# OrangeSodahub/InfGen

Measured on AMD Instinct MI355X. Metric: agent-steps/sec (closed-loop rollout), higher is better.
Workload: dtype f32

## Files before the change

### include/infgen_hip.h

```cpp
#ifndef INFGEN_HIP_H_
#define INFGEN_HIP_H_

#include <stdint.h>

#ifdef __cplusplus
extern "C" {
#endif

#define INFGEN_MAX_LAYERS 8

enum {
  INFGEN_Q_ATTN_PACK_SIZE = 0,
  INFGEN_Q_FOURIER_PACK_SIZE_N2 = 1,
  INFGEN_Q_FOURIER_PACK_SIZE_N3 = 2,
  INFGEN_Q_FOURIER_PACK_SIZE_N4 = 3,
  INFGEN_Q_TILE_ROWS = 4,
  INFGEN_Q_EDGE_ATTN_CAP = 5,
  INFGEN_Q_MAX_AGENTS = 6,
  INFGEN_Q_ABI_VERSION = 7,
  INFGEN_Q_SIZEOF_ROLLOUT = 8,
  INFGEN_Q_ATTN_SPLIT_ROWS = 9,
  INFGEN_Q_HEADS_SAMPLE_K = 10,
};
int infgen_layout_query(int what);
int infgen_attn_pack_offset(const char* field);
int infgen_fourier_pack_offset(const char* field, int n_dims, int dim);
const char* infgen_last_error(void);

typedef struct InfgenEdgeBuf {
  int* off;
  int* cnt;
  int* src;
  float* raw;
  float* rhat;
  int* total;
  int cap;
  int _pad;
} InfgenEdgeBuf;

typedef struct InfgenOptions {
  int use;
  int attn_mode;
  int gemm_terms;
  int fourier_mode;
  int edge_fuse;
  int edge_loop;
  int overlap;
  int row_group_margin;
  int layers_p;
  int rhat_format;
  int edge_kernel;
  int _pad0;
  const int* row_groups; const int* n_row_groups;
} InfgenOptions;

typedef struct InfgenRollout {
  int S, A_cap, T, M_cap, W, ring, R, token_size, grid_size, num_layers;
  int force_valid;
  int store_logits;
  float r_map, r_agent;
  const int* n_agents; const int* n_map; const int* av_index;
  float* pos; float* head; int* state; int* token; int* grid;
  uint8_t* tmask; uint8_t* imask; uint8_t* catflag;
  const int* type; int* bos;
  const float* map_pos; const float* map_orient;
  const float* attn_t[INFGEN_MAX_LAYERS]; const float* attn_m[INFGEN_MAX_LAYERS]; const float* attn_a[INFGEN_MAX_LAYERS];
  const float* four_t; const float* four_m; const float* four_a; const float* four_xa;
  const float* fusion_pack;
  const float* tok_head_pack; const float* st_head_pack;
  const float* tok_tab; const float* grid_tab; const float* state_emb;
  const float* cat_agent; const float* cat_seed; const float* vocab; const float* grid_xy;
  float* ringK[INFGEN_MAX_LAYERS]; float* ringV[INFGEN_MAX_LAYERS];
  const float* mapK[INFGEN_MAX_LAYERS]; const float* mapV[INFGEN_MAX_LAYERS];
  float* X; float* Q; float* U; float* Ka; float* Va; float* AGG; float* Z; float* SIG;
  InfgenEdgeBuf et, em, ea;
  float* raw2; float* cat; float* fus_in; float* tmp1; float* tmp2;
  int* next_token; int* next_state;
  float* logits;
  const int* teacher_token; const int* teacher_state;
  float* pred_traj; float* pred_head; float* pred_state;
  const int* first_new; const float* hv_ovr;
  int sample_k; int _pad1;
  const float* sample_u; float* logits_scratch;
  InfgenOptions opts;
  const int* teacher_grid;
  const float* four_t_dt;
  const float* teacher_pos; const float* teacher_head;
  const unsigned char* replay_row;
  const int* map_scene;
  float* tap_x;
  float* sample_logprob;
  float* token_logprob;
  int no_grid_token; int no_state_token;
} InfgenRollout;

int infgen_linear(const float* X, int ldx, const int* gather, int rows, int K,
                  const float* Wp, int Np, const float* bias, int N,
                  const float* pre_g, const float* pre_b, const float* post_g, const float* post_b, int relu,
                  float* Y, int ldy, void* stream);

typedef struct InfgenLinearDesc {
  const float* X; int ldx; const int* gather; int rows; int K;
  const float* Wp; int Np; const float* bias; int N;
  const float* pre_g; const float* pre_b; const float* post_g; const float* post_b; int relu;
  float* Y; int ldy;
} InfgenLinearDesc;
int infgen_linear_multi(const InfgenLinearDesc* desc, int n, void* stream);
int infgen_mlp_embedding(const float* X, int ldx, int rows, int K0, const float* pack, float* tmp1, float* tmp2,
                         float* Y, int ldy, void* stream);
int infgen_layernorm(const float* X, int rows, const float* gamma, const float* beta, float* Y, void* stream);
int infgen_fourier_embed(const float* raw, int n_dims, const int* count_dev, int e_cap, const float* pack,
                         const float* cat, int ldcat, float* out, int ldo, int normalize, void* stream);
int infgen_fourier_last_dim_table(const float* pack, int n_dims, float* table, void* stream);
int infgen_fourier_embed_tab(const float* raw, int n_dims, const int* count_dev, int e_cap, const float* pack,
                             const float* table, float* out, int ldo, int normalize, void* stream);
int infgen_set_fourier_mode(int mode);
int infgen_set_attn_mode(int mode);
int infgen_attn_pre(const float* X, int rows, const float* pack, int use_src_ln,
                    float* Q, float* U, float* K, float* V, void* stream);
int infgen_edge_attn(int rows, const float* Q, const float* U, const float* Ksrc, const float* Vsrc,
                     const int* off, const int* cnt, const int* src, const float* rhat,
                     float* AGG, float* Z, float* SIG, void* stream);
int infgen_edge_attn_fused(int rows, const float* Q, const float* pack, const float* Ksrc, const float* Vsrc,
                           const int* off, const int* cnt, const int* src, const float* rhat,
                           float* AGG, void* stream);
int infgen_fourier_embed_r24(const float* raw, int n_dims, const int* count_dev, int e_cap, const float* pack, void* out, void* stream);
int infgen_edge_attn_fused_r24(int rows, const float* Q, const float* pack, const float* Ksrc, const float* Vsrc,
                               const int* off, const int* cnt, const int* src, const void* rhat24, float* AGG, void* stream);
int infgen_set_rhat_format(int format);
int infgen_set_edge_kernel(int kernel);
int infgen_set_edge_fuse(int mode);
int infgen_get_options(InfgenOptions* out);
int infgen_thread_options(const InfgenOptions* o);
int infgen_get_effective_options(InfgenOptions* out);
int infgen_edge_fused_occupancy(void);
int infgen_debug_stream_read(const float* p, unsigned long long n_bytes, int width, float* out, void* stream);
int infgen_set_edge_loop(int variant);
int infgen_set_overlap(int mode);
int infgen_set_layers_p(int mode);
int infgen_layers_p_capacity(void);
int infgen_edge_attn_mode(int rows, const float* Q, const float* U, const float* Ksrc, const float* Vsrc,
                          const int* off, const int* cnt, const int* src, const float* rhat,
                          float* AGG, float* Z, float* SIG, int wide, void* stream);
int infgen_attn_post(float* X, int rows, const float* pack, const float* AGG, const float* Z, const float* SIG,
                     int has_pos, void* stream);
int infgen_attn_post_pre(float* X, int rows, const float* pack, const float* AGG, const float* Z, const float* SIG,
                         int has_pos, const float* next_pack, float* nQ, float* nU, float* nK, float* nV, void* stream);
int infgen_heads(const float* X, int rows, const float* tok_pack, const float* st_pack, int token_size,
                 float* logits, int* next_token, int* next_state, void* stream);
int infgen_heads_logprob(const float* X, int rows, const float* tok_pack, const float* st_pack, int token_size,
                         float* logits, int* next_token, int* next_state, float* token_logprob, void* stream);
int infgen_token_logprob(const float* logits, int rows, int n, const int* token, float* out, void* stream);
int infgen_heads_sample(const float* X, int rows, const float* tok_pack, const float* st_pack, int token_size, int k,
                        const float* uniform, float* logits, int* next_token, int* next_state, float* token_logprob,
                        float* sample_logprob, void* stream);
int infgen_heads_sample_fused(int attn_mode, int rows, int k);
int infgen_heads_logprob_fused(int attn_mode, int rows);
int infgen_map_token_head(const float* X, int ldx, const int* gather, int n, const float* pack, int token_size,
                          float* hidden, float* logits, long long* top_idx, void* stream);
int infgen_embedding_sum4(const float* tab0, const long long* idx0, int n0, const float* tab1, const long long* idx1, int n1,
                          const float* tab2, const long long* idx2, int n2, const float* tab3, const long long* idx3, int n3,
                          int rows, float* out, void* stream);
int infgen_map_graph(int S, int M_cap, const int* n_map, const float* pos, const float* orient, float radius,
                     int max_nbr, int* off, int* cnt, int* src, float* raw, int* total, int cap, void* stream);

int infgen_rollout_validate(const InfgenRollout* r);
int infgen_build_edges(const InfgenRollout* r, int c, int edgeless, void* stream);
int infgen_integrate(const InfgenRollout* r, int t, void* stream);
int infgen_raw_feature(const InfgenRollout* r, int col, void* stream);
int infgen_raw_feature_rows(const InfgenRollout* r, int col, const int* row_list, const int* row_mask, int n, void* stream);
int infgen_decode_layers(const InfgenRollout* r, int c, int edgeless, void* stream);
int infgen_decode_step(const InfgenRollout* r, int t, void* stream);
int infgen_rollout_run(const InfgenRollout* r, int t0, int t1, void* stream);

int infgen_sample_topk(const float* logits, int rows, int n, int k, const float* uniform, int* token, void* stream);
int infgen_sample_topk_logprob(const float* logits, int rows, int n, int k, const float* uniform, int* token,
// ... 178 lines not shown
```

### infgen_amd/_lib.py

```python
from __future__ import annotations

import ctypes as C
import threading
import os
from typing import Optional

_HERE = os.path.dirname(os.path.abspath(__file__))
LIB_PATH = os.path.join(_HERE, 'libinfgen_hip.so')
MAX_LAYERS = 8

_p = C.c_void_p
_i = C.c_int
_f = C.c_float


class LinearDesc(C.Structure):
    _fields_ = [('X', C.c_void_p), ('ldx', C.c_int), ('gather', C.c_void_p), ('rows', C.c_int), ('K', C.c_int),
                ('Wp', C.c_void_p), ('Np', C.c_int), ('bias', C.c_void_p), ('N', C.c_int),
                ('pre_g', C.c_void_p), ('pre_b', C.c_void_p), ('post_g', C.c_void_p), ('post_b', C.c_void_p), ('relu', C.c_int),
                ('Y', C.c_void_p), ('ldy', C.c_int)]


class EdgeBuf(C.Structure):
    _fields_ = [('off', _p), ('cnt', _p), ('src', _p), ('raw', _p), ('rhat', _p), ('total', _p),
# ... 1 lines not shown


class RadiusEdges(C.Structure):
    _fields_ = [('n_q', _i), ('_pad0', _i),
                ('q_node', _p), ('q_pt', _p), ('q_c0', _p), ('q_c1', _p), ('q_self', _p), ('q_pair_off', _p),
                ('p_pos', _p), ('p_head', _p), ('p_inv', _p),
                ('c_pos', _p), ('c_head', _p), ('c_inv', _p), ('c_ok', _p), ('c_src', _p), ('pair_ok', _p),
                ('radius', C.c_float), ('K', _i), ('gap_rule', _i), ('index_diff', _i), ('e_base', _i), ('_pad1', _i)]


class Insertion(C.Structure):
    _fields_ = [('attn_occ2sa', _p * 3), ('attn_pt2sa', _p * 3), ('attn_a2sa', _p * 3),
                ('four_a2sa', _p), ('four_pt2sa', _p),
                ('head_state', _p), ('head_type', _p), ('head_shape', _p), ('head_pos', _p), ('head_heading', _p),
                ('head_offset', _p), ('occ_embed', _p), ('shape_emb', _p), ('type_a_emb', _p), ('f_seed', _p),
                ('occ', _p), ('occ_emb', _p), ('Kocc', _p * 3), ('Vocc', _p * 3), ('mapK', _p * 3), ('mapV', _p * 3),
                ('Ksa', _p * 3), ('Vsa', _p * 3), ('Kh', _p * 3), ('Vh', _p * 3), ('Xc', _p),
                ('zero_agg', _p), ('zero_z', _p), ('zero_sig', _p),
                ('XS', _p), ('QS', _p), ('US', _p), ('AGGS', _p), ('ZS', _p), ('SIGS', _p), ('KN', _p), ('VN', _p),
                ('ea_s', EdgeBuf), ('em_s', EdgeBuf), ('ea_h', EdgeBuf), ('em_h', EdgeBuf),
                ('occ_off', _p), ('occ_cnt', _p), ('occ_src', _p),
                ('active', _p), ('n_new', _p), ('inserted', _p), ('new_row', _p), ('new_cell', _p), ('new_local', _p), ('new_shape', _p),
                ('prev_row', _p), ('prev_mask', _p), ('pend_row', _p), ('pend_mask', _p),
                ('hv_ovr', _p), ('shape_all', _p),
                ('hid', _p), ('lg_state', _p), ('lg_type', _p), ('shape', _p), ('lg_pos', _p), ('lg_heading', _p), ('offset', _p),
                ('t1', _p), ('t2', _p), ('shp', _p), ('host_dec', _p),
                ('r_seed', C.c_float), ('r_a2sa', C.c_float), ('r_pl2sa', C.c_float), ('angle_interval', C.c_float),
                ('n_heading', _i), ('force_enter', _i), ('insert_k', _i), ('max_new', _i),
                ('head_pos_xy', _p), ('head_heading_theta', _p), ('no_grid_token', _i), ('no_head_token', _i)]


class Options(C.Structure):
    _fields_ = [('use', _i), ('attn_mode', _i), ('gemm_terms', _i), ('fourier_mode', _i), ('edge_fuse', _i), ('edge_loop', _i),
                ('overlap', _i), ('row_group_margin', _i), ('layers_p', _i), ('rhat_format', _i), ('edge_kernel', _i), ('_pad0', _i), ('row_groups', _p), ('n_row_groups', _p)]


OPTIONS_VALUE_BYTES = C.sizeof(_i) * 12


class Rollout(C.Structure):
    _fields_ = [
        ('S', _i), ('A_cap', _i), ('T', _i), ('M_cap', _i), ('W', _i), ('ring', _i), ('R', _i),
        ('token_size', _i), ('grid_size', _i), ('num_layers', _i), ('force_valid', _i), ('store_logits', _i),
        ('r_map', _f), ('r_agent', _f),
        ('n_agents', _p), ('n_map', _p), ('av_index', _p),
        ('pos', _p), ('head', _p), ('state', _p), ('token', _p), ('grid', _p),
        ('tmask', _p), ('imask', _p), ('catflag', _p), ('type', _p), ('bos', _p),
        ('map_pos', _p), ('map_orient', _p),
        ('attn_t', _p * MAX_LAYERS), ('attn_m', _p * MAX_LAYERS), ('attn_a', _p * MAX_LAYERS),
        ('four_t', _p), ('four_m', _p), ('four_a', _p), ('four_xa', _p),
        ('fusion_pack', _p), ('tok_head_pack', _p), ('st_head_pack', _p),
        ('tok_tab', _p), ('grid_tab', _p), ('state_emb', _p), ('cat_agent', _p), ('cat_seed', _p),
        ('vocab', _p), ('grid_xy', _p),
        ('ringK', _p * MAX_LAYERS), ('ringV', _p * MAX_LAYERS), ('mapK', _p * MAX_LAYERS), ('mapV', _p * MAX_LAYERS),
        ('X', _p), ('Q', _p), ('U', _p), ('Ka', _p), ('Va', _p), ('AGG', _p), ('Z', _p), ('SIG', _p),
        ('et', EdgeBuf), ('em', EdgeBuf), ('ea', EdgeBuf),
        ('raw2', _p), ('cat', _p), ('fus_in', _p), ('tmp1', _p), ('tmp2', _p),
        ('next_token', _p), ('next_state', _p), ('logits', _p),
        ('teacher_token', _p), ('teacher_state', _p),
        ('pred_traj', _p), ('pred_head', _p), ('pred_state', _p),
        ('first_new', _p), ('hv_ovr', _p),
        ('sample_k', _i), ('_pad1', _i), ('sample_u', _p), ('logits_scratch', _p),
        ('opts', Options),
        ('teacher_grid', _p),
        ('four_t_dt', _p),
        ('teacher_pos', _p), ('teacher_head', _p),
        ('replay_row', _p),
        ('map_scene', _p),
        ('tap_x', _p),
        ('sample_logprob', _p),
        ('token_logprob', _p),
        ('no_grid_token', _i), ('no_state_token', _i),
    ]


class BatchIngest(C.Structure):
    _fields_ = ([(k, _i) for k in ('S', 'copies', 'A_cap', 'M_cap', 'T', 'T0', 'P', 'hc', 'H', 'motion_cols', 'pos_dim',
                                   'pt_pos_dim', 'n_polygons', '_pad0')] +
                [(k, _p) for k in ('agent_ptr', 'pt_ptr', 'av_index', 'src_graph', 'state_idx', 'token_idx', 'grid_token_idx',
                                   'token_pos', 'token_heading', 'raw_valid', 'valid_mask', 'shape', 'position', 'heading', 'type',
                                   'id', 'pt_position', 'pt_orientation', 'pt_token_idx', 'pt_type', 'pt_pl_type', 'pt_polygon',
                                   'light_type',
                                   'pos', 'head', 'state', 'token', 'gridtok', 'tmask', 'imask', 'catflag', 'atype', 'bos',
                                   'shape10', 'n_agents', 'av', 'n_map', 'map_pos', 'map_orient', 'map_tok', 'map_type', 'map_pl',
                                   'map_light', 'htok', 'hst', 'p0', 'h0', 'shp', 'gt', 'val', 'ids', 'counts',
                                   'replay_in', 'plan_token', 'plan_state', 'plan_pos', 'plan_head',
                                   'teacher_token', 'teacher_state', 'teacher_pos', 'teacher_head', 'replay_row')])


SYMBOLS = {
    'infgen_layout_query': (_i, [_i]),
    'infgen_attn_pack_offset': (_i, [C.c_char_p]),
    'infgen_fourier_pack_offset': (_i, [C.c_char_p, _i, _i]),
    'infgen_last_error': (C.c_char_p, []),
    'infgen_linear': (_i, [_p, _i, _p, _i, _i, _p, _i, _p, _i, _p, _p, _p, _p, _i, _p, _i, _p]),
    'infgen_linear_multi': (_i, [_p, _i, _p]),
    'infgen_radius_edges': (_i, [_p, _p, _p]),
    'infgen_motion_features': (_i, [_p, _p, _p, _p, _i, _i, _p, _p]),
    'infgen_layernorm': (_i, [_p, _i, _p, _p, _p, _p]),
    'infgen_fourier_embed': (_i, [_p, _i, _p, _i, _p, _p, _i, _p, _i, _i, _p]),
    'infgen_set_fourier_mode': (_i, [_i]),
    'infgen_set_attn_mode': (_i, [_i]),
# ... 3 lines not shown
    'infgen_rollout_validate': (_i, [_p]),
    'infgen_set_edge_loop': (_i, [_i]),
    'infgen_set_rhat_format': (_i, [_i]),
    'infgen_set_edge_kernel': (_i, [_i]),
    'infgen_mlp_embedding': (_i, [_p, _i, _i, _i, _p, _p, _p, _p, _i, _p]),
    'infgen_get_options': (_i, [C.POINTER(Options)]),
    'infgen_thread_options': (_i, [C.POINTER(Options)]),
    'infgen_get_effective_options': (_i, [C.POINTER(Options)]),
    'infgen_edge_fused_occupancy': (_i, []),
    'infgen_debug_stream_read': (_i, [_p, C.c_ulonglong, _i, _p, _p]),
    'infgen_set_overlap': (_i, [_i]),
    'infgen_edge_attn_fused': (_i, [_i, _p, _p, _p, _p, _p, _p, _p, _p, _p, _p]),
    'infgen_edge_attn_fused_r24': (_i, [_i, _p, _p, _p, _p, _p, _p, _p, _p, _p, _p]),
    'infgen_fourier_embed_r24': (_i, [_p, _i, _p, _i, _p, _p, _p]),
    'infgen_embedding_sum4': (_i, [_p, _p, _i, _p, _p, _i, _p, _p, _i, _p, _p, _i, _i, _p, _p]),
    'infgen_fourier_last_dim_table': (_i, [_p, _i, _p, _p]),
    'infgen_fourier_embed_tab': (_i, [_p, _i, _p, _i, _p, _p, _p, _i, _i, _p]),
    'infgen_distance_to_nearest_object': (_i, [_p, _p, _p, _p, _p, _p, _i, _i, _i, _i, C.c_float, _p, _p, _p]),
    'infgen_kinematic_features': (_i, [_p, _p, _p, _p, _i, _i, C.c_float, _p, _p, _p, _p, _p]),
    'infgen_time_to_collision': (_i, [_p, _p, _p, _p, _p, _p, _p, _p, _i, _i, _i, _i, _p, _p]),
    'infgen_set_gemm_terms': (_i, [_i]),
    'infgen_active_row_groups': (_i, [_p, _i, _i, _i, _p, _p, _p]),
    'infgen_set_row_groups': (_i, [_p, _p, _i]),
    'infgen_set_row_limits': (_i, [_p, _i, _i]),
    'infgen_fetch_enterings': (_i, [_p] * 5 + [_i] * 3 + [_p, _i, _f, _f, _i, _i] + [_p] * 9 + [_i, _p, _i, _p, _p]),
    'infgen_tokenize_agent': (_i, [_p] * 9 + [_i] * 10 + [_p] * 8),
    'infgen_distance_to_road_edge': (_i, [_p] * 9 + [_i] * 4 + [_p, _p, _p, _i, _f, _p, _p]),
    'infgen_window_log_likelihood': (_i, [_p, _p, _i, _i, _i, _i, _p, _p, _i, _p, _p, _p]),
    'infgen_placement_features': (_i, [_p, _p, _p, _p, _p, _i, _i, _i, _i, _i, _p, _p, _p, _p, _p]),
    'infgen_bundle_scores': (_i, [_p] * 14 + [_i] * 11 + [_p] * 5),
    'infgen_match_map_tokens': (_i, [_p, _p, _p, _i, _i, _p, _p]),
    'infgen_match_agent_tokens': (_i, [_p, _p, _p, _p, _p, _p, C.c_longlong, _i, _i, _i, _i, _p, _p, _p]),
    'infgen_attn_pre': (_i, [_p, _i, _p, _i, _p, _p, _p, _p, _p]),
    'infgen_edge_attn': (_i, [_i, _p, _p, _p, _p, _p, _p, _p, _p, _p, _p, _p, _p]),
    'infgen_edge_attn_mode': (_i, [_i, _p, _p, _p, _p, _p, _p, _p, _p, _p, _p, _p, _i, _p]),
    'infgen_attn_post': (_i, [_p, _i, _p, _p, _p, _p, _i, _p]),
    'infgen_attn_post_pre': (_i, [_p, _i, _p, _p, _p, _p, _i, _p, _p, _p, _p, _p, _p]),
    'infgen_heads': (_i, [_p, _i, _p, _p, _i, _p, _p, _p, _p]),
    'infgen_heads_logprob': (_i, [_p, _i, _p, _p, _i, _p, _p, _p, _p, _p]),
    'infgen_token_logprob': (_i, [_p, _i, _i, _p, _p, _p]),
    'infgen_heads_sample': (_i, [_p, _i, _p, _p, _i, _i, _p, _p, _p, _p, _p, _p, _p]),
    'infgen_heads_sample_fused': (_i, [_i, _i, _i]),
    'infgen_heads_logprob_fused': (_i, [_i, _i]),
    'infgen_map_token_head': (_i, [_p, _i, _p, _i, _p, _i, _p, _p, _p, _p]),
    'infgen_map_graph': (_i, [_i, _i, _p, _p, _p, _f, _i, _p, _p, _p, _p, _p, _i, _p]),
    'infgen_build_edges': (_i, [C.POINTER(Rollout), _i, _i, _p]),
    'infgen_integrate': (_i, [C.POINTER(Rollout), _i, _p]),
    'infgen_raw_feature': (_i, [C.POINTER(Rollout), _i, _p]),
    'infgen_raw_feature_rows': (_i, [_p, _i, _p, _p, _i, _p]),
    'infgen_decode_layers': (_i, [C.POINTER(Rollout), _i, _i, _p]),
    'infgen_decode_step': (_i, [C.POINTER(Rollout), _i, _p]),
    'infgen_rollout_run': (_i, [C.POINTER(Rollout), _i, _i, _p]),
    'infgen_sample_topk': (_i, [_p, _i, _i, _i, _p, _p, _p]),
    'infgen_sample_topk_logprob': (_i, [_p, _i, _i, _i, _p, _p, _p, _p]),
    'infgen_occupancy': (_i, [C.POINTER(Rollout), _i, _p, _p]),
    'infgen_occupancy_embed': (_i, [C.POINTER(Rollout), _i, _p, _p, _p, _p]),
    'infgen_point_edges': (_i, [C.POINTER(Rollout), _i, _p, _p, _i, _i, _f, _i, _f, _i, C.POINTER(EdgeBuf), C.POINTER(EdgeBuf), _p]),
    'infgen_insert_decide': (_i, [C.POINTER(Rollout), _i, _i, _i, _p, _p, _p, _p, _p, _p, _p, _p, _p, _p, _p, _p]),
    'infgen_insert_seed': (_i, [C.POINTER(Rollout), C.POINTER(Insertion), _i, _i, _i, _p, _p]),
    'infgen_insert_heading': (_i, [C.POINTER(Rollout), C.POINTER(Insertion), _i, _i, _i, _p]),
    'infgen_insert_decide_topk': (_i, [C.POINTER(Rollout), _i, _i, _i, _p, _p, _p, _p, _p, _p, _p, _p, _p, _p, _p, _i, _p, _p]),
    'infgen_insert_finalize': (_i, [C.POINTER(Rollout), _i, _f, _p, _p, _p, _i, _p, _p, _p]),
    'infgen_prof_enable': (_i, [C.c_uint, _i]),
    'infgen_prof_collect': (_i, [C.POINTER(C.c_double), C.POINTER(_i), C.POINTER(C.c_double), C.POINTER(C.c_ulonglong)]),
    'infgen_prof_collect_steps': (_i, [C.POINTER(C.c_double), C.POINTER(_i), C.POINTER(C.c_double), C.POINTER(C.c_ulonglong),
                                       C.POINTER(C.c_double), C.POINTER(_i)]),
# ... 22 lines not shown


class InfgenHipError(RuntimeError):
    pass


def load() -> C.CDLL:
    global _lib
    if _lib is not None:
        return _lib
    if not os.path.exists(LIB_PATH):
        raise InfgenHipError(
            f'{LIB_PATH} not found: build it with `python -c "import __graft_entry__ as g; g.build()"` '
            f'or `make -C infgen_amd/csrc` (there is no CPU fallback for the product path)')
    import torch
    lib = C.CDLL(LIB_PATH)
    for name, (res, args) in SYMBOLS.items():
        fn = getattr(lib, name)
        fn.restype = res
        fn.argtypes = args
    if lib.infgen_layout_query(Q_SIZEOF_ROLLOUT) != C.sizeof(Rollout):
        raise InfgenHipError('InfgenRollout layout mismatch between include/infgen_hip.h and infgen_amd/_lib.py: '
                             f'{lib.infgen_layout_query(Q_SIZEOF_ROLLOUT)} != {C.sizeof(Rollout)}')
    _lib = lib
    return lib


def check(rc: int, what: str = '') -> None:
    if rc != 0:
        msg = load().infgen_last_error()
        raise InfgenHipError(f'{what} failed ({rc}): {msg.decode() if msg else "?"}')


def ptr(t) -> Optional[int]:
    if t is None:
        return None
    assert t.is_contiguous(), 'tensor must be contiguous'
    return t.data_ptr()


_tl = threading.local()


class thread_options:

    def __init__(self, opts: 'Options'):
        self.opts, self.prev = opts, None

    def __enter__(self):
        lib = load()
        depth = getattr(_tl, 'depth', 0)
        if depth > 0:
            self.prev = Options()
            check(lib.infgen_get_effective_options(C.byref(self.prev)), 'infgen_get_effective_options')
        check(lib.infgen_thread_options(C.byref(self.opts)), 'infgen_thread_options')
        _tl.depth = depth + 1
        return self

    def __exit__(self, *exc):
        _tl.depth -= 1
        check(load().infgen_thread_options(C.byref(self.prev) if self.prev is not None else None), 'infgen_thread_options')
        return False


_prof_mask = 0


def prof_enable(mask: int, max_launches: int = 20000) -> None:
    global _prof_mask
    check(load().infgen_prof_enable(mask, max_launches), 'infgen_prof_enable')
# ... 33 lines not shown
```

### infgen_amd/csrc/api.hip

```cpp
#include <cstdio>
#include <cstring>
#include <cstdlib>
#include <string>
#include <vector>
#include <atomic>
#include <mutex>
#include <unordered_map>
#include "kernels.h"
#include "../../include/infgen_hip.h"

using namespace ig;

static thread_local std::string g_err;

static int fail(const char* where, const char* what) {
  g_err = std::string(where) + ": " + what;
  return -1;
}
static int check_launch(const char* where) {
  hipError_t e = hipGetLastError();
  if (e != hipSuccess) return fail(where, hipGetErrorString(e));
  return 0;
}
#define RET_IF(x) do { int _r = (x); if (_r) return _r; } while (0)

extern "C" const char* infgen_last_error(void) { return g_err.c_str(); }

static int env_int(const char* name, int dflt, bool* is_set = nullptr) {
  const char* e = getenv(name);
  if (is_set) *is_set = e != nullptr;
  return e ? atoi(e) : dflt;
}
static int env_layers_p() { const int v = env_int("INFGEN_LAYERS_P", 1); return v < 0 ? 0 : v > 2 ? 2 : v; }
static int env_lp_rows_min() {
  bool set8 = false;
  const int rows8 = env_int("INFGEN_LP_ROWS8", 0, &set8);
  return set8 ? (rows8 ? 8 : 16) : env_int("INFGEN_LP_ROWS_MIN", 4);
}
namespace knob {
const int layers_p = env_layers_p();
const int qs_dbg = env_int("INFGEN_QS_DBG", 0);
const int fh12_min = env_int("INFGEN_FH12_MIN", 150000);
const int fh12_multi_rows = env_int("INFGEN_FH12_MULTI_ROWS", 0);
const int fourier_nomulti = env_int("INFGEN_FOURIER_NOMULTI", 0);
const int attn_hs_max = env_int("INFGEN_ATTN_HS_MAX", 6144);
const int attn_waves = env_int("INFGEN_ATTN_WAVES", IG_QSU ? 8 : 4);
const int warm = env_int("INFGEN_WARM", 1);
const int warm_max_groups = env_int("INFGEN_WARM_MAX_GROUPS", 128);
const int edge_dbg = env_int("INFGEN_EDGE_DBG", 0);
const int edge_noxcd = env_int("INFGEN_EDGE_NOXCD", 0);
const int edge_small = env_int("INFGEN_EDGE_SMALL", 4096);
const int edge_wg2 = env_int("INFGEN_EDGE_WG2", 1);
const int edge_lds_pad = env_int("INFGEN_EDGE_LDS_PAD", 0);
const int heads_nosplit = env_int("INFGEN_HEADS_NOSPLIT", 0);
const int be_wide_scenes = env_int("INFGEN_BE_WIDE_SCENES", 128);
const int int_group_scenes = env_int("INFGEN_INT_GROUP_SCENES", 128);
const int no_tail_fold = env_int("INFGEN_NO_TAIL_FOLD", 0);
const int lp_max_chunks = env_int("INFGEN_LP_MAX_CHUNKS", 2);
const int lp_max_groups = env_int("INFGEN_LP_MAX_GROUPS", 256);
const int lp_rows_min = env_lp_rows_min();
const int lp_trace = env_int("INFGEN_LP_TRACE", 0);
const char* const lp_spin_str = getenv("INFGEN_LP_SPIN_LIMIT");
const unsigned lp_spin_limit = lp_spin_str ? (unsigned)strtoul(lp_spin_str, nullptr, 0) : 0u;
}

namespace {
InfgenOptions g_def = {0,  2,  3,  1,  1,  6,  0,
                        0,  knob::layers_p,  0,  1, 0, nullptr, nullptr};
int g_def_group_rows = 0;
const int* g_def_limit_n_agents = nullptr;
int g_def_limit_A_cap = 0;
struct Active { const InfgenOptions* o; int group_rows; const int* n_agents; int A_cap; };
thread_local Active tl_active = {nullptr, 0, nullptr, 0};
thread_local InfgenOptions tl_thread_opts;
thread_local bool tl_thread_set = false;
inline const InfgenOptions& O() { return tl_active.o ? *tl_active.o : tl_thread_set ? tl_thread_opts : g_def; }
inline int group_rows() { return tl_active.o ? tl_active.group_rows : g_def_group_rows; }
inline const int* limit_n_agents() { return tl_active.o ? tl_active.n_agents : g_def_limit_n_agents; }
inline int limit_A_cap() { return tl_active.o ? tl_active.A_cap : g_def_limit_A_cap; }
struct OptScope {
  Active prev;
  explicit OptScope(const InfgenRollout* r) : prev(tl_active) {
    if (r && r->opts.use) tl_active = Active{&r->opts, r->S * r->A_cap, r->opts.row_groups ? r->n_agents : nullptr, r->A_cap};
  }
  ~OptScope() { tl_active = prev; }
};
}

extern "C" int infgen_get_options(InfgenOptions* out) {
  if (!out) return fail("infgen_get_options", "null pointer");
  *out = g_def;
  return 0;
}

extern "C" int infgen_thread_options(const InfgenOptions* o) {
  if (o) { tl_thread_opts = *o; tl_thread_opts.row_groups = nullptr; tl_thread_opts.n_row_groups = nullptr; }
  tl_thread_set = o != nullptr;
  return 0;
}

extern "C" int infgen_get_effective_options(InfgenOptions* out) {
// ... 352 lines not shown
  if (per <= 0) return grid;
  w = req; w.wg0 = wg0; w.per_xcd = per;
  return wg0 + 8 * per;
}

static void launch_attn_h(const AttnHArgs& a_in, void* stream) {
  AttnHArgs a = a_in;
  a.dbg = knob::qs_dbg;
  if (O().row_groups && a.rows == group_rows()) { a.groups = O().row_groups; a.n_groups = O().n_row_groups; }
  if (attn_kind(a.rows) == 2) {
    const int grid = warm_take(a.warm, ceil_div(a.rows, 16));
    hipLaunchKernelGGL(by_terms(k_attn_hs<3>, k_attn_hs_b16<1>, k_attn_hs<1>), dim3(grid), dim3(512), 0, (hipStream_t)stream, a);
    return;
  }
  t_warm = WarmArgs{};
  if (knob::attn_waves != 8) {
    auto kern = by_terms(k_attn_h<4, 3>, k_attn_h_b16<4, 1>, k_attn_h<4, 1>);
    hipLaunchKernelGGL(kern, dim3(grid64(a.rows)), dim3(256), 0, (hipStream_t)stream, a);
  } else {
    int grid = ceil_div(a.rows, 128);
    if (grid > 256) grid = 256;
    hipLaunchKernelGGL((k_attn_h<8, 3>), dim3(grid), dim3(512), 0, (hipStream_t)stream, a);
  }
}

static double attn_pre_macs(int rows, const void* Q, const void* U, const void* K, const void* V) {
  return (double)rows * 16384.0 * ((Q || U ? 1 : 0) + (K ? 1 : 0) + (V ? 1 : 0) + (U ? 1 : 0));
}
static double attn_post_macs(int rows, int has_pos, const void* next_pack, const void* nQ, const void* nU, const void* nK, const void* nV) {
  return (double)rows * (196608.0 + (has_pos ? 16384.0 : 0.0)) + (next_pack ? attn_pre_macs(rows, nQ, nU, nK, nV) : 0.0);
}
static double heads_macs(int rows, int token_size) { return (double)rows * (2 * 16384.0 + 128.0 * token_size + 384.0); }

extern "C" int infgen_attn_pre(const float* X, int rows, const float* pack, int use_src_ln,
                               float* Q, float* U, float* K, float* V, void* stream) {
  if (rows <= 0) return 0;
  { ProfScope _ps(INFGEN_KID_ATTN_PRE, stream, attn_pre_macs(rows, Q, U, K, V));
    if (attn_kind(rows)) {
      launch_attn_h(AttnHArgs{const_cast<float*>(X), rows, nullptr, nullptr, nullptr, nullptr, 0, pack, use_src_ln, Q, U, K, V}, stream);
    } else {
      AttnPreArgs a{X, rows, pack, use_src_ln, Q, U, K, V};
      hipLaunchKernelGGL(k_attn_pre, dim3(ceil_div(rows, TR)), dim3(NT), 0, (hipStream_t)stream, a);
    } }
  return check_launch("infgen_attn_pre");
}

static int edge_attn_impl(int rows, const float* Q, const float* U, const float* Ksrc, const float* Vsrc,
                          const int* off, const int* cnt, const int* src, const float* rhat,
                          float* AGG, float* Z, float* SIG, int wide, void* stream, const int* row_mask = nullptr) {
  if (rows <= 0) return 0;
  EdgeAttnArgs a{rows, Q, U, Ksrc, Vsrc, EdgeSet{off, cnt, src, rhat}, AGG, Z, SIG, nullptr, nullptr, 0, 0, wide ? row_mask : nullptr};
  if (limit_n_agents() && O().row_groups && rows == group_rows() && !wide) {
    a.n_agents = limit_n_agents(); a.A_cap = limit_A_cap(); a.margin = O().row_group_margin;
  }
  { ProfScope _ps(INFGEN_KID_EDGE_ATTN, stream);
    if (wide) hipLaunchKernelGGL(k_edge_attn_wide, dim3(rows), dim3(512), 0, (hipStream_t)stream, a);
    else hipLaunchKernelGGL(k_edge_attn, dim3(ceil_div(rows, 4)), dim3(NT), 0, (hipStream_t)stream, a); }
  return check_launch("infgen_edge_attn");
}

extern "C" int infgen_set_edge_fuse(int mode) {
  if (mode < 0 || mode > 2) return fail("infgen_set_edge_fuse", "mode must be 0 (off), 1 (from 257 rows) or 2 (always)");
  g_def.edge_fuse = mode;
  return 0;
}

extern "C" int infgen_set_rhat_format(int format) {
  if (format != 0 && format != 1) return fail("infgen_set_rhat_format", "format must be 0 (fp32 rows) or 1 (packed 24-bit rows)");
  g_def.rhat_format = format;
  return 0;
}

extern "C" int infgen_set_edge_kernel(int kernel) {
  if (kernel < 0 || kernel > 2) return fail("infgen_set_edge_kernel", "kernel must be 0, 1 or 2");
  g_def.edge_kernel = kernel;
  return 0;
}

extern "C" int infgen_set_edge_loop(int v) {
  if (v != 4 && v != 6 && v != 8) return fail("infgen_set_edge_loop", "edges per trip must be 4, 6 or 8");
  g_def.edge_loop = v;
  return 0;
}

extern "C" int infgen_edge_fused_occupancy(void) {
  int n = -1;
  if (hipOccupancyMaxActiveBlocksPerMultiprocessor(&n, k_edge_fused<6, true, 1, 8>, 512, 0) != hipSuccess) return -1;
  return n;
}

static int edge_fused_launch(int rows, const float* Q, const float* pack, const float* Ksrc, const float* Vsrc, const EdgeSet& es,
                             float* AGG, int rows_per_scene, int kv_once, void* stream, int r24 = 0) {
  if (rows <= 0) return 0;
  if (!pack || !es.rhat) return fail("infgen_edge_attn_fused", "needs the layer pack and rhat");
  const int dbg = knob::edge_dbg, no_xcd = knob::edge_noxcd, small_max = knob::edge_small, wg2 = knob::edge_wg2;
  const int G = O().edge_loop;
  const bool small = rows <= small_max && G == 6;
  const bool two = !small && wg2 && G == 6;
  const int tr = (small || two) ? 16 : 32;
  EdgeFusedArgs a{rows, Q, pack, Ksrc, Vsrc, es, AGG, nullptr, nullptr, dbg, 0, kv_once};
  int grid = ceil_div(rows, tr);
  if (O().row_groups && rows == group_rows()) { a.groups = O().row_groups; a.n_groups = O().n_row_groups; }
  else if (rows_per_scene > tr && rows_per_scene % tr == 0 && !(no_xcd & 1)) {
    a.tiles_per_scene = rows_per_scene / tr;
    const int grp = 8 * a.tiles_per_scene;
    grid = ceil_div(grid, grp) * grp;
  }
  if (no_xcd & 2) a.kv_once = 0;
  if (!r24 && (O().edge_kernel == 2 || (O().edge_kernel == 1 && !small))) {
    EdgeFusedArgs m = a;
    int mg = ceil_div(rows, 16);
    m.tiles_per_scene = 0;
    if (!m.groups && rows_per_scene > 16 && rows_per_scene % 16 == 0 && !(no_xcd & 1)) {
      m.tiles_per_scene = rows_per_scene / 16;
      const int grp = 8 * m.tiles_per_scene;
      mg = ceil_div(mg, grp) * grp;
    }
    m.n_virtual = mg;
    t_warm = WarmArgs{};
    { ProfScope _ps(INFGEN_KID_EDGE_ATTN, stream);
      auto k3 = G == 4 ? k_edge_fused3<4> : G == 8 ? k_edge_fused3<8> : k_edge_fused3<6>;
      hipLaunchKernelGGL(k3, dim3(mg), dim3(512), knob::edge_lds_pad, (hipStream_t)stream, m); }
    return check_launch("infgen_edge_attn_fused(k_edge_fused3)");
  }
  a.n_virtual = grid;
  if (small) grid = warm_take(a.warm, grid); else t_warm = WarmArgs{};
  static unsigned long long* ef_trace = nullptr;
  if (dbg & 128) {
    if (!ef_trace && hipMalloc(&ef_trace, 64 * sizeof(unsigned long long)) != hipSuccess) return fail("infgen_edge_attn_fused", "trace buffer");
    (void)hipMemsetAsync(ef_trace, 0, 64 * sizeof(unsigned long long), (hipStream_t)stream);
    a.dbgbuf = reinterpret_cast<unsigned*>(ef_trace);
  }
  { ProfScope _ps(INFGEN_KID_EDGE_ATTN, stream);
    auto kern = small ? (r24 ? k_edge_fused<6, true, 1, 16> : k_edge_fused<6, false, 1, 16>)
              : two ? (r24 ? k_edge_fused<6, true, 1, 8> : k_edge_fused<6, false, 1, 8>)
              : r24 ? (G == 4 ? k_edge_fused<4, true, 2, 16> : G == 8 ? k_edge_fused<8, true, 2, 16> : k_edge_fused<6, true, 2, 16>)
                    : (G == 4 ? k_edge_fused<4, false, 2, 16> : G == 8 ? k_edge_fused<8, false, 2, 16> : k_edge_fused<6, false, 2, 16>);
    hipLaunchKernelGGL(kern, dim3(grid), dim3(two ? 512 : 1024), 0, (hipStream_t)stream, a); }
  if (dbg & 128) {
    static int dumps = 0;
    if (dumps++ < 3) {
      unsigned long long hst[64];
      (void)hipStreamSynchronize((hipStream_t)stream);
      (void)hipMemcpy(hst, ef_trace, sizeof(hst), hipMemcpyDeviceToHost);
      for (int i = 1; i < 8; ++i) fprintf(stderr, "[ef trace] %d +%lld\n", i, hst[i] && hst[0] ? (long long)(hst[i] - hst[0]) : -1ll);
    }
  }
  return check_launch("infgen_edge_attn_fused");
}

extern "C" int infgen_edge_attn_fused(int rows, const float* Q, const float* pack, const float* Ksrc, const float* Vsrc,
                                      const int* off, const int* cnt, const int* src, const float* rhat,
                                      float* AGG, void* stream) {
  return edge_fused_launch(rows, Q, pack, Ksrc, Vsrc, EdgeSet{off, cnt, src, rhat}, AGG, 0, 0, stream);
}

extern "C" int infgen_fourier_embed_r24(const float* raw, int n, const int* count_dev, int e_cap, const float* pack, void* out,
                                        void* stream) {
  return fourier_embed_impl(raw, n, count_dev, e_cap, pack, nullptr, 0, static_cast<float*>(out), 128, 1, 1, stream);
}

extern "C" int infgen_edge_attn_fused_r24(int rows, const float* Q, const float* pack, const float* Ksrc, const float* Vsrc,
                                          const int* off, const int* cnt, const int* src, const void* rhat24,
                                          float* AGG, void* stream) {
  return edge_fused_launch(rows, Q, pack, Ksrc, Vsrc, EdgeSet{off, cnt, src, static_cast<const float*>(rhat24)}, AGG, 0, 0, stream, 1);
}

extern "C" int infgen_edge_attn(int rows, const float* Q, const float* U, const float* Ksrc, const float* Vsrc,
                                const int* off, const int* cnt, const int* src, const float* rhat,
                                float* AGG, float* Z, float* SIG, void* stream) {
  return edge_attn_impl(rows, Q, U, Ksrc, Vsrc, off, cnt, src, rhat, AGG, Z, SIG, rows <= 256 ? 1 : 0, stream);
}

extern "C" int infgen_edge_attn_mode(int rows, const float* Q, const float* U, const float* Ksrc, const float* Vsrc,
                                     const int* off, const int* cnt, const int* src, const float* rhat,
                                     float* AGG, float* Z, float* SIG, int wide, void* stream) {
  return edge_attn_impl(rows, Q, U, Ksrc, Vsrc, off, cnt, src, rhat, AGG, Z, SIG, wide, stream);
}

static int attn_post_fused(float* X, int rows, const float* pack, const float* AGG, const float* Z, const float* SIG,
                           int has_pos, const float* next_pack, float* nQ, float* nU, float* nK, float* nV, void* stream) {
  if (rows <= 0) return 0;
  { ProfScope _ps(INFGEN_KID_ATTN_POST, stream, attn_post_macs(rows, has_pos, next_pack, nQ, nU, nK, nV));
    if (attn_kind(rows)) {
      launch_attn_h(AttnHArgs{X, rows, pack, AGG, Z, SIG, has_pos, next_pack, 0, nQ, nU, nK, nV}, stream);
    } else {
      AttnPostArgs a{X, rows, pack, AGG, Z, SIG, has_pos, next_pack, nQ, nU, nK, nV};
      hipLaunchKernelGGL(k_attn_post, dim3(ceil_div(rows, TR)), dim3(NT), 0, (hipStream_t)stream, a);
    } }
  return check_launch("infgen_attn_post");
}

extern "C" int infgen_attn_post(float* X, int rows, const float* pack, const float* AGG, const float* Z,
                                const float* SIG, int has_pos, void* stream) {
  return attn_post_fused(X, rows, pack, AGG, Z, SIG, has_pos, nullptr, nullptr, nullptr, nullptr, nullptr, stream);
}

extern "C" int infgen_attn_post_pre(float* X, int rows, const float* pack, const float* AGG, const float* Z,
                                    const float* SIG, int has_pos, const float* next_pack, float* nQ, float* nU,
                                    float* nK, float* nV, void* stream) {
  return attn_post_fused(X, rows, pack, AGG, Z, SIG, has_pos, next_pack, nQ, nU, nK, nV, stream);
}

extern "C" int infgen_match_agent_tokens(const unsigned char* valid, const float* pos, const float* heading, const float* shape,
                                        const int* type, const float* tok, long long tok_agent_stride, int A, int T, int shift,
                                        int n_token, int* token_index, float* token_contour, void* stream) {
  if (A <= 0) return 0;
  if (shift <= 0 || T <= shift) return fail("infgen_match_agent_tokens", "need 0 < shift < T");
  if (n_token <= 0 || n_token > 2048) return fail("infgen_match_agent_tokens", "n_token must be in 1..2048");
  MatchTokensArgs a{valid, pos, heading, shape, type, tok, tok_agent_stride, A, T, shift, n_token, token_index, token_contour};
  hipLaunchKernelGGL(k_match_tokens, dim3(A), dim3(256), 0, (hipStream_t)stream, a);
  return check_launch("infgen_match_agent_tokens");
}

extern "C" int infgen_tokenize_agent(unsigned char* valid, float* pos, float* heading, float* velocity, const int* type,
                                    const float* tok, const float* shape_in, float* shape_out, float* wl_work, int A, int T,
                                    int shift, int current_step, int n_token, int invalid_state, int valid_state,
                                    int enter_state, int exit_state, int predict_state, int* token_index,
                                    float* token_contour, int* state_idx, float* token_pos, float* token_heading,
                                    unsigned char* token_valid, unsigned char* raw_token_valid, void* stream) {
  if (A <= 0) return 0;
  if (shift <= 0 || T <= shift || current_step < shift || current_step >= T)
    return fail("infgen_tokenize_agent", "need 0 < shift <= current_step < T");
  if (n_token <= 0 || n_token > 2048) return fail("infgen_tokenize_agent", "n_token must be in 1..2048");
  TokenizeArgs t{valid, pos, heading, velocity, type, wl_work, shape_in, shape_out, A, T, shift, current_step,
                 invalid_state, valid_state, enter_state, exit_state, predict_state, token_index, token_contour,
                 state_idx, token_pos, token_heading, token_valid, raw_token_valid};
  hipLaunchKernelGGL(k_tokenize_prep, dim3((A + 63) / 64), dim3(64), 0, (hipStream_t)stream, t);
  MatchTokensArgs m{valid, pos, heading, wl_work, type, tok, 0, A, T, shift, n_token, token_index, token_contour};
  hipLaunchKernelGGL(k_match_tokens, dim3(A), dim3(256), 0, (hipStream_t)stream, m);
  hipLaunchKernelGGL(k_tokenize_state, dim3((A + 63) / 64), dim3(64), 0, (hipStream_t)stream, t);
  return check_launch("infgen_tokenize_agent");
}

// ... 379 lines not shown
                nullptr, nullptr, nullptr, nullptr, 0, logits, token_size};
  const int gy = tiles < 512 ? min(passes, ceil_div(512, tiles)) : 1;
  hipLaunchKernelGGL(k_linear, dim3(tiles, gy), dim3(NT), 0, s, l1);
  hipLaunchKernelGGL(k_map_topk, dim3(ceil_div(n, 4)), dim3(256), 0, s, a);
  return check_launch("infgen_map_token_head");
}

extern "C" int infgen_embedding_sum4(const float* tab0, const long long* idx0, int n0, const float* tab1, const long long* idx1, int n1,
                                     const float* tab2, const long long* idx2, int n2, const float* tab3, const long long* idx3, int n3,
                                     int rows, float* out, void* stream) {
  if (rows <= 0) return 0;
  if (!tab0 || !tab1 || !tab2 || !tab3 || !idx0 || !idx1 || !idx2 || !idx3 || !out || n0 < 1 || n1 < 1 || n2 < 1 || n3 < 1)
    return fail("infgen_embedding_sum4", "null table / index array or empty table");
  EmbedSum4Args a{{tab0, tab1, tab2, tab3}, {idx0, idx1, idx2, idx3}, {n0, n1, n2, n3}, rows, out};
  hipLaunchKernelGGL(k_embedding_sum4, dim3((unsigned)(((long long)rows * 32 + NT - 1) / NT)), dim3(NT), 0, (hipStream_t)stream, a);
  return check_launch("infgen_embedding_sum4");
}

extern "C" int infgen_map_graph(int S, int M_cap, const int* n_map, const float* pos, const float* orient,
                                float radius, int max_nbr, int* off, int* cnt, int* src, float* raw, int* total,
                                int cap, void* stream) {
  if (S <= 0 || M_cap <= 0) return 0;
  if (hipMemsetAsync(total, 0, sizeof(int), (hipStream_t)stream) != hipSuccess)
    return fail("infgen_map_graph", "memset failed");
  MapGraphArgs a{S, M_cap, n_map, pos, orient, radius, max_nbr, EdgeBuf{off, cnt, src, raw, total, cap}, 0};
  a.lds_tokens = (M_cap <= 4096 && M_cap % (4 * MAP_GRAPH_C) == 0) ? M_cap : 0;
  { ProfScope _ps(INFGEN_KID_MAP_GRAPH, stream);
    hipLaunchKernelGGL(k_map_graph, dim3(ceil_div(S * M_cap, 4 * MAP_GRAPH_C)), dim3(NT), (size_t)a.lds_tokens * 12, (hipStream_t)stream, a); }
  return check_launch("infgen_map_graph");
}

static SceneState scene_of(const InfgenRollout* r) {
  SceneState st;
  st.S = r->S; st.A_cap = r->A_cap; st.T = r->T; st.M_cap = r->M_cap; st.W = r->W; st.ring = r->ring;
  st.n_agents = r->n_agents; st.n_map = r->n_map; st.av_index = r->av_index;
  st.pos = r->pos; st.head = r->head; st.state = r->state; st.token = r->token; st.grid = r->grid;
  st.tmask = r->tmask; st.imask = r->imask; st.catflag = r->catflag; st.type = r->type; st.bos = r->bos;
  st.map_pos = r->map_pos; st.map_orient = r->map_orient; st.map_scene = r->map_scene;
  st.first_new = r->first_new; st.hv_ovr = r->hv_ovr;
  return st;
}
static EdgeBuf ebuf(const InfgenEdgeBuf& e) { return EdgeBuf{e.off, e.cnt, e.src, e.raw, e.total, e.cap}; }
static EdgeSet eset(const InfgenEdgeBuf& e) { return EdgeSet{e.off, e.cnt, e.src, e.rhat}; }

static int validate(const InfgenRollout* r, const char* where) {
  if (!r) return fail(where, "null context");
  if (r->A_cap > 1024 || r->A_cap <= 0) return fail(where, "A_cap must be in 1..1024");
  if (r->A_cap % 32) return fail(where, "A_cap must be a multiple of 32");
  if (r->num_layers <= 0 || r->num_layers > INFGEN_MAX_LAYERS) return fail(where, "bad num_layers");
  if (r->ring <= r->W) return fail(where, "ring must exceed the temporal window");
  if (r->W > 16) return fail(where, "temporal window larger than 16 columns is not supported");
  if ((r->no_grid_token | r->no_state_token) & ~1) return fail(where, "no_grid_token / no_state_token must be 0 or 1");
  if (r->token_logprob && !(r->store_logits && r->logits) && !r->logits_scratch) {
    const int mode = (r->opts.use ? r->opts : O()).attn_mode;
    const bool sampled = r->sample_k > 1 && r->sample_u;
    const bool fused = sampled ? heads_sample_fused_for(mode, r->S * r->A_cap, r->sample_k) : attn_split_for(mode, r->S * r->A_cap);
    if (!fused) return fail(where, "token_logprob needs store_logits or logits_scratch [rows][token_size] (few rows, or sampling)");
  }
  return 0;
}

static int build_edges_impl(const InfgenRollout* r, int c, int edgeless, void* stream, bool zero_totals, unsigned long long* clear_keys = nullptr,
                            bool clear_sync = false) {
  RET_IF(validate(r, "infgen_build_edges"));
  OptScope _opts(r);
  hipStream_t s = (hipStream_t)stream;
  if (!edgeless && zero_totals) {
    if (r->em.total == r->et.total + 1 && r->ea.total == r->et.total + 2) {
      if (hipMemsetAsync(r->et.total, 0, 3 * sizeof(int), s) != hipSuccess) return fail("infgen_build_edges", "memset failed");
    } else if (hipMemsetAsync(r->et.total, 0, sizeof(int), s) != hipSuccess ||
               hipMemsetAsync(r->em.total, 0, sizeof(int), s) != hipSuccess ||
               hipMemsetAsync(r->ea.total, 0, sizeof(int), s) != hipSuccess)
      return fail("infgen_build_edges", "memset failed");
  }
  BuildEdgesArgs a;
  a.st = scene_of(r); a.c = c; a.edgeless = edgeless; a.r_map = r->r_map; a.r_agent = r->r_agent;
  a.rows = r->S * r->A_cap; a.t = ebuf(r->et); a.m = ebuf(r->em); a.a = ebuf(r->ea);
  a.clear_keys = clear_keys;
  a.clear_sync = clear_sync ? reinterpret_cast<int*>(r->SIG) : nullptr;
  a.prof = (g_prof.mask & ((1u << INFGEN_KID_EDGE_ATTN) | (1u << INFGEN_KID_BUILD_EDGES))) ? g_prof.rows_dev : nullptr;
  { ProfScope _ps(INFGEN_KID_BUILD_EDGES, stream);
    a.map_lds = r->M_cap < 4096 ? r->M_cap : 4096;
    const size_t lds = (size_t)a.map_lds * 8;
// ... 251 lines not shown
    if (hipEventRecord(g_ev_m, g_side) != hipSuccess) return fail("infgen_decode_layers", "event failed");
    RET_IF(launch_fourier(step_fourier_set(r, FS_AGENT, sm), g_side));
    if (hipEventRecord(g_ev_a, g_side) != hipSuccess) return fail("infgen_decode_layers", "event failed");
    RET_IF(launch_fourier(step_fourier_set(r, FS_TEMPORAL, sm), stream));
  } else if (fourier_multi_ok(rows, edgeless)) {
    const int n_sets = with_xa ? 4 : 3;
    FourierMultiArgs m;
    for (int k = 0; k < n_sets; ++k) m.set[k] = step_fourier_set(r, (FourierSet)k, sm);
    int cap = r->et.cap > r->em.cap ? r->et.cap : r->em.cap;
    if (r->ea.cap > cap) cap = r->ea.cap;
    const bool wide = knob::fh12_multi_rows > 0 && rows >= knob::fh12_multi_rows && three_terms() && FH_WAVES == 8;
    const int grid = fourier_h_grid(cap, wide);
    { ProfScope _ps(INFGEN_KID_FOURIER, stream);
      if (wide) hipLaunchKernelGGL(k_fourier_h12_multi<3>, dim3(grid, n_sets), dim3(FH12_NT), 0, (hipStream_t)stream, m);
      else hipLaunchKernelGGL(by_terms(k_fourier_h_multi<3>, k_fourier_h_multi_b16<1>, k_fourier_h_multi<1>), dim3(grid, n_sets),
                              dim3(FH_NT), 0, (hipStream_t)stream, m); }
    RET_IF(check_launch("infgen_decode_layers(fourier)"));
  } else if (!edgeless) {
    for (FourierSet k : {FS_TEMPORAL, FS_MAP, FS_AGENT}) RET_IF(launch_fourier(step_fourier_set(r, k, sm), stream));
  }
  return 0;
}

constexpr int LP_REFUSED = -12345;
static int layers_p_launch(const InfgenRollout* r, int c, const StepMode& sm, void* stream, bool sync_clear = true) {
  const int rows = r->S * r->A_cap;
  LayersPArgs a;
  a.rows = rows; a.A_cap = r->A_cap; a.num_layers = r->num_layers;
  a.X = r->X;
  for (int i = 0; i < r->num_layers; ++i) {
    a.attn_t[i] = r->attn_t[i]; a.attn_m[i] = r->attn_m[i]; a.attn_a[i] = r->attn_a[i];
    a.ringK[i] = r->ringK[i]; a.ringV[i] = r->ringV[i]; a.mapK[i] = r->mapK[i]; a.mapV[i] = r->mapV[i];
  }
  a.slot_off = (size_t)(c % r->ring) * rows * D;
  a.Ka[0] = r->Ka; a.Va[0] = r->Va; a.Ka[1] = r->U; a.Va[1] = r->U + (size_t)rows * D;
  a.et = eset(r->et); a.em = eset(r->em); a.ea = eset(r->ea);
  a.sync = reinterpret_cast<int*>(r->SIG);
  a.trace = nullptr;
  const int lp_trace = knob::lp_trace;
  static unsigned long long* trace_dev = nullptr;
  if (lp_trace) {
    if (!trace_dev && hipMalloc(&trace_dev, 2048 * sizeof(unsigned long long)) != hipSuccess) return fail("infgen_decode_layers", "trace buffer");
    (void)hipMemsetAsync(trace_dev, 0, 2048 * sizeof(unsigned long long), (hipStream_t)stream);
    a.trace = trace_dev;
  }
  if (sync_clear && hipMemsetAsync(a.sync, 0, (size_t)r->S * sizeof(int), (hipStream_t)stream) != hipSuccess)
    return fail("infgen_decode_layers", "memset failed");
  const int limit = lp_limit();
  a.rows_per_wg = 16;
  for (int rr = 8; rr >= 4 && rr >= knob::lp_rows_min; rr >>= 1)
    if (r->A_cap % rr == 0 && rows / rr <= (rr == 4 ? limit / 2 : limit)) a.rows_per_wg = rr;
  const int gps = r->A_cap / a.rows_per_wg;
  const int per = rows / a.rows_per_wg <= limit ? r->S : (a.rows_per_wg == 16 ? lp_chunk_scenes(r, limit) : 0);
  if (per <= 0 || per * gps > infgen_layers_p_capacity()) return fail("infgen_decode_layers", "k_layers_p: batch does not fit the device's resident capacity");
  auto kern = a.rows_per_wg == 4 ? (sm.r24 ? k_layers_p<true, 4> : k_layers_p<false, 4>)
            : a.rows_per_wg == 8 ? (sm.r24 ? k_layers_p<true, 8> : k_layers_p<false, 8>)
                                 : (sm.r24 ? k_layers_p<true, 16> : k_layers_p<false, 16>);
  const bool capturing = is_capturing(stream);
  a.spin_limit = capturing ? (1u << 22) : knob::lp_spin_str ? knob::lp_spin_limit : (O().layers_p == 2 ? 0u : (1u << 24));
  std::unique_lock<std::mutex> lk(g_lp_mu, std::defer_lock);
  LpOrder& ord = g_lp_order[lp_current_device()];
  if (!capturing) {
    lk.lock();
    if (!ord.ev && hipEventCreateWithFlags(&ord.ev, hipEventDisableTiming) != hipSuccess)
      return fail("infgen_decode_layers", "event creation failed");
    if (ord.any && hipStreamWaitEvent((hipStream_t)stream, ord.ev, 0) != hipSuccess) {
      (void)hipGetLastError();
      ord.any = false;
// ... 15 lines not shown
        (void)hipGetLastError();
        if (s0 > 0) return fail("infgen_decode_layers", "k_layers_p: cooperative launch of a later chunk refused");
        g_lp_refused.store(true);
        return LP_REFUSED;
      }
    }
  }
  if (!capturing) {
    ord.any = hipEventRecord(ord.ev, (hipStream_t)stream) == hipSuccess;
    if (!ord.any) (void)hipGetLastError();
    lk.unlock();
  }
  if (lp_trace) {
    static int dumps = 0;
    if (dumps++ == lp_trace) {
      std::vector<unsigned long long> h(2048);
      (void)hipStreamSynchronize((hipStream_t)stream);
      (void)hipMemcpy(h.data(), trace_dev, 2048 * sizeof(unsigned long long), hipMemcpyDeviceToHost);
      for (int i = 0; i < 1024 && (i == 0 || h[2 * i + 1]); ++i)
        fprintf(stderr, "[lp trace] %d %llu %llu\n", i, h[2 * i], i ? h[2 * i + 1] - h[2 * i - 1] : 0ull);
    }
  }
  return check_launch("infgen_decode_layers(k_layers_p)");
}

static int layers_core(const InfgenRollout* r, int c, int edgeless, void* stream, bool lp_sync_clear = true) {
  const int rows = r->S * r->A_cap;
  const StepMode sm = step_mode(r, rows, edgeless, stream);
  if (sm.lp && sm.fuse) {
    const int rc = layers_p_launch(r, c, sm, stream, lp_sync_clear);
    if (rc != LP_REFUSED) return rc;
  }
  const bool overlap = sm.overlap, fuse = sm.fuse; const int r24 = sm.r24;
  const size_t slot = (size_t)(c % r->ring) * rows * D;
  const int L = r->num_layers;
  float* U = fuse ? nullptr : r->U;
  const float* Z = fuse ? nullptr : r->Z;
  const float* SIG = fuse ? nullptr : r->SIG;
  const int has_pos = fuse ? 0 : 1;
  const int QB = 16384;
  const bool skip_edges = edgeless && fuse;
  if (skip_edges && hipMemsetAsync(r->AGG, 0, (size_t)rows * D * sizeof(float), (hipStream_t)stream) != hipSuccess)
    return fail("infgen_decode_layers", "memset failed");
  auto edge = [&](const float* pack, const float* Ks, const float* Vs, const InfgenEdgeBuf& e, int kv_once = 0, const float* next_pack = nullptr, int fmt = -1) {
    if (skip_edges) return 0;
    if (fuse && O().attn_mode != 0)
      warm_request(pack + AH_POST + 4 * (QB / 4), 48 * QB, next_pack ? next_pack + AH_PRE : nullptr, 16 * QB);
    return fuse ? edge_fused_launch(rows, r->Q, pack, Ks, Vs, eset(e), r->AGG, r->A_cap, kv_once, stream, fmt < 0 ? r24 : fmt)
                : infgen_edge_attn(rows, r->Q, r->U, Ks, Vs, e.off, e.cnt, e.src, e.rhat, r->AGG, r->Z, r->SIG, stream);
  };
  RET_IF(infgen_attn_pre(r->X, rows, r->attn_t[0], 0, r->Q, U, r->ringK[0] + slot, r->ringV[0] + slot, stream));
  auto warm_post = [&](const float* pack) { if (fuse && O().attn_mode != 0) warm_request(pack + AH_POST, 52 * QB, nullptr, 0); };
  for (int i = 0; i < L; ++i) {
    RET_IF(edge(r->attn_t[i], r->ringK[i], r->ringV[i], r->et, 1, r->attn_m[i]));
    warm_post(r->attn_m[i]);
    RET_IF(infgen_attn_post_pre(r->X, rows, r->attn_t[i], r->AGG, Z, SIG, has_pos, r->attn_m[i], r->Q, U,
                                nullptr, nullptr, stream));
    if (overlap && i == 0 && hipStreamWaitEvent((hipStream_t)stream, g_ev_m, 0) != hipSuccess)
      return fail("infgen_decode_layers", "join failed");
    RET_IF(edge(r->attn_m[i], r->mapK[i], r->mapV[i], r->em, 0, r->attn_a[i]));
    warm_post(r->attn_a[i]);
    RET_IF(infgen_attn_post_pre(r->X, rows, r->attn_m[i], r->AGG, Z, SIG, has_pos, r->attn_a[i], r->Q, U,
                                r->Ka, r->Va, stream));
    if (overlap && i == 0 && hipStreamWaitEvent((hipStream_t)stream, g_ev_a, 0) != hipSuccess)
      return fail("infgen_decode_layers", "join failed");
    RET_IF(edge(r->attn_a[i], r->Ka, r->Va, r->ea, 0, i + 1 < L ? r->attn_t[i + 1] : nullptr, sm.ra));
    if (i + 1 < L) {
      warm_post(r->attn_t[i + 1]);
      RET_IF(infgen_attn_post_pre(r->X, rows, r->attn_a[i], r->AGG, Z, SIG, has_pos, r->attn_t[i + 1], r->Q, U,
                                  r->ringK[i + 1] + slot, r->ringV[i + 1] + slot, stream));
    } else {
      RET_IF(infgen_attn_post(r->X, rows, r->attn_a[i], r->AGG, Z, SIG, has_pos, stream));
    }
    if (r->tap_x && hipMemcpyAsync(r->tap_x + (size_t)i * rows * D, r->X, (size_t)rows * D * sizeof(float), hipMemcpyDeviceToDevice,
                                   (hipStream_t)stream) != hipSuccess)
      return fail("infgen_decode_layers", "tap copy failed");
  }
  return 0;
}

extern "C" int infgen_decode_layers(const InfgenRollout* r, int c, int edgeless, void* stream) {
  RET_IF(validate(r, "infgen_decode_layers"));
  OptScope _opts(r);
  ProfPhase _pp(edgeless ? t_prof_phase : 1);
  const StepMode sm = step_mode(r, r->S * r->A_cap, edgeless, stream);
  const bool lp = sm.lp && sm.fuse && r->SIG != nullptr;
  RET_IF(prepare_edges(r, c, edgeless, stream, true, false, nullptr, lp));
  return layers_core(r, c, edgeless, stream, !lp);
}

extern "C" int infgen_decode_step(const InfgenRollout* r, int t, void* stream) {
  RET_IF(validate(r, "infgen_decode_step"));
  OptScope _opts(r);
  ProfPhase _pp(1);
  const int rows = r->S * r->A_cap;
  const int c = 1 + t;
  if (t < 0 || c + 1 > r->T - 1) return fail("infgen_decode_step", "step beyond the column range");
  RET_IF(infgen_decode_layers(r, c, 0, stream));
  float* lg = (r->store_logits && r->logits) ? r->logits + (size_t)t * rows * r->token_size : nullptr;
  const bool s_fused = r->sample_k > 1 && r->sample_u && heads_sample_fused_for(O().attn_mode, rows, r->sample_k);
  const bool sample = r->sample_k > 1 && r->sample_u && (s_fused || lg || r->logits_scratch);
  if (sample && !s_fused && !lg) lg = r->logits_scratch;
  const float* su = sample ? r->sample_u + (size_t)t * rows : nullptr;
// ... 263 lines not shown
  return 0;
}

extern "C" int infgen_insert_heading(const InfgenRollout* r, const InfgenInsertion* I, int t, int h_ready, int riders, void* stream) {
  RET_IF(validate(r, "infgen_insert_heading"));
  if (!I) return fail("infgen_insert_heading", "null insertion block");
  if (I->no_head_token && !I->head_heading_theta) return fail("infgen_insert_heading", "no_head_token needs head_heading_theta");
  OptScope _opts(r);
  hipStream_t hs = (hipStream_t)stream;
  const int S = r->S, rows = r->S * r->A_cap, c = 1 + t;
  RET_IF(mlp_embedding_fp32(I->new_shape, 3, S, 3, 8, I->shape_emb, I->t1, I->t2, I->shp, 128, stream));
  InsertCatArgs ca{S, r->A_cap, I->inserted, I->new_row, r->type, I->type_a_emb, I->shp, I->new_shape, const_cast<float*>(r->cat_agent),
                   I->shape_all, I->new_local};
  hipLaunchKernelGGL(k_insert_cat, dim3(ceil_div(S * 32, NT)), dim3(NT), 0, hs, ca);
  RET_IF(check_launch("k_insert_cat"));
  RET_IF(infgen_raw_feature_rows(r, c, I->new_row, I->inserted, S, stream));
  RET_IF(infgen_point_edges(r, c, I->new_local, I->inserted, 1, 3, I->r_a2sa, 24, I->r_pl2sa, 128, &I->ea_h, &I->em_h, stream));
  RET_IF(infgen_fourier_embed(I->ea_h.raw, 3, I->ea_h.total, I->ea_h.cap, r->four_a, nullptr, 0, I->ea_h.rhat, 128, 1, stream));
  RET_IF(infgen_fourier_embed(I->em_h.raw, 3, I->em_h.total, I->em_h.cap, r->four_m, nullptr, 0, I->em_h.rhat, 128, 1, stream));
  if (!h_ready) {
    if (hipMemcpyAsync(I->Xc, r->X, (size_t)rows * D * sizeof(float), hipMemcpyDeviceToDevice, hs) != hipSuccess)
      return fail("infgen_insert_heading", "copy failed");
    for (int i = 0; i < 3; ++i) {
      RET_IF(infgen_attn_post_pre(I->Xc, rows, r->attn_m[i], I->zero_agg, I->zero_z, I->zero_sig, 0, r->attn_a[i], nullptr, nullptr,
                                  I->Kh[i], I->Vh[i], stream));
      RET_IF(edgeless(I->Xc, rows, r->attn_a[i], I, stream));
    }
  }
  const int R = riders ? 2 * S : S;
  RET_IF(gather_rows(r->X, I->new_row, nullptr, S, rows, I->XS, stream));
  if (riders) RET_IF(gather_rows(r->X, I->pend_row, I->pend_mask, S, rows, I->XS + (size_t)S * D, stream));
  RET_IF(infgen_attn_pre(I->XS, R, r->attn_m[0], 0, I->QS, I->US, nullptr, nullptr, stream));
  for (int i = 0; i < 3; ++i) {
    RET_IF(infgen_edge_attn(S, I->QS, I->US, r->mapK[i], r->mapV[i], I->em_h.off, I->em_h.cnt, I->em_h.src, I->em_h.rhat, I->AGGS, I->ZS,
                            I->SIGS, stream));
    RET_IF(infgen_attn_post_pre(I->XS, R, r->attn_m[i], I->AGGS, I->ZS, I->SIGS, 1, r->attn_a[i], I->QS, I->US, riders ? I->KN : nullptr,
                                riders ? I->VN : nullptr, stream));
    if (riders) {
      RET_IF(scatter_rows2(I->KN + (size_t)S * D, I->VN + (size_t)S * D, I->pend_row, I->pend_mask, S, I->Kh[i], I->Vh[i], stream));
    }
    RET_IF(infgen_edge_attn(S, I->QS, I->US, I->Kh[i], I->Vh[i], I->ea_h.off, I->ea_h.cnt, I->ea_h.src, I->ea_h.rhat, I->AGGS, I->ZS,
                            I->SIGS, stream));
    if (i < 2) RET_IF(infgen_attn_post_pre(I->XS, R, r->attn_a[i], I->AGGS, I->ZS, I->SIGS, 1, r->attn_m[i + 1], I->QS, I->US, nullptr,
                                           nullptr, stream));
    else RET_IF(infgen_attn_post(I->XS, R, r->attn_a[i], I->AGGS, I->ZS, I->SIGS, 1, stream));
  }
  InfgenLinearDesc d1[2], d2[2];
  const size_t hs_ = (size_t)S * 128;
  const bool head_tok = !I->no_head_token, offset = !I->no_grid_token;
  if (head_tok) mlp_layer_descs(I->XS, S, I->head_heading, I->n_heading, I->hid + 4 * hs_, I->lg_heading, d1[0], d2[0]);
  else mlp_layer_descs(I->XS, S, I->head_heading_theta, 1, I->hid + 4 * hs_, I->lg_heading, d1[0], d2[0]);
  if (offset) mlp_layer_descs(I->XS, S, I->head_offset, 2, I->hid + 5 * hs_, I->offset, d1[1], d2[1]);
  RET_IF(infgen_linear_multi(d1, offset ? 2 : 1, stream));
  RET_IF(infgen_linear_multi(d2, offset ? 2 : 1, stream));
  RET_IF(insert_finalize_impl(r, c, I->angle_interval, I->inserted, I->new_row, I->lg_heading, head_tok ? I->n_heading : 1, I->offset,
                              I->hv_ovr, stream, head_tok, offset));
  RET_IF(infgen_raw_feature_rows(r, c, I->new_row, I->inserted, S, stream));
  hipLaunchKernelGGL(k_note_riders, dim3(ceil_div(S, NT)), dim3(NT), 0, hs, I->new_row, I->inserted, S, I->prev_row, I->prev_mask,
                     I->pend_row, I->pend_mask);
  return check_launch("k_note_riders");
}

extern "C" int infgen_ingest_batch(const InfgenBatchIngest* a, void* stream) {
  if (!a) return fail("infgen_ingest_batch", "null argument block");
  if (a->S <= 0) return 0;
  if (a->copies < 1 || a->S % a->copies) return fail("infgen_ingest_batch", "S must be a positive multiple of copies");
  if (a->A_cap < 1 || a->A_cap > MAX_SCENE_AGENTS) return fail("infgen_ingest_batch", "A_cap must be in 1..INFGEN_Q_MAX_AGENTS");
  if (a->M_cap < 1) return fail("infgen_ingest_batch", "M_cap must be positive");
// ... 39 lines not shown
```

### infgen_amd/csrc/attn_h.hip

```cpp
#include <type_traits>
#include "kernels.h"
#include "layout.h"
#include "tile.cuh"
#include "split.cuh"
#include "attn_h.cuh"

namespace ig {

template <int WAVES, int TERMS>
__global__ __launch_bounds__(64 * WAVES, WAVES == 4 ? 2 : 1) void k_attn_h(AttnHArgs a) {
  constexpr int NTH = 64 * WAVES, TILE = 16 * WAVES;
  constexpr int XRING = WAVES == 4 ? IG_AH_RING4 : IG_AH_RING8;
  __shared__ __attribute__((aligned(16))) unsigned short Wb[XRING][QUARTER];
  __shared__ __attribute__((aligned(16))) float Vt[VT_SIZE];
  __shared__ const unsigned short* seg_ptr[5];
  __shared__ int seg_n[5];
  const int ngroups = a.groups ? *a.n_groups : (a.rows + 15) / 16;
  const int ntiles = (ngroups + WAVES - 1) / WAVES;
  if ((int)blockIdx.x >= ntiles) return;
  const int tid = threadIdx.x;
  const int lane = tid & 63, w = tid >> 6;
  const int j = lane & 15, rg = lane >> 4;
  const float* P = a.pack;
  const float* NP = a.next_pack;
// ... 181 lines not shown
        if (need_u) {
          u32x4 Qh[4], Ql[4];
          const float cq = frags_scaled(q, Qh, Ql) * hdr[1];
          float* urow = valid ? a.nU + (size_t)row * (H * D) : nullptr;
          for (int hp = 0; hp < 4; ++hp) {
            const unsigned short* Wl = take();
#pragma unroll
            for (int hh = 0; hh < 2; ++hh) {
              u32x2 qh, ql;
#define IG_PICK(S) case S: qh = hh ? u32x2{Qh[S][2], Qh[S][3]} : u32x2{Qh[S][0], Qh[S][1]}; \
                           ql = hh ? u32x2{Ql[S][2], Ql[S][3]} : u32x2{Ql[S][0], Ql[S][1]}; break;
              switch (hp) { IG_PICK(0) IG_PICK(1) IG_PICK(2) default: IG_PICK(3) }
#undef IG_PICK
              const v4h vqh = __builtin_bit_cast(v4h, qh), vql = __builtin_bit_cast(v4h, ql);
#pragma unroll
              for (int ct = 0; ct < 8; ++ct) {
                const v4h ah = *reinterpret_cast<const v4h*>(Wl + ((hh * 8 + ct) * 2) * 256 + lane * 4);
                const v4h al = *reinterpret_cast<const v4h*>(Wl + ((hh * 8 + ct) * 2 + 1) * 256 + lane * 4);
                f32x4 acc = {0.f, 0.f, 0.f, 0.f};
                acc = __builtin_amdgcn_mfma_f32_16x16x16f16(ah, vqh, acc, 0, 0, 0);
                if constexpr (TERMS == 3) {
                  acc = __builtin_amdgcn_mfma_f32_16x16x16f16(ah, vql, acc, 0, 0, 0);
                  acc = __builtin_amdgcn_mfma_f32_16x16x16f16(al, vqh, acc, 0, 0, 0);
                }
                if (urow)
                  *reinterpret_cast<float4*>(urow + (2 * hp + hh) * D + 16 * ct + 4 * rg) =
                      make_float4(acc[0] * cq, acc[1] * cq, acc[2] * cq, acc[3] * cq);
              }
            }
          }
        }
      }
      if (need_kv) {
        f32x4 kk[8];
        zero_acc(kk);
        gemm_unit(kk, Bh, Bl);
        scale_bias(kk, inv_n * hdr[2], nullptr, rg);
        store_row(valid ? a.nK + (size_t)row * D : nullptr, kk, rg);
        zero_acc(kk);
        gemm_unit(kk, Bh, Bl);
        scale_bias(kk, inv_n * hdr[3], Vt + VT_N_BV, rg);
        store_row(valid && a.nV ? a.nV + (size_t)row * D : nullptr, kk, rg);
      }
    }
  }
}

#if !IG_BF16_OPERANDS
template __global__ void k_attn_h<4, 3>(AttnHArgs);
template __global__ void k_attn_h<8, 3>(AttnHArgs);
#endif
template __global__ void k_attn_h<4, 1>(AttnHArgs);

__global__ __launch_bounds__(1024) void k_active_groups(ActiveGroupsArgs a) {
  __shared__ int wave_cnt[16];
  __shared__ int base;
  const int total = (a.S * a.A_cap + 15) / 16;
  const int lane = threadIdx.x & 63, w = threadIdx.x >> 6;
  if (threadIdx.x == 0) base = 0;
  __syncthreads();
  for (int g0 = 0; g0 < total; g0 += 1024) {
    const int g = g0 + threadIdx.x;
    bool on = false;
    if (g < total) {
      const int r0 = 16 * g, r1 = min(16 * g + 15, a.S * a.A_cap - 1);
      const int s0 = r0 / a.A_cap, s1 = r1 / a.A_cap;
      on = (r0 - s0 * a.A_cap) < a.n_agents[s0] + a.margin;
      if (s1 != s0) on = on || a.n_agents[s1] + a.margin > 0;
    }
    const unsigned long long m = __ballot(on);
    if (lane == 0) wave_cnt[w] = __popcll(m);
    __syncthreads();
    int off = base;
    for (int k = 0; k < w; ++k) off += wave_cnt[k];
    if (on) a.groups[off + __popcll(m & ((1ull << lane) - 1))] = g;
// ... 9 lines not shown
```

### infgen_amd/csrc/attn_hs.hip

```cpp
#define IG_LN_PREFETCH 0
#include "kernels.h"
#include "layout.h"
#include "tile.cuh"
#include "split.cuh"
#include "attn_h.cuh"

namespace ig {

namespace {

template <int TERMS>
struct AFrag {
  v8h h[4], l[4];
  __device__ __forceinline__ void load(const unsigned short* W, int w, int lane) {
#pragma unroll
    for (int s = 0; s < 4; ++s) {
      h[s] = *reinterpret_cast<const v8h*>(W + (size_t)s * QUARTER + w * 1024 + lane * 8);
      if constexpr (TERMS == 3) l[s] = *reinterpret_cast<const v8h*>(W + (size_t)s * QUARTER + w * 1024 + 512 + lane * 8);
    }
  }
};

template <int TERMS>
__device__ __forceinline__ f32x4 mm_step(const AFrag<TERMS>& f, int s, u32x4 Bh, u32x4 Bl, f32x4 acc) {
// ... 205 lines not shown
          split_pair(q[2] * sc, q[3] * sc, hi, lo); qh[1] = hi; ql[1] = lo;
        }
        const v4h vqh = __builtin_bit_cast(v4h, qh), vql = __builtin_bit_cast(v4h, ql);
        const float cq = inv * hdr[1];
        float* urow = valid ? a.nU + (size_t)row * (H * D) + w * D + 4 * rg : nullptr;
        f32x4 acc[8];
#pragma unroll
        for (int ct = 0; ct < 8; ++ct) {
          const v4h ah = *reinterpret_cast<const v4h*>(Wk + (ct * 2) * 256);
          acc[ct] = __builtin_amdgcn_mfma_f32_16x16x16f16(ah, vqh, f32x4{0.f, 0.f, 0.f, 0.f}, 0, 0, 0);
          if constexpr (TERMS == 3) {
            const v4h al = *reinterpret_cast<const v4h*>(Wk + (ct * 2 + 1) * 256);
            acc[ct] = __builtin_amdgcn_mfma_f32_16x16x16f16(ah, vql, acc[ct], 0, 0, 0);
            acc[ct] = __builtin_amdgcn_mfma_f32_16x16x16f16(al, vqh, acc[ct], 0, 0, 0);
          }
        }
        if (urow) {
#pragma unroll
          for (int ct = 0; ct < 8; ++ct)
            *reinterpret_cast<float4*>(urow + 16 * ct) = make_float4(acc[ct][0] * cq, acc[ct][1] * cq, acc[ct][2] * cq, acc[ct][3] * cq);
        }
      }
    }
    if (need_kv) {
      f32x4 kk = {0.f, 0.f, 0.f, 0.f}, vv = kk;
#pragma unroll
      for (int s = 0; s < 4; ++s) {
        kk = mm_step<TERMS>(fb, s, Bh[s], Bl[s], kk);
        vv = mm_step<TERMS>(fc, s, Bh[s], Bl[s], vv);
      }
      kk = kk * splat4(inv_n * hdr[2]);
      vv = fma4(vv, splat4(inv_n * hdr[3]), lds4(Vt + VT_N_BV + own));
      if (valid) {
        *reinterpret_cast<float4*>(a.nK + (size_t)row * D + own) = make_float4(kk[0], kk[1], kk[2], kk[3]);
        if (a.nV) *reinterpret_cast<float4*>(a.nV + (size_t)row * D + own) = make_float4(vv[0], vv[1], vv[2], vv[3]);
      }
    }
  }
}

#if !IG_BF16_OPERANDS
template __global__ void k_attn_hs<3>(AttnHArgs);
#endif
template __global__ void k_attn_hs<1>(AttnHArgs);

}
```

### infgen_amd/csrc/edge_attn.cuh

```cuda
#pragma once
#include "kernels.h"

namespace ig {

typedef unsigned u32x2_t __attribute__((ext_vector_type(2)));
__device__ __forceinline__ float readlane_f(float v, int l) {
  return __int_as_float(__builtin_amdgcn_readlane(__float_as_int(v), l));
}

struct AttnState {
  float2 z[H];
  float2 ag;
  float m, lsum;
};

typedef float pk2 __attribute__((ext_vector_type(2)));
__device__ __forceinline__ pk2 pk_fma(pk2 a, pk2 b, pk2 c) { return __builtin_elementwise_fma(a, b, c); }
__device__ __forceinline__ pk2 bc_s(float s) {
#if defined(IG_EDGE_SPAIR)
  const unsigned u = __builtin_amdgcn_readfirstlane(__float_as_uint(s));
  unsigned long long p = ((unsigned long long)u << 32) | u;
  asm volatile("" : "+s"(p));
  return __builtin_bit_cast(pk2, p);
#elif defined(IG_EDGE_SVPAIR)
// ... 85 lines not shown
      m = mn;
    }
    const float pe = __builtin_amdgcn_exp2f(val - m);
    lsum += pe;
#if defined(IG_EDGE_OPSEL_BROADCAST)
    ag = pk_fma(bc_v(pe), v2, ag);
#else
    ag = pk2{fmaf(pe, v2[0], ag[0]), fmaf(pe, v2[1], ag[1])};
#endif
    if constexpr (HASR) {
#ifdef IG_EDGE_ZDROP
      constexpr int HZ = 1;
#else
      constexpr int HZ = H;
#endif
      float ph[HZ];
#pragma unroll
      for (int h = 0; h < HZ; ++h) ph[h] = readlane_f(pe, 8 * h);
#pragma unroll
      for (int h = 0; h < HZ; ++h) zz[h] = pk_fma(bc_s(ph[h]), r2, zz[h]);
    }
  }
};

__device__ __forceinline__ pk2 ea_ld(const float* p, bool nt) {
  return nt ? __builtin_nontemporal_load(reinterpret_cast<const pk2*>(p)) : *reinterpret_cast<const pk2*>(p);
}

template <int PF, bool ULDS, bool HASR>
__device__ __forceinline__ void edge_attn_wave2(const EdgeAttnArgs& a, int row, int E, int e_base, int e_first,
                                                int e_step, AttnState& st, const float* u_lds = nullptr, bool kv_once = false) {
  const int lane = lane_id();
  const bool b3 = lane & 8;
  EdgeAcc<HASR> acc;
  acc.q = *reinterpret_cast<const float2*>(a.Q + (size_t)row * D + 2 * lane);
  if constexpr (ULDS) acc.load_u(u_lds, lane);
  else if constexpr (HASR) acc.load_u(a.U + (size_t)row * (H * D), lane);
  acc.reset();
  const int n = E > e_first ? (E - e_first + e_step - 1) / e_step : 0;
  for (int c0 = 0; c0 < n; c0 += 64) {
    const int mc = min(64, n - c0);
    const int srcv = a.es.src[e_base + e_first + (c0 + min(lane, mc - 1)) * e_step];
    for (int i0 = 0; i0 < mc; i0 += PF) {
      pk2 kb[PF], vb[PF], rb[PF];
#pragma unroll
      for (int s = 0; s < PF; ++s) {
        const int ic = min(i0 + s, mc - 1);
        const int sj = __builtin_amdgcn_readlane(srcv, ic);
        const size_t e = (size_t)(e_base + e_first + (c0 + ic) * e_step);
        kb[s] = ea_ld(a.Ksrc + (size_t)sj * D + 2 * lane, kv_once);
        vb[s] = ea_ld(a.Vsrc + (size_t)sj * D + 2 * lane, kv_once);
        if constexpr (HASR) rb[s] = __builtin_nontemporal_load(reinterpret_cast<const pk2*>(a.es.rhat + e * D + 2 * lane));
      }
#pragma unroll
      for (int s = 0; s < PF; ++s) acc.step(kb[s], vb[s], HASR ? rb[s] : pk2{0.f, 0.f}, i0 + s < mc, b3);
    }
  }
#pragma unroll
  for (int h = 0; h < H; ++h) st.z[h] = make_float2(acc.zz[h][0], acc.zz[h][1]);
  st.ag = make_float2(acc.ag[0], acc.ag[1]);
  st.m = acc.m;
  st.lsum = acc.lsum;
}

__device__ __forceinline__ void edge_attn_write(const EdgeAttnArgs& a, int row, const AttnState& st) {
  const int lane = lane_id();
  const float inv = 1.0f / (st.lsum + 1e-16f);
  *reinterpret_cast<float2*>(a.AGG + (size_t)row * D + 2 * lane) = make_float2(st.ag.x * inv, st.ag.y * inv);
  if (a.Z) {
#pragma unroll
    for (int h = 0; h < H; ++h) {
      const float ih = readlane_f(inv, 8 * h);
      *reinterpret_cast<float2*>(a.Z + (size_t)row * (H * D) + h * D + 2 * lane) =
          make_float2(st.z[h].x * ih, st.z[h].y * ih);
    }
  }
  if ((lane & 7) == 0) a.SIG[(size_t)row * H + (lane >> 3)] = st.lsum * inv;
}

}
```

### infgen_amd/csrc/edge_fused.hip

```cpp
#include "kernels.h"
#include "layout.h"
#include "tile.cuh"
#include "split.cuh"
#include "edge_attn.cuh"

namespace ig {

constexpr int EF_HALVES = 2;
constexpr int EF_WAVES = 8 * EF_HALVES;
constexpr int EF_NT = 64 * EF_WAVES;
constexpr int EF_ROWS = 16 * EF_HALVES;
constexpr int EF_LDU = H * D + 4;
constexpr int EF_LDA = D + 4;

#ifndef IG_EF_TRACE
#define IG_EF_TRACE 0
#endif
#if IG_EF_TRACE
#define EF_STAMP(i) do { if ((a.dbg & 128) && blockIdx.x == 2600 && threadIdx.x == 0) reinterpret_cast<unsigned long long*>(a.dbgbuf)[i] = __builtin_readcyclecounter(); } while (0)
#else
#define EF_STAMP(i) do {} while (0)
#endif
template <int G, bool R24, int HALVES, int WAVES>
__global__ __launch_bounds__(64 * WAVES, 4) void k_edge_fused(EdgeFusedArgs a) {
// ... 63 lines not shown
    float m = fmaxf(fmaxf(fabsf(qv.x), fabsf(qv.y)), fmaxf(fabsf(qv.z), fabsf(qv.w)));
    m = fmaxf(m, __shfl_xor(m, 16, 64));
    m = fmaxf(m, __shfl_xor(m, 32, 64));
    unsigned ebits = __float_as_uint(m) >> 23;
    ebits = min(max(ebits, 15u), 253u);
    const float sc = __uint_as_float((268u - ebits) << 23), inv = __uint_as_float((ebits - 14u) << 23);
    u32x2 qh, ql;
    {
      unsigned hi, lo;
      split_pair(qv.x * sc, qv.y * sc, hi, lo); qh[0] = hi; ql[0] = lo;
      split_pair(qv.z * sc, qv.w * sc, hi, lo); qh[1] = hi; ql[1] = lo;
    }
    const v4h vqh = __builtin_bit_cast(v4h, qh), vql = __builtin_bit_cast(v4h, ql);
    const float cq = inv * hdr[1];
    f32x4 acc[8];
#pragma unroll
    for (int ct = 0; ct < 8; ++ct) acc[ct] = __builtin_amdgcn_mfma_f32_16x16x16f16(ah[ct], vqh, f32x4{0.f, 0.f, 0.f, 0.f}, 0, 0, 0);
#pragma unroll
    for (int ct = 0; ct < 8; ++ct) acc[ct] = __builtin_amdgcn_mfma_f32_16x16x16f16(ah[ct], vql, acc[ct], 0, 0, 0);
#pragma unroll
    for (int ct = 0; ct < 8; ++ct) acc[ct] = __builtin_amdgcn_mfma_f32_16x16x16f16(al[ct], vqh, acc[ct], 0, 0, 0);
    float* urow = UZ + jl * EF_LDU + h * D + 4 * g;
#pragma unroll
    for (int ct = 0; ct < 8; ++ct)
      *reinterpret_cast<float4*>(urow + 16 * ct) = make_float4(acc[ct][0] * cq, acc[ct][1] * cq, acc[ct][2] * cq, acc[ct][3] * cq);
  }
  EF_STAMP(2);
  __syncthreads();
  EF_STAMP(3);

  {
    const bool b3 = lane & 8;
    const bool kv_once = a.kv_once != 0;
    const unsigned lo8 = 8u * (unsigned)lane;
    auto ld8 = [&](const float* base, bool nt) {
      return ea_ld(reinterpret_cast<const float*>(reinterpret_cast<const char*>(base) + lo8), nt);
    };
    auto ld_r24 = [&](size_t e) {
      const char* rowp = reinterpret_cast<const char*>(a.es.rhat) + e * R24_ROW_BYTES;
      const unsigned hi = __builtin_nontemporal_load(reinterpret_cast<const unsigned*>(rowp + 4 * lane));
      const unsigned lo = __builtin_nontemporal_load(reinterpret_cast<const unsigned short*>(rowp + R24_LO_PLANE + 2 * lane));
      return pk2{__uint_as_float((hi << 16) | ((lo & 0xffu) << 8)), __uint_as_float((hi & 0xffff0000u) | (lo & 0xff00u))};
    };
    auto take_row = [&]() {
      int r = 0;
      if (lane == 0) { r = atomicAdd(&next_row, 1); if (SORT_ROWS && r < ROWS) r = row_order[r]; }
      return __builtin_amdgcn_readfirstlane(r);
    };
    for (int rl = take_row(); rl < ROWS; rl = take_row()) {
      const int rbase = (HALVES > 1 && (rl >> 4)) ? r0h[HALVES - 1] : r0h[0];
      const int drow = rbase + (rl & 15);
      const bool live = rbase >= 0 && drow < a.rows && !(a.dbg & 1);
      const int E = live ? __builtin_amdgcn_readfirstlane(a.es.cnt[drow]) : 0;
      const int e_base = live ? __builtin_amdgcn_readfirstlane(a.es.off[drow]) : 0;
      int sv = E > 0 ? a.es.src[e_base + min(lane, E - 1)] : 0;
      float* uz = UZ + rl * EF_LDU;
      EdgeAcc<true> acc;
      acc.q = *reinterpret_cast<const float2*>(AG + rl * EF_LDA + 2 * lane);
      acc.load_u(uz, lane);
      acc.reset();
      for (int c0 = 0; c0 < E; c0 += 64) {
        const int mc = min(64, E - c0);
        if (c0 > 0) sv = a.es.src[e_base + c0 + min(lane, mc - 1)];
        for (int i0 = 0; i0 < mc; i0 += G) {
          pk2 kb[G], vb[G], rb[G];
#pragma unroll
          for (int s = 0; s < G; ++s) {
            const int ic = min(i0 + s, mc - 1);
            const int sj = __builtin_amdgcn_readlane(sv, ic);
            kb[s] = ld8(a.Ksrc + (size_t)sj * D, kv_once);
            vb[s] = ld8(a.Vsrc + (size_t)sj * D, kv_once);
            if constexpr (R24) rb[s] = ld_r24((size_t)(e_base + c0 + ic));
            else rb[s] = ld8(a.es.rhat + (size_t)(e_base + c0 + ic) * D, true);
          }
#pragma unroll
          for (int s = 0; s < G; ++s) acc.step(kb[s], vb[s], rb[s], i0 + s < mc, b3);
        }
      }
      const float inv = 1.0f / (acc.lsum + 1e-16f);
      *reinterpret_cast<float2*>(AG + rl * EF_LDA + 2 * lane) = make_float2(acc.ag[0] * inv, acc.ag[1] * inv);
#pragma unroll
      for (int hd = 0; hd < H; ++hd) {
        const float ih = readlane_f(inv, 8 * hd);
        *reinterpret_cast<float2*>(uz + hd * D + 2 * lane) = make_float2(acc.zz[hd][0] * ih, acc.zz[hd][1] * ih);
      }
      if ((lane & 7) == 0) SG[rl * H + (lane >> 3)] = acc.lsum * inv;
    }
  }
  EF_STAMP(4);
  v8h p3h[4], p3l[4];
  if (mat) {
    const unsigned short* Wv = reinterpret_cast<const unsigned short*>(a.pack + AH_POST) + (size_t)hp * QUARTER +
                               (size_t)(hh * 4) * 2 * 512 + lane * 8;
#pragma unroll
    for (int s = 0; s < 4; ++s) {
      p3h[s] = *reinterpret_cast<const v8h*>(Wv + (s * 2) * 512);
      p3l[s] = *reinterpret_cast<const v8h*>(Wv + (s * 2 + 1) * 512);
    }
  }
  EF_STAMP(5);
  __syncthreads();
  EF_STAMP(6);

  if (mat) {
// ... 48 lines not shown
```

### infgen_amd/csrc/edge_fused3.hip

```cpp
#include "kernels.h"
#include "layout.h"
#include "tile.cuh"
#include "split.cuh"
#include "edge_attn.cuh"

namespace ig {

constexpr int E3_LDU = H * D + 4;
constexpr int E3_LDA = D + 4;
static_assert(E3_LDU * 4 >= 8 * 512, "a row's slot holds the ring of eight 512-byte rhat rows");

template <int G>
__global__ __launch_bounds__(512, 4) void k_edge_fused3(EdgeFusedArgs a) {
  static_assert(G % 2 == 0 && G >= 2 && G <= 8, "trips of 2, 4, 6 or 8 edges");
  __shared__ __attribute__((aligned(16))) float UZ[16 * E3_LDU];
  __shared__ __attribute__((aligned(16))) float AG[16 * E3_LDA];
  __shared__ float SG[16 * H];
  const int ngroups = a.groups ? *a.n_groups : (a.rows + 15) / 16;
  int tile = blockIdx.x;
  if (a.tiles_per_scene > 1) {
    const int tps = a.tiles_per_scene, grp = 8 * tps;
    const int bq = tile / grp, br = tile % grp;
    tile = bq * grp + (br % 8) * tps + br / 8;
  }
// ... 45 lines not shown
  {
    *reinterpret_cast<float4*>(AG + j * E3_LDA + DH * h + 4 * g) = qv;
    float m = fmaxf(fmaxf(fabsf(qv.x), fabsf(qv.y)), fmaxf(fabsf(qv.z), fabsf(qv.w)));
    m = fmaxf(m, __shfl_xor(m, 16, 64));
    m = fmaxf(m, __shfl_xor(m, 32, 64));
    unsigned ebits = __float_as_uint(m) >> 23;
    ebits = min(max(ebits, 15u), 253u);
    const float sc = __uint_as_float((268u - ebits) << 23), inv = __uint_as_float((ebits - 14u) << 23);
    u32x2 qh, ql;
    {
      unsigned hi, lo;
      split_pair(qv.x * sc, qv.y * sc, hi, lo); qh[0] = hi; ql[0] = lo;
      split_pair(qv.z * sc, qv.w * sc, hi, lo); qh[1] = hi; ql[1] = lo;
    }
    const v4h vqh = __builtin_bit_cast(v4h, qh), vql = __builtin_bit_cast(v4h, ql);
    const float cq = inv * hdr[1];
    f32x4 acc[8];
#pragma unroll
    for (int ct = 0; ct < 8; ++ct) acc[ct] = __builtin_amdgcn_mfma_f32_16x16x16f16(ah[ct], vqh, f32x4{0.f, 0.f, 0.f, 0.f}, 0, 0, 0);
#pragma unroll
    for (int ct = 0; ct < 8; ++ct) acc[ct] = __builtin_amdgcn_mfma_f32_16x16x16f16(ah[ct], vql, acc[ct], 0, 0, 0);
#pragma unroll
    for (int ct = 0; ct < 8; ++ct) acc[ct] = __builtin_amdgcn_mfma_f32_16x16x16f16(al[ct], vqh, acc[ct], 0, 0, 0);
    float* urow = UZ + j * E3_LDU + h * D + 4 * g;
#pragma unroll
    for (int ct = 0; ct < 8; ++ct)
      *reinterpret_cast<float4*>(urow + 16 * ct) = make_float4(acc[ct][0] * cq, acc[ct][1] * cq, acc[ct][2] * cq, acc[ct][3] * cq);
  }
  __syncthreads();

  {
    const int eh = lane >> 3, ei = lane & 7;
    const bool kv_once = a.kv_once != 0;
    const unsigned lo8 = 8u * (unsigned)lane;
    auto ld8 = [&](const float* base, bool nt) {
      return ea_ld(reinterpret_cast<const float*>(reinterpret_cast<const char*>(base) + lo8), nt);
    };
#pragma unroll 1
    for (int pass = 0; pass < 2; ++pass) {
      const int rl = pass ? rl2[1] : rl2[0];
      const int E = pass ? E2[1] : E2[0];
      const int e_base = pass ? eb2[1] : eb2[0];
      float* uz = UZ + rl * E3_LDU;
      pk2 ux[8];
      {
        const float* up = uz + eh * D + 4 * ei;
#pragma unroll
        for (int k = 0; k < 4; ++k) {
          const float4 t = *reinterpret_cast<const float4*>(up + 32 * k);
          ux[2 * k] = pk2{t.x, t.y} * pk2{EA_LOG2E, EA_LOG2E};
          ux[2 * k + 1] = pk2{t.z, t.w} * pk2{EA_LOG2E, EA_LOG2E};
        }
      }
      const float2 q0 = *reinterpret_cast<const float2*>(AG + rl * E3_LDA + 2 * lane);
      const pk2 q = pk2{q0.x, q0.y} * pk2{EA_LOG2E, EA_LOG2E};
      asm volatile("s_waitcnt lgkmcnt(0)" ::: "memory");
      const unsigned ring = lds_addr(uz);
      const float* rbase = uz + 4 * ei;
      pk2 zz[8];
#pragma unroll
      for (int k = 0; k < 8; ++k) zz[k] = pk2{0.f, 0.f};
      pk2 ag = pk2{0.f, 0.f};
      float m = -INFINITY, lsum = 0.f;
      const int lhalf = lane >> 5;
      const unsigned lcol = 16u * (unsigned)(lane & 31);
      for (int c0 = 0; c0 < E; c0 += 64) {
        const int mc = min(64, E - c0);
        int sv = pass ? sv2[1] : sv2[0];
        if (c0 > 0) sv = a.es.src[e_base + c0 + min(lane, mc - 1)];
        asm volatile("" : "+v"(sv));
        const char* rrows = reinterpret_cast<const char*>(a.es.rhat) + (size_t)(e_base + c0) * (D * sizeof(float));
        for (int i0 = 0; i0 < mc; i0 += G) {
#pragma unroll
          for (int p = 0; p < G / 2; ++p) {
            const int ic = min(i0 + 2 * p + lhalf, mc - 1);
            lds_dma16(rrows + (size_t)ic * (D * sizeof(float)) + lcol, ring + 1024u * (unsigned)p);
          }
          pk2 kb[G], vb[G];
#pragma unroll
          for (int s = 0; s < G; ++s) {
            const int ic = min(i0 + s, mc - 1);
            const int sj = __builtin_amdgcn_readlane(sv, ic);
            kb[s] = ld8(a.Ksrc + (size_t)sj * D, kv_once);
            vb[s] = ld8(a.Vsrc + (size_t)sj * D, kv_once);
          }
          asm volatile("s_waitcnt vmcnt(%0)" :: "n"(2 * G) : "memory");
          {
#pragma unroll
            for (int s = 0; s < G; ++s) {
              pk2 r[8];
#pragma unroll
              for (int k = 0; k < 4; ++k) {
                const float4 t = *reinterpret_cast<const float4*>(rbase + 128 * s + 32 * k);
                r[2 * k] = pk2{t.x, t.y};
                r[2 * k + 1] = pk2{t.z, t.w};
              }
              pk2 d2 = q * kb[s], d3 = ux[0] * r[0];
#pragma unroll
              for (int k = 1; k < 8; k += 2) d2 = pk_fma(ux[k], r[k], d2);
#pragma unroll
              for (int k = 2; k < 8; k += 2) d3 = pk_fma(ux[k], r[k], d3);
              d2 += d3;
              float val = sum8(d2[0] + d2[1]);
              {
                const unsigned lim = __builtin_amdgcn_readfirstlane(i0 + s < mc ? 0x7f800000u : 0xff800000u);
                asm("v_min_f32 %0, %1, %2" : "=v"(val) : "s"(lim), "v"(val));
              }
              const bool grow = val > m + EA_TAU;
              if (__any(grow)) {
                const float mn = grow ? val : m;
                const float sc = __builtin_amdgcn_exp2f(m - mn);
                lsum *= sc;
                const pk2 sc2 = bc_v(sc);
                ag *= sc2;
#pragma unroll
                for (int k = 0; k < 8; ++k) zz[k] *= sc2;
                m = mn;
// ... 73 lines not shown
```

### infgen_amd/csrc/edge_kernels.hip

```cpp
#include "kernels.h"
#include "edge_attn.cuh"

namespace ig {

constexpr int INVALID = 0, VALID = 1, ENTER = 2, EXIT = 3;
constexpr int NUM_SEED_FEATURE = 10;
constexpr int A2A_MAX_NBR = 300;
constexpr float MOTION_GAP = 1.0f, HEADING_GAP = 1.0f, INVALID_MOTION = -2.0f, INVALID_HEAD = -2.0f;

__global__ __launch_bounds__(NT) void k_edge_attn(EdgeAttnArgs a) {
  const int row = __builtin_amdgcn_readfirstlane(blockIdx.x * 4 + wave_id());
  if (row >= a.rows) return;
  if (a.n_agents && (row % a.A_cap) >= a.n_agents[row / a.A_cap] + a.margin + 15) return;
  const int E = __builtin_amdgcn_readfirstlane(a.es.cnt[row]);
  const int e_base = __builtin_amdgcn_readfirstlane(a.es.off[row]);
  const bool has_r = a.es.rhat != nullptr && a.U != nullptr;
  AttnState st;
  if (has_r) edge_attn_wave2<4, false, true>(a, row, E, e_base, 0, 1, st);
  else edge_attn_wave2<4, false, false>(a, row, E, e_base, 0, 1, st);
  edge_attn_write(a, row, st);
}

constexpr int WIDE_WAVES = 8;
__global__ __launch_bounds__(64 * WIDE_WAVES) void k_edge_attn_wide(EdgeAttnArgs a) {
// ... 120 lines not shown
      for (int wq = 0; wq < WMAX; ++wq) {
        const int j = lo + wq;
        sx[wq] = 0.f; sy[wq] = 0.f; sh[wq] = 0.f; sst[wq] = 0;
        if (j < c && wq < st.W) {
          const size_t i = sidx(st, s, j, t);
          const bool ok = j >= bos && st.tmask[i];
          sx[wq] = st.pos[2 * i]; sy[wq] = st.pos[2 * i + 1]; sh[wq] = st.head[i]; sst[wq] = st.state[i];
          if (ok) ok_mask |= 1u << wq;
        }
      }
      cnt = __popc(ok_mask);
    }
    int tot;
    const int excl = block_excl_scan<BT>(cnt, scan, &tot, min(st.A_cap, BT));
    if (t == 0) { base_t = atomicAdd(a.t.total, tot); if (a.prof) atomicAdd(a.prof + 8, (unsigned long long)tot); }
    __syncthreads();
    if (t < st.A_cap) {
      int e = base_t + excl;
      a.t.off[row] = e;
      a.t.cnt[row] = cnt;
      if (cnt > 0) {
        const bool d_inv = stt[t] == INVALID;
#pragma unroll
        for (int wq = 0; wq < WMAX; ++wq) {
          if (!((ok_mask >> wq) & 1u)) continue;
          const int j = lo + wq;
          float dx = sx[wq] - px[t], dy = sy[wq] - py[t];
          float dth = wrap_angle(sh[wq] - hd[t]);
          const bool s_inv = sst[wq] == INVALID;
          if (s_inv && !d_inv) { dx = -MOTION_GAP; dy = -MOTION_GAP; dth = -HEADING_GAP; }
          if (!s_inv && d_inv) { dx = MOTION_GAP; dy = MOTION_GAP; }
          if (s_inv && d_inv) { dx = INVALID_MOTION; dy = INVALID_MOTION; dth = INVALID_HEAD; }
          if (e < a.t.cap) {
            a.t.src[e] = (j % st.ring) * rows_total + row;
            *reinterpret_cast<float4*>(a.t.raw + 4 * (size_t)e) =
                make_float4(norm2(dx, dy), angle_between(hc[t], hs[t], dx, dy), dth, (float)(j - c));
          }
          ++e;
        }
      }
    }
    __syncthreads();
  }

  if (part == 1) {
    const int ms = st.map_scene ? st.map_scene[s] : s;
    const int M = st.n_map[ms];
    const float r2 = a.r_map * a.r_map;
    const float* mp = st.map_pos + (size_t)ms * st.M_cap * 2;
    const int lane = lane_id();
    const bool map_in_lds = M <= a.map_lds;
    if (map_in_lds) {
      for (int m = t; m < M; m += BT) mxy[m] = *reinterpret_cast<const float2*>(mp + 2 * m);
      __syncthreads();
    }
    for (int ag = wave_id(); ag < st.A_cap; ag += BT / 64) {
      int found = 0;
      if (ag < A && im[ag]) {
        const float ax = px[ag], ay = py[ag];
        for (int m0 = 0; m0 < M && found < 5; m0 += 64) {
          const int m = m0 + lane;
          bool in = false;
          if (m < M) {
            const float2 mc = map_in_lds ? mxy[m] : *reinterpret_cast<const float2*>(mp + 2 * m);
            const float dx = ax - mc.x, dy = ay - mc.y;
            in = (dx * dx + dy * dy) < r2;
          }
// ... 839 lines not shown
```

### infgen_amd/csrc/kernels.h

```cpp
#pragma once
#include "tile.cuh"
#include "layout.h"
#include "../../include/infgen_hip.h"

namespace ig {

struct LinearArgs {
  const float* X; int ldx; const int* gather;
  int rows; int K; int Kp;
  const float* Wp; int Np; const float* bias; int N;
  const float* pre_g; const float* pre_b;
  const float* post_g; const float* post_b; int relu;
  float* Y; int ldy;
};

constexpr int LINEAR_MULTI_MAX = 6;
struct LinearMultiArgs { LinearArgs d[LINEAR_MULTI_MAX]; };

struct FourierArgs {
  const float* raw;
  int n;
  const int* count_dev;
  int e_cap;
  const float* pack;
// ... 18 lines not shown
#ifndef IG_FH_RING
#define IG_FH_RING ((IG_QSU || IG_FH_AP) ? 8 : 5)
#endif
constexpr int FH_WAVES = IG_FH_WAVES;
constexpr int FH_NT = 64 * FH_WAVES;
constexpr int FH_TILE = 16 * FH_WAVES;
constexpr int FH_RING = IG_FH_RING;
constexpr int FH_WG_PER_CU = FH_WAVES == 8 ? 1 : 2;
#ifndef IG_AH_RING4
#define IG_AH_RING4 3
#endif
#ifndef IG_AH_RING8
#define IG_AH_RING8 (IG_QSU ? 8 : 5)
#endif
struct FourierMultiArgs { FourierArgs set[4]; };

constexpr int R24_ROW_BYTES = 384;
constexpr int R24_LO_PLANE = 256;

struct EdgeSet {
  const int* off;
  const int* cnt;
  const int* src;
  const float* rhat;
};

struct AttnPreArgs {
  const float* X; int rows;
  const float* pack;
  int use_src_ln;
  float* Q;
  float* U;
  float* K; float* V;
};

struct EdgeAttnArgs {
  int rows;
  const float* Q; const float* U;
  const float* Ksrc; const float* Vsrc;
  EdgeSet es;
  float* AGG;
  float* Z;
  float* SIG;
  const float* wkr;
  const int* n_agents; int A_cap, margin;
  const int* row_mask;
};

struct EdgeFusedArgs {
  int rows;
  const float* Q;
  const float* pack;
  const float* Ksrc; const float* Vsrc;
  EdgeSet es;
  float* AGG;
  const int* groups; const int* n_groups;
  int dbg;
  int tiles_per_scene;
  int kv_once;
  int n_virtual;
  unsigned* dbgbuf;
  WarmArgs warm;
};

constexpr int LP_MAX_LAYERS = 8;
struct LayersPArgs {
  int rows, A_cap, num_layers;
  int xcd_order;
  int row0;
  int rows_per_wg;
  float* X;
  const float* attn_t[LP_MAX_LAYERS]; const float* attn_m[LP_MAX_LAYERS]; const float* attn_a[LP_MAX_LAYERS];
  float* ringK[LP_MAX_LAYERS]; float* ringV[LP_MAX_LAYERS];
  size_t slot_off;
  const float* mapK[LP_MAX_LAYERS]; const float* mapV[LP_MAX_LAYERS];
  float* Ka[2]; float* Va[2];
  EdgeSet et, em, ea;
  int* sync;
  unsigned spin_limit;
  unsigned long long* trace;
};

struct AttnPostArgs {
  float* X; int rows;
  const float* pack;
  const float* AGG; const float* Z; const float* SIG;
  int has_pos;
  const float* next_pack;
  float* nQ; float* nU; float* nK; float* nV;
};

struct AttnHArgs {
  float* X; int rows;
  const float* pack;
  const float* AGG; const float* Z; const float* SIG;
  int has_pos;
  const float* next_pack;
  int next_src_ln;
  float* nQ; float* nU; float* nK; float* nV;
  const int* groups; const int* n_groups;
  int dbg;
  WarmArgs warm;
};

struct ActiveGroupsArgs { const int* n_agents; int S, A_cap, margin; int* groups; int* n_groups; };

struct NearestArgs {
  const float* cx; const float* cy; const float* length; const float* width; const float* heading;
  const unsigned char* valid;
  int B, N, T, n_eval;
  float rounding;
  float* work;
  float* out;
};

struct KinematicArgs {
  const float* x; const float* y; const float* z; const float* heading;
  int n, T; float dt;
  float* speed; float* accel; float* yaw_rate; float* yaw_accel;
};
struct TtcArgs {
  const float* cx; const float* cy; const float* length; const float* width; const float* heading; const float* speed;
  const unsigned char* valid;
  const int* eval_idx;
  int B, N, T, n_eval;
  float* out;
};

struct TokenizeArgs {
  unsigned char* valid; float* pos; float* heading; float* velocity;
  const int* type; float* wl;
  const float* shape_in; float* shape_out;
  int A, T, shift, current_step;
  int invalid_state, valid_state, enter_state, exit_state, predict_state;
  int* token_index; const float* token_contour;
// ... 90 lines not shown
};
constexpr int HEADS_KS = 16;

constexpr int MAP_HEAD_N = 1024, MAP_TOPK = 10;
struct MapHeadArgs {
  const float* X; int ldx; const int* gather; int rows;
  const float* pack;
  float* logits;
  long long* top;
};
__global__ void k_heads_finish(const unsigned long long* part, int rows, int* next_token);

struct SceneState {
  int S, A_cap, T, M_cap, W;
  int ring;
  const int* n_agents;
  const int* n_map;
  const int* av_index;
  float* pos;
  float* head;
  int* state;
  int* token;
  int* grid;
  unsigned char* tmask;
  unsigned char* imask;
  unsigned char* catflag;
  const int* type;
  int* bos;
  const float* map_pos;
  const float* map_orient;
  const int* map_scene;
  const int* first_new;
  const float* hv_ovr;
};

struct EdgeBuf {
  int* off; int* cnt; int* src; float* raw; int* total; int cap;
};

struct RadiusEdgesArgs {
  int n_q;
  const int* q_node; const int* q_pt; const int* q_c0; const int* q_c1; const int* q_self; const int* q_pair_off;
  const float* p_pos; const float* p_head; const unsigned char* p_inv;
  const float* c_pos; const float* c_head; const unsigned char* c_inv; const unsigned char* c_ok; const int* c_src;
  const unsigned char* pair_ok;
  float radius; int K; int gap_rule; int index_diff;
  EdgeBuf e; int e_base;
};

struct MotionFeatArgs {
  const float* pos; const float* head; const int* state; const unsigned char* gap_mask;
  int rows, T;
  float* out;
};

struct BuildEdgesArgs {
  SceneState st;
  int c;
  int edgeless;
  float r_map, r_agent;
  int rows;
  EdgeBuf t, m, a;
  unsigned long long* prof;
  int map_lds;
  unsigned long long* clear_keys;
  int* clear_sync;
// ... 266 lines not shown
```

### infgen_amd/csrc/layer_kernels.hip

```cpp
#include "kernels.h"

namespace ig {

__global__ __launch_bounds__(NT, 2) void k_attn_pre(AttnPreArgs a);

__device__ __forceinline__ void pre_from_lds(const float* Xn, float* Qs, const float* P, int row0, int nvalid,
                                             float* Q, float* U, float* K, float* V, BHalf& cur) {
  const int n0 = 32 * wave_id();
  const int col = n0 + acc_col();
  const int lane = lane_id();
  {
    f32x16 acc = zero16();
    gemm128(acc, Xn, LDT, P + AL_WQ, 128, n0, cur, [&] { return b_load_half(P + AL_WK, 128, n0, 0); });
    const float bq = P[AL_BQ + col];
#pragma unroll
    for (int reg = 0; reg < 16; ++reg) {
      const int r = acc_row(reg);
      const float q = acc[reg] + bq;
      Qs[r * LDT + col] = q;
      if (Q && r < nvalid) Q[(size_t)(row0 + r) * D + col] = q;
    }
  }
  if (K) {
    f32x16 acc = zero16();
    gemm128(acc, Xn, LDT, P + AL_WK, 128, n0, cur, [&] { return b_load_half(P + AL_WV, 128, n0, 0); });
#pragma unroll
    for (int reg = 0; reg < 16; ++reg) {
      const int r = acc_row(reg);
      if (r < nvalid) K[(size_t)(row0 + r) * D + col] = acc[reg];
    }
    f32x16 accv = zero16();
    gemm128(accv, Xn, LDT, P + AL_WV, 128, n0, cur, [&] { return cur; });
    const float bv = P[AL_BV + col];
#pragma unroll
    for (int reg = 0; reg < 16; ++reg) {
      const int r = acc_row(reg);
      if (r < nvalid) V[(size_t)(row0 + r) * D + col] = accv[reg] + bv;
    }
  }
  if (U) {
    const float* bp = P + AL_WKR + ((size_t)(n0 + (lane & 31))) * 8 + 4 * (lane >> 5);
    float4 bu[H][2];
#pragma unroll
    for (int h = 0; h < H; ++h) {
      bu[h][0] = *reinterpret_cast<const float4*>(bp + h * (DH * D));
      bu[h][1] = *reinterpret_cast<const float4*>(bp + h * (DH * D) + 128 * 8);
    }
    __syncthreads();
    const float* ap = Qs + (lane & 31) * LDT + 4 * (lane >> 5);
#pragma unroll
    for (int h = 0; h < H; ++h) {
      f32x16 acc = zero16();
#pragma unroll
      for (int g = 0; g < 2; ++g) {
        const float4 a = *reinterpret_cast<const float4*>(ap + DH * h + 8 * g);
        const float4 b = bu[h][g];
        acc = __builtin_amdgcn_mfma_f32_32x32x2f32(a.x, b.x, acc, 0, 0, 0);
        acc = __builtin_amdgcn_mfma_f32_32x32x2f32(a.y, b.y, acc, 0, 0, 0);
        acc = __builtin_amdgcn_mfma_f32_32x32x2f32(a.z, b.z, acc, 0, 0, 0);
        acc = __builtin_amdgcn_mfma_f32_32x32x2f32(a.w, b.w, acc, 0, 0, 0);
      }
#pragma unroll
      for (int reg = 0; reg < 16; ++reg) {
        const int r = acc_row(reg);
        if (r < nvalid) U[(size_t)(row0 + r) * (H * D) + h * D + col] = acc[reg];
      }
    }
  }
}

// ... 75 lines not shown
    acc_to_lds(acco, B2, LDT, n0, P + AL_BO);
  }
  __syncthreads();
  x = seg_add(x, seg_layernorm(seg_load(B2 + srow * LDT), P + AL_LN_POST_G, P + AL_LN_POST_B, false));
  seg_store(B1 + srow * LDT, seg_layernorm(x, P + AL_LN_FFPRE_G, P + AL_LN_FFPRE_B, false));
  __syncthreads();
  f32x16 accf = zero16();
  const float* NP = a.next_pack;
#pragma unroll
  for (int cc = 0; cc < 4; ++cc) {
    const float* Wd = P + AL_W2 + (size_t)(16 * cc) * 128 * 8;
    f32x16 acch = zero16();
    gemm128(acch, B1, LDT, P + AL_W1, 512, 128 * cc + n0, cur, [&] { return b_load_half(Wd, 128, n0, 0); });
    {
      const int col = n0 + acc_col();
      const float b1 = P[AL_B1 + 128 * cc + col];
#pragma unroll
      for (int reg = 0; reg < 16; ++reg) B3[acc_row(reg) * LDT + col] = fmaxf(acch[reg] + b1, 0.f);
    }
    __syncthreads();
    gemm128(accf, B3, LDT, Wd, 128, n0, cur, [&] {
      return cc + 1 < 4 ? b_load_half(P + AL_W1, 512, 128 * (cc + 1) + n0, 0)
                        : (NP ? b_load_half(NP + AL_WQ, 128, n0, 0) : cur);
    });
    __syncthreads();
  }
  acc_to_lds(accf, B2, LDT, n0, P + AL_B2);
  __syncthreads();
  x = seg_add(x, seg_layernorm(seg_load(B2 + srow * LDT), P + AL_LN_FFPOST_G, P + AL_LN_FFPOST_B, false));
  seg_store(xrow, x);
  if (NP) {
    seg_store(B1 + srow * LDT, seg_layernorm(x, NP + AL_LN_DST_G, NP + AL_LN_DST_B, false));
    __syncthreads();
    pre_from_lds(B1, B3, NP, row0, nvalid, a.nQ, a.nU, a.nK, a.nV, cur);
  }
}

__global__ __launch_bounds__(NT, 2) void k_attn_pre(AttnPreArgs a) {
  __shared__ __attribute__((aligned(16))) float Xs[TR * LDT];
  __shared__ __attribute__((aligned(16))) float Qs[TR * LDT];
  const int row0 = blockIdx.x * TR;
  const int nvalid = min(TR, a.rows - row0);
  if (nvalid <= 0) return;
  const int n0 = 32 * wave_id();
  const int srow = seg_row();
  const float* g = a.pack + (a.use_src_ln ? AL_LN_SRC_G : AL_LN_DST_G);
  const float* b = a.pack + (a.use_src_ln ? AL_LN_SRC_B : AL_LN_DST_B);
  BHalf cur = b_load_half(a.pack + ((a.Q || a.U) ? AL_WQ : AL_WK), 128, n0, 0);
  seg_store(Xs + srow * LDT, seg_layernorm(seg_load(srow < nvalid ? a.X + (size_t)(row0 + srow) * D : nullptr), g, b, false));
  __syncthreads();
  if (a.Q || a.U) {
    pre_from_lds(Xs, Qs, a.pack, row0, nvalid, a.Q, a.U, a.K, a.V, cur);
  } else {
    const int col = n0 + acc_col();
    f32x16 acc = zero16();
    gemm128(acc, Xs, LDT, a.pack + AL_WK, 128, n0, cur, [&] { return b_load_half(a.pack + AL_WV, 128, n0, 0); });
#pragma unroll
    for (int reg = 0; reg < 16; ++reg) {
      const int r = acc_row(reg);
      if (r < nvalid && a.K) a.K[(size_t)(row0 + r) * D + col] = acc[reg];
    }
    f32x16 accv = zero16();
    gemm128(accv, Xs, LDT, a.pack + AL_WV, 128, n0, cur, [&] { return cur; });
    const float bv = a.pack[AL_BV + col];
#pragma unroll
    for (int reg = 0; reg < 16; ++reg) {
      const int r = acc_row(reg);
      if (r < nvalid && a.V) a.V[(size_t)(row0 + r) * D + col] = accv[reg] + bv;
    }
  }
}

__global__ __launch_bounds__(NT, 2) void k_heads(HeadsArgs a) {
  __shared__ __attribute__((aligned(16))) float Xs[TR * LDT];
  __shared__ __attribute__((aligned(16))) float Hs[TR * LDT];
  __shared__ float red_v[4][TR];
  __shared__ int red_i[4][TR];
  const int row0 = blockIdx.x * TR;
  const int nvalid = min(TR, a.rows - row0);
  if (nvalid <= 0) return;
  const int w = wave_id(), n0 = 32 * w, lane = lane_id();
  BHalf cur = b_load_half(a.tok_pack, 128, n0, 0);
  stage_rows_128(Xs, [&](int r) { return a.X + (size_t)(row0 + r) * D; }, nvalid);
  __syncthreads();
  {
    const float* P = a.tok_pack;
    f32x16 acc = zero16();
    const float* W3p = P + 16768;
    const int nchunk = a.token_size / 128, ns = a.nsplit > 1 ? a.nsplit : 1, sp = blockIdx.y;
    const int p0 = nchunk * sp / ns, p1 = nchunk * (sp + 1) / ns;
    gemm128(acc, Xs, LDT, P, 128, n0, cur, [&] { return b_load_half(W3p, a.token_size, 128 * p0 + n0, 0); });
    acc_to_lds(acc, Hs, LDT, n0, P + 16384);
    __syncthreads();
    ln_tile(Hs, LDT, Hs, LDT, P + 16512, P + 16640, true);
    __syncthreads();
    const float* W3 = P + 16768;
    const float* b3 = W3 + (size_t)128 * a.token_size;
    float bv[16];
    int bi[16];
#pragma unroll
    for (int reg = 0; reg < 16; ++reg) { bv[reg] = -INFINITY; bi[reg] = 0; }
// ... 81 lines not shown
```

### infgen_amd/csrc/layers_p.hip

```cpp
#include "kernels.h"
#include "layout.h"
#include "tile.cuh"
#include "split.cuh"
#include "attn_h.cuh"
#include "edge_attn.cuh"

#ifndef IG_LP_NOLOAD
#define IG_LP_NOLOAD 0
#endif
#ifndef IG_LP_NOMFMA
#define IG_LP_NOMFMA 0
#endif
#ifndef IG_LP_X32
#define IG_LP_X32 7
#endif
#ifndef IG_LP_SYNC1
#define IG_LP_SYNC1 1
#endif
#ifndef IG_LP_NOAUX
#define IG_LP_NOAUX 0
#endif
#ifndef IG_LP_NOSYNC
#define IG_LP_NOSYNC 0
#endif
// ... 153 lines not shown
    acc[s] = __builtin_amdgcn_mfma_f32_16x16x32_f16(f.h[s], __builtin_bit_cast(v8h, bh[s]), f32x4{0.f, 0.f, 0.f, 0.f}, 0, 0, 0);
#pragma unroll
  for (int s = 0; s < 4; ++s)
    acc[s] = __builtin_amdgcn_mfma_f32_16x16x32_f16(f.h[s], __builtin_bit_cast(v8h, bl[s]), acc[s], 0, 0, 0);
#pragma unroll
  for (int s = 0; s < 4; ++s)
    acc[s] = __builtin_amdgcn_mfma_f32_16x16x32_f16(f.l[s], __builtin_bit_cast(v8h, bh[s]), acc[s], 0, 0, 0);
  const f32x4 o = (acc[0] + acc[1]) + (acc[2] + acc[3]);
  __builtin_amdgcn_sched_barrier(0);
  return o;
}

}

template <bool R24, int ROWS>
__global__ __launch_bounds__(512, 1) void k_layers_p(LayersPArgs a) {
  __shared__ __attribute__((aligned(16))) float UZ[16 * LP_LDU];
  __shared__ __attribute__((aligned(16))) float AG[16 * LP_LDA];
  __shared__ __attribute__((aligned(16))) float SG[16 * H];
  __shared__ __attribute__((aligned(16))) float Vt[VT_SIZE + 4];
  __shared__ __attribute__((aligned(16))) uint4 FRx[512];
  __shared__ __attribute__((aligned(16))) uint4 FRp[2][512];
  __shared__ __attribute__((aligned(16))) float SCx[128], SCp[2][128], SCH[4][128];
  __shared__ __attribute__((aligned(16))) float2 STp[2][128];
  __shared__ __attribute__((aligned(16))) float2 MMp[2][128];
  __shared__ __attribute__((aligned(16))) float HM[128];
  uint4* FRH = reinterpret_cast<uint4*>(UZ);

  const int tid = threadIdx.x, lane = tid & 63, w = tid >> 6;
  const int j = lane & 15, rg = lane >> 4;
  constexpr int R = ROWS;
  const int gps = a.A_cap / R;
  const int L = a.num_layers;
  int grp = blockIdx.x;
  if (a.xcd_order) {
    const int per = 8 * gps, bq = grp / per, br = grp % per;
    grp = bq * per + (br % 8) * gps + br / 8;
  }
  const int r0 = a.row0 + R * grp, row = r0 + (j & (R - 1));
  const bool own_row = j < R;
  const int scene = r0 / a.A_cap;
  const int own = 16 * w + 4 * rg;
  int* ctr = a.sync + scene;
  int fp = 0, sp = 0;
  float inv_x = 1.0f;
  int n_trace = 0;
  auto STAMP = [&](int id) __attribute__((always_inline)) {
#if IG_LP_TRACE
    if (a.trace && blockIdx.x == 0 && tid == 0 && n_trace < 1020) {
      a.trace[2 * n_trace] = (unsigned long long)id; a.trace[2 * n_trace + 1] = __builtin_amdgcn_s_memtime(); ++n_trace;
    }
#endif
  };

  f32x4 x;
  { const float4 t = *reinterpret_cast<const float4*>(a.X + (size_t)row * D + own); x = f32x4{t.x, t.y, t.z, t.w}; }
  AFragP fa, fb, fc;

  auto table_fetch = [&](const float* P, const float* NP, float4& tv0, float4& tv1, int& o0, int& o1) __attribute__((always_inline)) {
    const int d0 = 4 * tid, d1 = 4 * (tid + 512);
    const float* anyp = P ? P : NP;
    const float* ts0 = attn_table_src(d0, P, NP, 0);
    const float* ts1 = d1 < VT_SIZE ? attn_table_src(d1, P, NP, 0) : nullptr;
    tv0 = *reinterpret_cast<const float4*>(ts0 ? ts0 : anyp);
    tv1 = *reinterpret_cast<const float4*>(ts1 ? ts1 : anyp);
    o0 = ts0 ? d0 : VT_SIZE;
// ... 4 lines not shown
  int el_cnt, el_off;
  auto edge_lists_request = [&](const EdgeSet& es) __attribute__((always_inline)) {
    el_cnt = es.cnt[r0 + (lane & (R - 1))];
    el_off = es.off[r0 + (lane & (R - 1))];
  };
  auto edge_lists_resolve = [&](const EdgeSet& es) __attribute__((always_inline)) {
    const int rl = lane & 15;
    const int off = el_off;
    const int cnt = rl < R ? el_cnt : -1;
    int rank = 0;
#pragma unroll
    for (int k = 0; k < 16; ++k) {
      const int ck = __shfl(cnt, k, 64);
      rank += (ck > cnt || (ck == cnt && k < rl)) ? 1 : 0;
    }
#pragma unroll
    for (int i = 0; i < (R == 16 ? 2 : 1); ++i) {
      const int want = R == 4 ? (w >> 1) : (i == 0 ? w : 15 - w);
      const unsigned long long m = __ballot(rank == want && lane < 16);
      const int r = __builtin_ctzll(m);
      eR[i] = r;
      int E = __builtin_amdgcn_readlane(cnt, r), B = __builtin_amdgcn_readlane(off, r);
      if constexpr (R == 4) {
        const int first = (E + 1) >> 1;
        B += (w & 1) ? first : 0;
        E = (w & 1) ? E - first : first;
      }
      eE[i] = E;
      eB[i] = B;
      eS[i] = es.src[B + max(min(lane, E - 1), 0)];
    }
  };

  auto node_pre = [&](const float* NP, float* nK, float* nV) __attribute__((always_inline)) {
    const unsigned short* pre = reinterpret_cast<const unsigned short*>(NP + AH_PRE);
    const float* hdr = Vt + VT_N_HDR;
    STAMP(16);
    publish_stats(x, STp[sp], w, lane);
    if (IG_LP_X32 & 2) publish_minmax(x, MMp[sp], w, lane);
    wg_barrier();
    STAMP(17);
    float mean, rstd;
    row_stats(STp[sp], j, mean, rstd);
    const f32x4 xn = ln_own(x, mean, rstd, Vt + VT_N_LN_G + own, Vt + VT_N_LN_B + own);
    if (IG_LP_X32 & 2) {
      const unsigned ebx = scale_bits(fmaf(row_dev(MMp[sp], j, mean) * rstd, hdr[12], hdr[13]));
      inv_x = scale_inv(ebx);
      publish_frag_common(xn, FRx, ebx, w, lane);
    } else {
      publish_frag(xn, FRx, SCx, w, lane);
    }
    sp ^= 1;
    wg_barrier();
    STAMP(18);
    f32x4 q = (IG_LP_X32 & 2) ? gemm32(fa, FRx, lane) * splat4(inv_x) : gemm_tiles(fa, FRx, SCx, lane);
    q = fma4(q, splat4(hdr[0]), lds4(Vt + VT_N_BQ + own));
    if (nK) {
      f32x4 kk = (IG_LP_X32 & 2) ? gemm32(fb, FRx, lane) * splat4(inv_x) : gemm_tiles(fb, FRx, SCx, lane);
      f32x4 vv = (IG_LP_X32 & 2) ? gemm32(fc, FRx, lane) * splat4(inv_x) : gemm_tiles(fc, FRx, SCx, lane);
      kk = kk * splat4(hdr[2]);
      vv = fma4(vv, splat4(hdr[3]), lds4(Vt + VT_N_BV + own));
      if (own_row && !IG_LP_NOKV) {
        *reinterpret_cast<float4*>(nK + (size_t)row * D + own) = make_float4(kk[0], kk[1], kk[2], kk[3]);
        *reinterpret_cast<float4*>(nV + (size_t)row * D + own) = make_float4(vv[0], vv[1], vv[2], vv[3]);
      }
    }
    STAMP(19);
    {
      const unsigned short* Wk = pre + (size_t)(4 + (w >> 1)) * QUARTER + (size_t)((w & 1) * 8) * 2 * 256 + lane * 4;
      v4h ah[8], al[8];
#pragma unroll
      for (int ct = 0; ct < 8; ++ct) {
#if IG_LP_NOAUX
        asm volatile("" : "=v"(ah[ct]), "=v"(al[ct]));
#else
        ah[ct] = *reinterpret_cast<const v4h*>(Wk + (ct * 2) * 256);
        al[ct] = *reinterpret_cast<const v4h*>(Wk + (ct * 2 + 1) * 256);
#endif
      }
      *reinterpret_cast<float4*>(AG + j * LP_LDA + own) = make_float4(q[0], q[1], q[2], q[3]);
      float m = fmaxf(fmaxf(fabsf(q[0]), fabsf(q[1])), fmaxf(fabsf(q[2]), fabsf(q[3])));
      m = xor_lanes_max(m);
      unsigned ebits = __float_as_uint(m) >> 23;
      ebits = min(max(ebits, 15u), 253u);
      const float sc = __uint_as_float((268u - ebits) << 23), inv = __uint_as_float((ebits - 14u) << 23);
      u32x2 qh, ql;
      {
        unsigned hi, lo;
        split_pair(q[0] * sc, q[1] * sc, hi, lo); qh[0] = hi; ql[0] = lo;
        split_pair(q[2] * sc, q[3] * sc, hi, lo); qh[1] = hi; ql[1] = lo;
      }
      const v4h vqh = __builtin_bit_cast(v4h, qh), vql = __builtin_bit_cast(v4h, ql);
      const float cq = inv * hdr[1];
      f32x4 acc[8];
#pragma unroll
      for (int ct = 0; ct < 8; ++ct) acc[ct] = __builtin_amdgcn_mfma_f32_16x16x16f16(ah[ct], vqh, f32x4{0.f, 0.f, 0.f, 0.f}, 0, 0, 0);
#pragma unroll
      for (int ct = 0; ct < 8; ++ct) acc[ct] = __builtin_amdgcn_mfma_f32_16x16x16f16(ah[ct], vql, acc[ct], 0, 0, 0);
#pragma unroll
      for (int ct = 0; ct < 8; ++ct) acc[ct] = __builtin_amdgcn_mfma_f32_16x16x16f16(al[ct], vqh, acc[ct], 0, 0, 0);
      float* urow = UZ + j * LP_LDU + w * D + 4 * rg;
#pragma unroll
      for (int ct = 0; ct < 8; ++ct)
        *reinterpret_cast<float4*>(urow + 16 * ct) = make_float4(acc[ct][0] * cq, acc[ct][1] * cq, acc[ct][2] * cq, acc[ct][3] * cq);
    }
  };

  auto sublayer = [&](const EdgeSet& es, const EdgeSet& es_next, const float* Ksrc, const float* Vsrc, bool kv_once, const float* P,
                      const float* NP, float* nK, float* nV) __attribute__((always_inline)) {
    const unsigned short* post = reinterpret_cast<const unsigned short*>(P + AH_POST);
    const unsigned short* pre_any = reinterpret_cast<const unsigned short*>((NP ? NP : P) + AH_PRE);
    float4 tv0, tv1; int to0, to1;
    table_fetch(P, NP, tv0, tv1, to0, to1);
    fa.load(post + 4 * QUARTER, w, lane);
    fb.load(post + 8 * QUARTER, w, lane);
    fc.load(post + 12 * QUARTER, w, lane);
    wg_barrier();
    STAMP(1);

    {
      const bool b3 = lane & 8;
      const unsigned lo8 = 8u * (unsigned)lane;
      auto ld8 = [&](const float* base, bool nt) {
        return ea_ld(reinterpret_cast<const float*>(reinterpret_cast<const char*>(base) + lo8), nt);
      };
      auto ld_r24 = [&](size_t e) {
        const char* rowp = reinterpret_cast<const char*>(es.rhat) + e * R24_ROW_BYTES;
        const unsigned hi = __builtin_nontemporal_load(reinterpret_cast<const unsigned*>(rowp + 4 * lane));
        const unsigned lo = __builtin_nontemporal_load(reinterpret_cast<const unsigned short*>(rowp + R24_LO_PLANE + 2 * lane));
        return pk2{__uint_as_float((hi << 16) | ((lo & 0xffu) << 8)), __uint_as_float((hi & 0xffff0000u) | (lo & 0xff00u))};
      };
      for (int ri = 0; ri < (R == 16 ? 2 : 1); ++ri) {
        const int rl = ri == 0 ? eR[0] : eR[1];
        const int E = IG_LP_NOEDGE ? 0 : (ri == 0 ? eE[0] : eE[1]);
        const int e_base = ri == 0 ? eB[0] : eB[1];
        int sv = ri == 0 ? eS[0] : eS[1];
        float* uz = UZ + rl * LP_LDU;
        EdgeAcc<true> acc;
        acc.q = *reinterpret_cast<const float2*>(AG + rl * LP_LDA + 2 * lane);
        acc.load_u(uz, lane);
        acc.reset();
        for (int c0 = 0; c0 < E; c0 += 64) {
          const int mc = min(64, E - c0);
          if (c0 > 0) sv = es.src[e_base + c0 + min(lane, mc - 1)];
          for (int i0 = 0; i0 < mc; i0 += LP_G) {
            pk2 kb[LP_G], vb[LP_G], rb[LP_G];
#pragma unroll
            for (int s = 0; s < LP_G; ++s) {
              const int ic = min(i0 + s, mc - 1);
              const int sj = __builtin_amdgcn_readlane(sv, ic);
              kb[s] = ld8(Ksrc + (size_t)sj * D, kv_once);
              vb[s] = ld8(Vsrc + (size_t)sj * D, kv_once);
              if constexpr (R24) rb[s] = ld_r24((size_t)(e_base + c0 + ic));
              else rb[s] = ld8(es.rhat + (size_t)(e_base + c0 + ic) * D, true);
            }
#pragma unroll
            for (int s = 0; s < LP_G; ++s) acc.step(kb[s], vb[s], rb[s], i0 + s < mc, b3);
          }
        }
        if constexpr (R == 4) {
          float* ps = UZ + (4 + 2 * (w >> 1)) * LP_LDU;
          if (w & 1) {
#pragma unroll
            for (int hd = 0; hd < H; ++hd) *reinterpret_cast<float2*>(ps + hd * D + 2 * lane) = make_float2(acc.zz[hd][0], acc.zz[hd][1]);
            *reinterpret_cast<float2*>(ps + LP_LDU + 2 * lane) = make_float2(acc.ag[0], acc.ag[1]);
            ps[LP_LDU + 128 + lane] = acc.m;
            ps[LP_LDU + 192 + lane] = acc.lsum;
          }
          wg_barrier();
          if (w & 1) continue;
          const float m1 = ps[LP_LDU + 128 + lane], l1 = ps[LP_LDU + 192 + lane];
          const float mm = fmaxf(acc.m, m1);
          const float s0 = acc.m == -INFINITY ? 0.f : __builtin_amdgcn_exp2f(acc.m - mm);
          const float s1 = m1 == -INFINITY ? 0.f : __builtin_amdgcn_exp2f(m1 - mm);
          acc.lsum = fmaf(l1, s1, acc.lsum * s0);
          const float2 a1 = *reinterpret_cast<const float2*>(ps + LP_LDU + 2 * lane);
          acc.ag = pk2{fmaf(a1.x, s1, acc.ag[0] * s0), fmaf(a1.y, s1, acc.ag[1] * s0)};
#pragma unroll
          for (int hd = 0; hd < H; ++hd) {
            const float h0 = readlane_f(s0, 8 * hd), h1 = readlane_f(s1, 8 * hd);
            const float2 z1 = *reinterpret_cast<const float2*>(ps + hd * D + 2 * lane);
            acc.zz[hd] = pk2{fmaf(z1.x, h1, acc.zz[hd][0] * h0), fmaf(z1.y, h1, acc.zz[hd][1] * h0)};
          }
        }
        const float inv = 1.0f / (acc.lsum + 1e-16f);
// ... 136 lines not shown
        if (rg == 0) HM[j * 8 + w] = mo;
        wg_barrier();
        const float4 hm0 = *reinterpret_cast<const float4*>(HM + j * 8), hm1 = *reinterpret_cast<const float4*>(HM + j * 8 + 4);
        const unsigned ebh = scale_bits(fmaxf(fmaxf(fmaxf(hm0.x, hm0.y), fmaxf(hm0.z, hm0.w)), fmaxf(fmaxf(hm1.x, hm1.y), fmaxf(hm1.z, hm1.w))));
        inv_h = scale_inv(ebh);
#pragma unroll
        for (int cc = 0; cc < 4; ++cc) publish_frag_common(hd4[cc], FRH + cc * 512, ebh, w, lane);
      }
      STAMP(12);
      wg_barrier();
      STAMP(13);
      f32x4 f = {0.f, 0.f, 0.f, 0.f};
#pragma unroll
      for (int cc = 0; cc < 4; ++cc) {
        f32x4 part;
        if (IG_LP_X32 & 4) part = (cc == 1 ? gemm32(fa, FRH + cc * 512, lane) : cc == 2 ? gemm32(fb, FRH + cc * 512, lane) : gemm32(fc, FRH + cc * 512, lane)) * splat4(inv_h);
        else part = cc == 1 ? gemm_tiles(fa, FRH + cc * 512, SCH[cc], lane) : cc == 2 ? gemm_tiles(fb, FRH + cc * 512, SCH[cc], lane)
                                                                                  : gemm_tiles(fc, FRH + cc * 512, SCH[cc], lane);
        if (cc == 0) fc.load(post + (size_t)48 * QUARTER, w, lane);
        if (cc == 1) fa.load(pre_any, w, lane);
        if (cc == 2) fb.load(pre_any + 8 * QUARTER, w, lane);
        if (cc == 3) fc.load(pre_any + 12 * QUARTER, w, lane);
        f = fma4(part, splat4(hdr[9]), f);
      }
      f = f + lds4(Vt + VT_B2 + own);
      STAMP(14);
      publish_stats(f, STp[sp], w, lane);
      wg_barrier();
      STAMP(15);
      float m2, r2;
      row_stats(STp[sp], j, m2, r2); sp ^= 1;
      x += ln_own(f, m2, r2, Vt + VT_LNO_G + own, Vt + VT_LNO_B + own);
    }
    if (NP) node_pre(NP, nK, nV);
    STAMP(20);
  };

  {
    float4 tv0, tv1; int to0, to1;
    table_fetch(nullptr, a.attn_t[0], tv0, tv1, to0, to1);
    const unsigned short* pre = reinterpret_cast<const unsigned short*>(a.attn_t[0] + AH_PRE);
    edge_lists_request(a.et);
    fa.load(pre, w, lane);
    fb.load(pre + 8 * QUARTER, w, lane);
    fc.load(pre + 12 * QUARTER, w, lane);
    edge_lists_resolve(a.et);
    *reinterpret_cast<float4*>(Vt + to0) = tv0;
    *reinterpret_cast<float4*>(Vt + to1) = tv1;
    wg_barrier();
    node_pre(a.attn_t[0], a.ringK[0] + a.slot_off, a.ringV[0] + a.slot_off);
  }
  for (int k = 0; k < 3 * L; ++k) {
    const int i = k / 3, kind = k - 3 * i;
    const bool last = k + 1 == 3 * L;
    float* Ka = a.Ka[i & 1];
    float* Va = a.Va[i & 1];
    const EdgeSet es = kind == 0 ? a.et : kind == 1 ? a.em : a.ea;
    const EdgeSet es_next = kind == 0 ? a.em : kind == 1 ? a.ea : a.et;
    const float* Ksrc = kind == 0 ? a.ringK[i] : kind == 1 ? a.mapK[i] : Ka;
    const float* Vsrc = kind == 0 ? a.ringV[i] : kind == 1 ? a.mapV[i] : Va;
    const float* P = kind == 0 ? a.attn_t[i] : kind == 1 ? a.attn_m[i] : a.attn_a[i];
    const float* NP = kind == 0 ? a.attn_m[i] : kind == 1 ? a.attn_a[i] : last ? nullptr : a.attn_t[i + 1];
    float* nK = kind == 0 ? nullptr : kind == 1 ? Ka : last ? nullptr : a.ringK[i + 1] + a.slot_off;
    float* nV = kind == 0 ? nullptr : kind == 1 ? Va : last ? nullptr : a.ringV[i + 1] + a.slot_off;
    STAMP(30 + kind);
    if (kind == 2 && !IG_LP_NOSYNC) {
#if IG_LP_SYNC1
      asm volatile("s_waitcnt vmcnt(0)" ::: "memory");
      __syncthreads();
      if (w == 0) {
        __builtin_amdgcn_fence(__ATOMIC_RELEASE, "agent");
        if (tid == 0) {
          __hip_atomic_fetch_add(ctr, 1, __ATOMIC_RELAXED, __HIP_MEMORY_SCOPE_AGENT);
          const int target = (i + 1) * gps;
          unsigned spins = 0;
          while (__hip_atomic_load(ctr, __ATOMIC_RELAXED, __HIP_MEMORY_SCOPE_AGENT) < target) {
            __builtin_amdgcn_s_sleep(2);
            if (a.spin_limit && ++spins > a.spin_limit) __builtin_trap();
          }
        }
        __builtin_amdgcn_fence(__ATOMIC_ACQUIRE, "agent");
      }
      __syncthreads();
#else
      __builtin_amdgcn_fence(__ATOMIC_RELEASE, "agent");
      __syncthreads();
      if (tid == 0) {
        __hip_atomic_fetch_add(ctr, 1, __ATOMIC_RELAXED, __HIP_MEMORY_SCOPE_AGENT);
        const int target = (i + 1) * gps;
        unsigned spins = 0;
        while (__hip_atomic_load(ctr, __ATOMIC_RELAXED, __HIP_MEMORY_SCOPE_AGENT) < target) {
          __builtin_amdgcn_s_sleep(2);
          if (a.spin_limit && ++spins > a.spin_limit) __builtin_trap();
        }
      }
      __syncthreads();
      __builtin_amdgcn_fence(__ATOMIC_ACQUIRE, "agent");
#endif
    }
    STAMP(0);
    sublayer(es, es_next, Ksrc, Vsrc, kind == 0, P, NP, nK, nV);
  }
  if (own_row) *reinterpret_cast<float4*>(a.X + (size_t)row * D + own) = make_float4(x[0], x[1], x[2], x[3]);
}

template __global__ void k_layers_p<true, 16>(LayersPArgs);
template __global__ void k_layers_p<false, 16>(LayersPArgs);
template __global__ void k_layers_p<true, 8>(LayersPArgs);
template __global__ void k_layers_p<false, 8>(LayersPArgs);
template __global__ void k_layers_p<true, 4>(LayersPArgs);
template __global__ void k_layers_p<false, 4>(LayersPArgs);

}
```

### infgen_amd/csrc/layout.h

```cpp
#pragma once

namespace ig {

enum AttnLayout : int {
  AL_LN_SRC_G = 0,
  AL_LN_SRC_B = AL_LN_SRC_G + 128,
  AL_LN_DST_G = AL_LN_SRC_B + 128,
  AL_LN_DST_B = AL_LN_DST_G + 128,
  AL_WQ = AL_LN_DST_B + 128,
  AL_BQ = AL_WQ + 16384,
  AL_WK = AL_BQ + 128,
  AL_WV = AL_WK + 16384,
  AL_BV = AL_WV + 16384,
  AL_WKR = AL_BV + 128,
  AL_WVR = AL_WKR + 16384,
  AL_BVR = AL_WVR + 16384,
  AL_WS = AL_BVR + 128,
  AL_BS = AL_WS + 16384,
  AL_WG = AL_BS + 128,
  AL_BG = AL_WG + 32768,
  AL_WO = AL_BG + 128,
  AL_BO = AL_WO + 16384,
  AL_LN_POST_G = AL_BO + 128,
  AL_LN_POST_B = AL_LN_POST_G + 128,
// ... 22 lines not shown
  FD_LN_B = FD_LN_G + 128,
  FD_W2 = FD_LN_B + 128,
  FD_SIZE = FD_W2 + 16384,
  FT_B2SUM = 0,
  FT_LN_G = 128,
  FT_LN_B = 256,
  FT_W3 = 384,
  FT_B3 = FT_W3 + 16384,
  FT_SIZE = FT_B3 + 128,
};
__host__ __device__ inline int fourier_pack_size_f32(int n) { return FE_DIM0 + n * FD_SIZE + FT_SIZE; }

enum FourierHLayout : int {
  FH_HDR = 0,
  FH_FREQ = 16,
  FH_DIM0 = FH_FREQ + 256,
  FHD_WX = 0,
  FHD_B1 = 128,
  FHD_G1 = 256,
  FHD_BE1 = 384,
  FHD_SIZE = 512,
  FH_TAIL = FH_DIM0 + 4 * FHD_SIZE,
  FHT_B2SUM = 0,
  FHT_G2 = 128,
  FHT_BE2 = 256,
  FHT_B3 = 384,
  FH_VEC_SIZE = FH_TAIL + 512,
  FH_HALF_MAT_FLOATS = 8192,
};
__host__ __device__ inline int fourier_pack_size(int n) {
  return fourier_pack_size_f32(n) + FH_VEC_SIZE + 2 * (2 * n + 1) * FH_HALF_MAT_FLOATS;
}

constexpr float AH_HDR_VERSION = 2.0f;

}
```

### infgen_amd/engine.py

```python
from __future__ import annotations

import ctypes as C
import hashlib
import os
from typing import Dict, List, Mapping, Optional, Sequence

import numpy as np
import torch

from . import _lib, logprob, packing, scene_setup
from .scene_setup import EVAL_SHAPE, INVALID_SHAPE
from .synth import INVALID, VALID, ENTER, EXIT, AGENT_SHAPE, RolloutConfig

D = 128
SEED_TYPE = 3


def _round_up(x: int, m: int) -> int:
    return (x + m - 1) // m * m


class LazyOut(dict):
    __slots__ = ('_lazy',)

# ... 287 lines not shown
    def mlp_layers(self, x, packs_nout):
        rows, n = x.shape[0], len(packs_nout)
        hid = torch.empty(n, rows, 128, device=self.device, dtype=torch.float32)
        outs = [torch.empty(rows, no, device=self.device, dtype=torch.float32) for _, no in packs_nout]
        d1, d2 = (_lib.LinearDesc * n)(), (_lib.LinearDesc * n)()
        o_b0, o_w3 = 128 * 128, 128 * 128 + 3 * 128
        for i, (pack, no) in enumerate(packs_nout):
            base = pack.data_ptr()
            a = d1[i]
            a.X, a.ldx, a.gather, a.rows, a.K = x.data_ptr(), x.stride(0), None, rows, 128
            a.Wp, a.Np, a.bias, a.N = base, 128, base + 4 * o_b0, 128
            a.pre_g = a.pre_b = None
            a.post_g, a.post_b, a.relu = base + 4 * (o_b0 + 128), base + 4 * (o_b0 + 256), 1
            a.Y, a.ldy = hid[i].data_ptr(), 128
            b = d2[i]
            npad = _round_up(no, 32)
            b.X, b.ldx, b.gather, b.rows, b.K = hid[i].data_ptr(), 128, None, rows, 128
            b.Wp, b.Np, b.bias, b.N = base + 4 * o_w3, npad, base + 4 * (o_w3 + 128 * npad), no
            b.pre_g = b.pre_b = b.post_g = b.post_b = None
            b.relu = 0
            b.Y, b.ldy = outs[i].data_ptr(), outs[i].stride(0)
        _lib.check(self.lib.infgen_linear_multi(d1, n, self.stream), 'infgen_linear_multi')
        _lib.check(self.lib.infgen_linear_multi(d2, n, self.stream), 'infgen_linear_multi')
        return outs

    def fourier(self, raw, n, pack, out, count_dev=None, rows=None, cat=None, normalize=False):
        rows = raw.shape[0] if rows is None else rows
        _lib.check(self.lib.infgen_fourier_embed(_lib.ptr(raw), n, _lib.ptr(count_dev), rows, _lib.ptr(pack),
                                                 _lib.ptr(cat), cat.stride(0) if cat is not None else 0,
                                                 out.data_ptr(), out.stride(0), int(normalize), self.stream),
                   'infgen_fourier_embed')
        return out

    def attn_pre(self, x, pack, use_src_ln=False, q=None, u=None, k=None, v=None, rows=None):
        rows = x.shape[0] if rows is None else rows
        _lib.check(self.lib.infgen_attn_pre(_lib.ptr(x), rows, _lib.ptr(pack), int(use_src_ln), _lib.ptr(q),
                                            _lib.ptr(u), _lib.ptr(k), _lib.ptr(v), self.stream), 'infgen_attn_pre')

    def edge_attn(self, rows, q, u, ksrc, vsrc, off, cnt, src, rhat, agg, z, sig, wide=None):
        args = (rows, _lib.ptr(q), _lib.ptr(u), _lib.ptr(ksrc), _lib.ptr(vsrc), _lib.ptr(off), _lib.ptr(cnt),
                _lib.ptr(src), _lib.ptr(rhat), _lib.ptr(agg), _lib.ptr(z), _lib.ptr(sig))
        if wide == 'fused':
            _lib.check(self.lib.infgen_edge_attn_fused(rows, _lib.ptr(q), _lib.ptr(u), *args[3:10], self.stream),
                       'infgen_edge_attn_fused')
        elif wide is None:
            _lib.check(self.lib.infgen_edge_attn(*args, self.stream), 'infgen_edge_attn')
        else:
            _lib.check(self.lib.infgen_edge_attn_mode(*args, int(wide), self.stream), 'infgen_edge_attn_mode')

    def attn_post(self, x, pack, agg, z, sig, has_pos=True, rows=None):
        rows = x.shape[0] if rows is None else rows
        _lib.check(self.lib.infgen_attn_post(_lib.ptr(x), rows, _lib.ptr(pack), _lib.ptr(agg), _lib.ptr(z),
                                             _lib.ptr(sig), int(has_pos), self.stream), 'infgen_attn_post')

    def attn_post_pre(self, x, pack, agg, z, sig, next_pack, has_pos=True, q=None, u=None, k=None, v=None):
        _lib.check(self.lib.infgen_attn_post_pre(_lib.ptr(x), x.shape[0], _lib.ptr(pack), _lib.ptr(agg), _lib.ptr(z),
                                                 _lib.ptr(sig), int(has_pos), _lib.ptr(next_pack), _lib.ptr(q), _lib.ptr(u),
                                                 _lib.ptr(k), _lib.ptr(v), self.stream), 'infgen_attn_post_pre')

    def attention_layer(self, x, pack, off, cnt, src, rhat, x_src=None, scratch=None, wide=None):
        rows = x.shape[0]
        dev = self.device
        sc = scratch if scratch is not None else {}
        q = sc.get('Q', torch.empty(rows, D, device=dev))
        u = sc.get('U', torch.empty(rows, 8 * D, device=dev))
        agg = sc.get('AGG', torch.empty(rows, D, device=dev))
        z = sc.get('Z', torch.empty(rows, 8 * D, device=dev))
        sig = sc.get('SIG', torch.empty(rows, 8, device=dev))
        fused = wide == 'fused'
        if x_src is None:
# ... 199 lines not shown
        self.G = int(grid.shape[0])
        self.teacher_token = self.teacher_state = None
        self.teacher_grid = self.teacher_pos = self.teacher_head = None
        if teacher is not None:
            tt = np.full((S, T, A_cap), -1, np.int32); ts = np.zeros((S, T, A_cap), np.int32)
            tg = np.full((S, T, A_cap), -2, np.int32)
            tp, th = None, None
            for s, tch in enumerate(teacher):
                tok_s, st_s = tch[0], tch[1]
                A = min(np.asarray(tok_s).shape[0], A_cap)
                tt[s, :, :A] = np.asarray(tok_s)[:A].T; ts[s, :, :A] = np.asarray(st_s)[:A].T
                if len(tch) > 2 and tch[2] is not None:
                    tg[s, :, :A] = np.asarray(tch[2])[:A].T
                if len(tch) > 4 and tch[3] is not None:
                    if tp is None:
                        tp, th = np.zeros((S, T, A_cap, 2), np.float32), np.zeros((S, T, A_cap), np.float32)
                    tp[s, :, :A] = np.asarray(tch[3], np.float32)[:A].transpose(1, 0, 2); th[s, :, :A] = np.asarray(tch[4], np.float32)[:A].T
            self.teacher_token, self.teacher_state = t(tt), t(ts)
            if (tg > -2).any():
                self.teacher_grid = t(tg)
            if tp is not None:
                self.teacher_pos, self.teacher_head = t(tp), t(th)
        self.replay_row = None
        self._replay_pose = None
        if replay is not None and teacher is not None:
            raise ValueError('teacher= forces every row; replay= forces the flagged rows: give one of them')

        f = lambda *shape: torch.zeros(*shape, device=dev, dtype=torch.float32)
        i32 = lambda *shape: torch.zeros(*shape, device=dev, dtype=torch.int32)
        L = cfg.num_agent_layers
        self.X, self.Q, self.U = f(rows, D), f(rows, D), f(rows, 8 * D)
        if self._tap_layers:
            self.tap_x = f(cfg.num_agent_layers, rows, D)
        self.Ka, self.Va, self.AGG, self.Z, self.SIG = f(rows, D), f(rows, D), f(rows, D), f(rows, 8 * D), f(rows, 8)
        self.ringK = [f(self.ring, rows, D) for _ in range(L)]
        self.ringV = [f(self.ring, rows, D) for _ in range(L)]
        self.mapK = [f(self.S0 * M_cap, D) for _ in range(L)]
        self.mapV = [f(self.S0 * M_cap, D) for _ in range(L)]
        self.edges = {}
        totals = i32(3)
        for k, (name, cap) in enumerate((('t', rows * self.W), ('m', rows * 5), ('a', rows * (A_cap - 1)))):
            cap = max(cap, 32)
            self.edges[name] = dict(off=i32(rows), cnt=i32(rows), src=i32(cap), raw=f(cap, 4), rhat=f(cap, D),
                                    total=totals[k:k + 1], cap=cap)
        self.raw2, self.cat, self.fus_in = f(rows, 4), f(rows, D), f(rows, 4 * D)
        self.tmp1, self.tmp2 = f(rows, D), f(rows, D)
        self.next_token, self.next_state = i32(rows), i32(rows)
        steps = cfg.num_decode_steps
        self.logits = f(steps, rows, cfg.token_size) if store_logits else None
        self.pred_traj, self.pred_head, self.pred_state = f(S, A_cap, R, 2), f(S, A_cap, R), f(S, A_cap, R)
        self.sample_u = self.logits_scratch = None
        if self.sample_k > 1:
            assert sample_uniforms is not None, 'top-k sampling needs caller-supplied uniforms'
            self.sample_u = torch.from_numpy(self._uniform_rows(sample_uniforms, amax)).to(dev)
        self.token_logprob = f(steps, rows) if token_logprob else None
        self.sample_logprob = f(steps, rows) if sample_logprob else None
        self._rollout_lp = self._rollout_slp = None
        self.tok_tab = self.grid_tab = self.cat_agent = self.cat_seed = None
        self.x_pt = None
        self._ctx = None
        self._init = None
        self.ins = None
        self._mg = None
        self._mg_checked = False
        self._map_nbr_cap = 40
        self._prologue_done = False
        self._decoded_rows = torch.zeros((), device=dev, dtype=torch.int64)
        self._ing = None
        if batch is not None:
            self._ingest(batch, batch_layout, replay=replay)
        elif replay is not None:
# ... 406 lines not shown
                                                               _lib.ptr(g['V']), _lib.ptr(g['off']), _lib.ptr(g['cnt']),
                                                               _lib.ptr(g['src']), g['rhat'].data_ptr(), _lib.ptr(g['AGG']),
                                                               ops.stream), 'infgen_edge_attn_fused_r24')
            else:
                ops.edge_attn(mrows, g['Q'], w.attn_pt[i], g['K'], g['V'], g['off'], g['cnt'], g['src'], g['rhat'],
                              g['AGG'], None, None, wide='fused')
            if i + 1 < cfg.num_map_layers:
                ops.attn_post_pre(x_pt, w.attn_pt[i], g['AGG'], None, None, w.attn_pt[i + 1], has_pos=False,
                                  q=g['Q'], k=g['K'], v=g['V'])
            else:
                ops.attn_post(x_pt, w.attn_pt[i], g['AGG'], None, None, has_pos=False)
        if map_only:
            return
        self._finish_prologue()

    def map_token_head(self, rows: torch.Tensor):
        with _lib.thread_options(self._effective_options()):
            return self.ops.map_token_head(self.x_pt, rows.to(self.device, torch.int32).contiguous(), self.w.map_head)

    def _prologue_with_given_map(self):
        S0, M_cap, dev = self.S0, self.M_cap, self.device
        if self.x_pt is None:
            self.x_pt = torch.zeros(S0 * M_cap, D, device=dev)
        assert len(self._x_pt_override) == S0, 'one x_pt per distinct scene'
        for s, xp in enumerate(self._x_pt_override):
            M = self.hosts[s * self.copies]['M']
            self.x_pt[s * M_cap:s * M_cap + M] = xp.detach().to(dev, torch.float32)
        self._finish_prologue()

    def _finish_prologue(self):
        ops, w, cfg = self.ops, self.w, self.cfg
        x_pt = self.x_pt
        for i in range(cfg.num_agent_layers):
            ops.attn_pre(x_pt, w.attn_m[i], use_src_ln=True, k=self.mapK[i], v=self.mapV[i])

        if self.insertion:
            self._alloc_insertion()
            for i in range(3):
                ops.attn_pre(x_pt, w.attn_pt2sa[i], use_src_ln=True, k=self.ins['mapK'][i], v=self.ins['mapV'][i])
        if self._ctx is None:
            self._build_ctx()
        self._refresh_opts()
        self._decoded_rows.zero_()
        st = ops.stream
        _lib.check(self.lib.infgen_raw_feature(C.byref(self._ctx), 0, st), 'raw_feature(0)')
        _lib.check(self.lib.infgen_decode_layers(C.byref(self._ctx), 0, 1, st), 'decode_layers(0)')
        _lib.check(self.lib.infgen_raw_feature(C.byref(self._ctx), 1, st), 'raw_feature(1)')
        self._prologue_done = True

    def rollout(self):
        self._bc_host = None
        if (self._graph_all and not self.insertion and self._x_pt_override is None and self._mg_checked and self._init is not None
                and self._ctx is not None and not _lib.prof_active()):
            self._rollout_graph()
            return
        self.prologue()
        self.run()

    def _rollout_graph(self):
        cur = torch.cuda.current_stream(self.device)
        if getattr(self, '_gstream', None) is None:
            self._gstream = torch.cuda.Stream(device=self.device)
        gs = self._gstream
        gs.wait_stream(cur)
        with torch.cuda.stream(gs):
            self._refresh_opts(groups=True)
            snap = bytes(self._ctx.opts)[:_lib.OPTIONS_VALUE_BYTES] + bytes([self._ctx.four_t_dt is not None])
# ... 133 lines not shown
            nr_host = hd[1][ins_idx_host].astype(np.int64)
            for s_i, r_i in zip(ins_idx_host, nr_host):
                I['inserted_rows'][int(s_i)].append((int(r_i), t))
            if self.seed_out is not None:
                ops, w = self.ops, self.w
                ins = torch.from_numpy(ins_idx_host.astype(np.int64)).to(self.device)
                so, slot = self.seed_out, I['n_new'][ins].long()
                XS_in = I['XS'][:S][ins].contiguous()
                so['state'][ins, slot, t] = torch.softmax(I['lg_state'][ins], dim=-1)[:, -1]
                if 'pos' in so:
                    so['pos'][ins, slot, t] = torch.softmax(I['lg_pos'][ins], dim=-1)
                    so['occ_a'][ins, slot, t] = ops.mlp_layer(XS_in, w.fwd_heads['grid_agent_occ_head'], D, self.G)
                    so['occ_p'][ins, slot, t] = ops.mlp_layer(XS_in, w.fwd_heads['grid_pt_occ_head'], D, self.G)
                    so['occ_gt'][ins, slot, t] = I['occ'][ins]
            _lib.check(lib.infgen_insert_heading(ctx, blk, t, int(h_ready), int(riders_h and h_ready), self.ops.stream), 'infgen_insert_heading')
            h_ready = True
            riders = riders_h = True

    def _build_ctx(self):
        cfg, w = self.cfg, self.w
        c = _lib.Rollout()
        c.S, c.A_cap, c.T, c.M_cap, c.W, c.ring, c.R = self.S, self.A_cap, self.T, self.M_cap, self.W, self.ring, self.R
        c.token_size, c.grid_size, c.num_layers = cfg.token_size, self.G, cfg.num_agent_layers
        c.force_valid, c.store_logits = int(self.force_valid), int(self.store_logits)
        c.no_grid_token, c.no_state_token = int(not cfg.use_grid_token), int(not cfg.use_state_token)
        c.r_map, c.r_agent = float(cfg.pl2a_radius), float(cfg.a2a_radius)
        P = _lib.ptr
        c.n_agents, c.n_map, c.av_index = P(self.n_agents), P(self.n_map), P(self.av)
        c.pos, c.head, c.state, c.token, c.grid = P(self.pos), P(self.head), P(self.state), P(self.token), P(self.gridtok)
        c.tmask, c.imask, c.catflag, c.type, c.bos = P(self.tmask), P(self.imask), P(self.catflag), P(self.atype), P(self.bos)
        c.map_pos, c.map_orient = P(self.map_pos), P(self.map_orient)
        c.map_scene = P(self.map_scene)
        c.tap_x = P(self.tap_x)
        for i in range(cfg.num_agent_layers):
            c.attn_t[i], c.attn_m[i], c.attn_a[i] = P(w.attn_t[i]), P(w.attn_m[i]), P(w.attn_a[i])
            c.ringK[i], c.ringV[i], c.mapK[i], c.mapV[i] = P(self.ringK[i]), P(self.ringV[i]), P(self.mapK[i]), P(self.mapV[i])
        c.four_t, c.four_m, c.four_a, c.four_xa = P(w.four_t), P(w.four_m), P(w.four_a), P(w.four_xa)
        c.fusion_pack, c.tok_head_pack, c.st_head_pack = P(w.fusion), P(w.tok_head), P(w.st_head)
        c.tok_tab, c.grid_tab, c.state_emb = P(self.tok_tab), P(self.grid_tab), P(w.state_a_emb)
        c.cat_agent, c.cat_seed, c.vocab, c.grid_xy = P(self.cat_agent), P(self.cat_seed), P(self.vocab), P(self.grid_xy)
        c.X, c.Q, c.U, c.Ka, c.Va, c.AGG, c.Z, c.SIG = (P(self.X), P(self.Q), P(self.U), P(self.Ka), P(self.Va),
                                                          P(self.AGG), P(self.Z), P(self.SIG))
        for name, field in (('t', 'et'), ('m', 'em'), ('a', 'ea')):
            e, b = self.edges[name], getattr(c, field)
            b.off, b.cnt, b.src, b.raw, b.rhat, b.total, b.cap = (P(e['off']), P(e['cnt']), P(e['src']), P(e['raw']),
                                                                   P(e['rhat']), P(e['total']), e['cap'])
        c.raw2, c.cat, c.fus_in, c.tmp1, c.tmp2 = P(self.raw2), P(self.cat), P(self.fus_in), P(self.tmp1), P(self.tmp2)
        c.next_token, c.next_state, c.logits = P(self.next_token), P(self.next_state), P(self.logits)
        c.teacher_token, c.teacher_state = P(self.teacher_token), P(self.teacher_state)
        c.teacher_grid = P(self.teacher_grid)
        c.teacher_pos, c.teacher_head = P(self.teacher_pos), P(self.teacher_head)
        c.replay_row = P(self.replay_row)
        c.pred_traj, c.pred_head, c.pred_state = P(self.pred_traj), P(self.pred_head), P(self.pred_state)
        if self.insertion:
            c.first_new, c.hv_ovr = P(self.ins['first_new']), P(self.ins['hv_ovr'])
        c.sample_k, c.sample_u, c.logits_scratch = self.sample_k, P(self.sample_u), P(self.logits_scratch)
        c.token_logprob = P(self.token_logprob)
        c.sample_logprob = P(self.sample_logprob)
        self._ctx = c
        self._refresh_opts()
        _lib.check(self.lib.infgen_rollout_validate(C.byref(c)), 'infgen_rollout_validate')

    def _refresh_opts(self, groups: bool = False):
        o = self._ctx.opts
        _lib.check(self.lib.infgen_get_options(C.byref(o)), 'infgen_get_options')
        for k, v in (self.options or {}).items():
            setattr(o, k, int(v))
        o.use = 1
        if (int(o.gemm_terms) == 2) != (self.w.operand_bits == 8):
            raise ValueError(f'gemm_terms = {int(o.gemm_terms)} with packs of {self.w.operand_bits}-bit operands: the bf16 mode '
                             '(gemm_terms = 2) takes PackedWeights(..., operand_bits=8), every other mode operand_bits=11')
        self._ctx.four_t_dt = None
        if o.fourier_mode != 0 and self.flags['dt_table']:
            self._ctx.four_t_dt = _lib.ptr(self.w.time_gap_table(self.lib, int(o.gemm_terms), self.ops.stream))
# ... 411 lines not shown
```

Baseline: 29.50 million.

## Interleave K/V rows and store the temporal ring row-major for gather locality

Stores K and V for each source row side by side in one buffer (pitch 2*D) and lays out the temporal ring as row-major (row*ring+slot), so edge-attention gathers pull K and V for a source from adjacent memory. New _kv entry points and a stride/pitch parameter run through the pre/post, edge and persistent kernels, with both options on by default through env knobs. This is meant to cut scattered global loads and cache-line waste in the edge gather. In exchange it adds pitch shifts, an overflow check on the ring size, and a wide ABI change to the option and rollout structs.

New measurement: 29.62 million (median of 6 runs). No clear change (+0.4%).

```diff
diff --git a/include/infgen_hip.h b/include/infgen_hip.h
--- a/include/infgen_hip.h
+++ b/include/infgen_hip.h
@@ -50,6 +50,8 @@
   int layers_p;
   int rhat_format;
   int edge_kernel;
+  int kv_interleave;
+  int ring_row_major;
   int _pad0;
   const int* row_groups; const int* n_row_groups;
 } InfgenOptions;
@@ -89,6 +91,7 @@
   const unsigned char* replay_row;
   const int* map_scene;
   float* tap_x;
+  int kv_pitch; int ring_row_major;
   float* sample_logprob;
   float* token_logprob;
   int no_grid_token; int no_state_token;
@@ -142,6 +145,16 @@
 int infgen_edge_attn_mode(int rows, const float* Q, const float* U, const float* Ksrc, const float* Vsrc,
                           const int* off, const int* cnt, const int* src, const float* rhat,
                           float* AGG, float* Z, float* SIG, int wide, void* stream);
+int infgen_attn_pre_kv(const float* X, int rows, const float* pack, int use_src_ln,
+                       float* Q, float* U, float* K, float* V, int kv_stride, void* stream);
+int infgen_attn_post_pre_kv(float* X, int rows, const float* pack, const float* AGG, const float* Z, const float* SIG,
+                            int has_pos, const float* next_pack, float* nQ, float* nU, float* nK, float* nV, int kv_stride, void* stream);
+int infgen_edge_attn_fused_kv(int rows, const float* Q, const float* pack, const float* Ksrc, const float* Vsrc, int kv_pitch,
+                              const int* off, const int* cnt, const int* src, const float* rhat, float* AGG, void* stream);
+int infgen_edge_attn_kv(int rows, const float* Q, const float* U, const float* Ksrc, const float* Vsrc, int kv_pitch,
+                        const int* off, const int* cnt, const int* src, const float* rhat,
+                        float* AGG, float* Z, float* SIG, int wide, void* stream);
+long long infgen_ring_row_index(int row, int slot, int rows, int ring, int row_major);
 int infgen_attn_post(float* X, int rows, const float* pack, const float* AGG, const float* Z, const float* SIG,
                      int has_pos, void* stream);
 int infgen_attn_post_pre(float* X, int rows, const float* pack, const float* AGG, const float* Z, const float* SIG,
diff --git a/infgen_amd/_lib.py b/infgen_amd/_lib.py
--- a/infgen_amd/_lib.py
+++ b/infgen_amd/_lib.py
@@ -57,10 +57,11 @@
 
 class Options(C.Structure):
     _fields_ = [('use', _i), ('attn_mode', _i), ('gemm_terms', _i), ('fourier_mode', _i), ('edge_fuse', _i), ('edge_loop', _i),
-                ('overlap', _i), ('row_group_margin', _i), ('layers_p', _i), ('rhat_format', _i), ('edge_kernel', _i), ('_pad0', _i), ('row_groups', _p), ('n_row_groups', _p)]
-
-
-OPTIONS_VALUE_BYTES = C.sizeof(_i) * 12
+                ('overlap', _i), ('row_group_margin', _i), ('layers_p', _i), ('rhat_format', _i), ('edge_kernel', _i), ('kv_interleave', _i),
+                ('ring_row_major', _i), ('_pad0', _i), ('row_groups', _p), ('n_row_groups', _p)]
+
+
+OPTIONS_VALUE_BYTES = C.sizeof(_i) * 14
 
 
 class Rollout(C.Structure):
@@ -93,6 +94,7 @@
         ('replay_row', _p),
         ('map_scene', _p),
         ('tap_x', _p),
+        ('kv_pitch', _i), ('ring_row_major', _i),
         ('sample_logprob', _p),
         ('token_logprob', _p),
         ('no_grid_token', _i), ('no_state_token', _i),
@@ -162,6 +164,11 @@
     'infgen_match_map_tokens': (_i, [_p, _p, _p, _i, _i, _p, _p]),
     'infgen_match_agent_tokens': (_i, [_p, _p, _p, _p, _p, _p, C.c_longlong, _i, _i, _i, _i, _p, _p, _p]),
     'infgen_attn_pre': (_i, [_p, _i, _p, _i, _p, _p, _p, _p, _p]),
+    'infgen_attn_pre_kv': (_i, [_p, _i, _p, _i, _p, _p, _p, _p, _i, _p]),
+    'infgen_attn_post_pre_kv': (_i, [_p, _i, _p, _p, _p, _p, _i, _p, _p, _p, _p, _p, _i, _p]),
+    'infgen_edge_attn_fused_kv': (_i, [_i, _p, _p, _p, _p, _i, _p, _p, _p, _p, _p, _p]),
+    'infgen_edge_attn_kv': (_i, [_i, _p, _p, _p, _p, _i, _p, _p, _p, _p, _p, _p, _p, _i, _p]),
+    'infgen_ring_row_index': (C.c_longlong, [_i, _i, _i, _i, _i]),
     'infgen_edge_attn': (_i, [_i, _p, _p, _p, _p, _p, _p, _p, _p, _p, _p, _p, _p]),
     'infgen_edge_attn_mode': (_i, [_i, _p, _p, _p, _p, _p, _p, _p, _p, _p, _p, _p, _i, _p]),
     'infgen_attn_post': (_i, [_p, _i, _p, _p, _p, _p, _i, _p]),
@@ -250,10 +257,21 @@
         raise InfgenHipError(f'{what} failed ({rc}): {msg.decode() if msg else "?"}')
 
 
+def ring_row_index(row: int, slot: int, rows: int, ring: int, row_major: int) -> int:
+    return row * ring + slot if row_major else slot * rows + row
+
+
 def ptr(t) -> Optional[int]:
     if t is None:
         return None
     assert t.is_contiguous(), 'tensor must be contiguous'
+    return t.data_ptr()
+
+
+def ptr_rows(t) -> Optional[int]:
+    if t is None:
+        return None
+    assert t.dim() == 2 and t.stride(1) == 1, 'rows must be contiguous'
     return t.data_ptr()
 
 
diff --git a/infgen_amd/csrc/api.hip b/infgen_amd/csrc/api.hip
--- a/infgen_amd/csrc/api.hip
+++ b/infgen_amd/csrc/api.hip
@@ -39,6 +39,8 @@
 }
 namespace knob {
 const int layers_p = env_layers_p();
+const int kv_interleave = env_int("INFGEN_KV_INTERLEAVE", 1) != 0;
+const int ring_row_major = env_int("INFGEN_RING_ROW_MAJOR", 1) != 0;
 const int qs_dbg = env_int("INFGEN_QS_DBG", 0);
 const int fh12_min = env_int("INFGEN_FH12_MIN", 150000);
 const int fh12_multi_rows = env_int("INFGEN_FH12_MULTI_ROWS", 0);
@@ -66,7 +68,8 @@
 
 namespace {
 InfgenOptions g_def = {0,  2,  3,  1,  1,  6,  0,
-                        0,  knob::layers_p,  0,  1, 0, nullptr, nullptr};
+                        0,  knob::layers_p,  0,  1,  knob::kv_interleave,
+                        knob::ring_row_major, 0, nullptr, nullptr};
 int g_def_group_rows = 0;
 const int* g_def_limit_n_agents = nullptr;
 int g_def_limit_A_cap = 0;
@@ -485,24 +488,41 @@
 }
 static double heads_macs(int rows, int token_size) { return (double)rows * (2 * 16384.0 + 128.0 * token_size + 384.0); }
 
-extern "C" int infgen_attn_pre(const float* X, int rows, const float* pack, int use_src_ln,
-                               float* Q, float* U, float* K, float* V, void* stream) {
+static int attn_pre_impl(const float* X, int rows, const float* pack, int use_src_ln,
+                         float* Q, float* U, float* K, float* V, int kv_stride, void* stream) {
   if (rows <= 0) return 0;
   { ProfScope _ps(INFGEN_KID_ATTN_PRE, stream, attn_pre_macs(rows, Q, U, K, V));
     if (attn_kind(rows)) {
-      launch_attn_h(AttnHArgs{const_cast<float*>(X), rows, nullptr, nullptr, nullptr, nullptr, 0, pack, use_src_ln, Q, U, K, V}, stream);
+      AttnHArgs h{const_cast<float*>(X), rows, nullptr, nullptr, nullptr, nullptr, 0, pack, use_src_ln, Q, U, K, V};
+      h.kv_stride = kv_stride;
+      launch_attn_h(h, stream);
     } else {
-      AttnPreArgs a{X, rows, pack, use_src_ln, Q, U, K, V};
+      AttnPreArgs a{X, rows, pack, use_src_ln, Q, U, K, V, kv_stride};
       hipLaunchKernelGGL(k_attn_pre, dim3(ceil_div(rows, TR)), dim3(NT), 0, (hipStream_t)stream, a);
     } }
   return check_launch("infgen_attn_pre");
 }
+extern "C" int infgen_attn_pre(const float* X, int rows, const float* pack, int use_src_ln,
+                               float* Q, float* U, float* K, float* V, void* stream) {
+  return attn_pre_impl(X, rows, pack, use_src_ln, Q, U, K, V, 0, stream);
+}
+static int kv_stride_ok(const char* where, int v) {
+  return v < 0 || v % 4 ? fail(where, "the K/V row stride must be a non-negative multiple of 4 floats (0: 128)") : 0;
+}
+static int kv_pitch_ok(const char* where, int v) {
+  return v < 0 || (v && (v < 128 || (v & (v - 1)))) ? fail(where, "the K/V row pitch must be 0 (128) or a power of two >= 128 floats") : 0;
+}
+extern "C" int infgen_attn_pre_kv(const float* X, int rows, const float* pack, int use_src_ln,
+                                  float* Q, float* U, float* K, float* V, int kv_stride, void* stream) {
+  RET_IF(kv_stride_ok("infgen_attn_pre_kv", kv_stride));
+  return attn_pre_impl(X, rows, pack, use_src_ln, Q, U, K, V, kv_stride, stream);
+}
 
 static int edge_attn_impl(int rows, const float* Q, const float* U, const float* Ksrc, const float* Vsrc,
                           const int* off, const int* cnt, const int* src, const float* rhat,
-                          float* AGG, float* Z, float* SIG, int wide, void* stream, const int* row_mask = nullptr) {
+                          float* AGG, float* Z, float* SIG, int wide, void* stream, const int* row_mask = nullptr, int kv_pitch = 0) {
   if (rows <= 0) return 0;
-  EdgeAttnArgs a{rows, Q, U, Ksrc, Vsrc, EdgeSet{off, cnt, src, rhat}, AGG, Z, SIG, nullptr, nullptr, 0, 0, wide ? row_mask : nullptr};
+  EdgeAttnArgs a{rows, Q, U, Ksrc, Vsrc, EdgeSet{off, cnt, src, rhat}, AGG, Z, SIG, nullptr, nullptr, 0, 0, wide ? row_mask : nullptr, kv_pitch};
   if (limit_n_agents() && O().row_groups && rows == group_rows() && !wide) {
     a.n_agents = limit_n_agents(); a.A_cap = limit_A_cap(); a.margin = O().row_group_margin;
   }
@@ -543,7 +563,7 @@
 }
 
 static int edge_fused_launch(int rows, const float* Q, const float* pack, const float* Ksrc, const float* Vsrc, const EdgeSet& es,
-                             float* AGG, int rows_per_scene, int kv_once, void* stream, int r24 = 0) {
+                             float* AGG, int rows_per_scene, int kv_once, void* stream, int r24 = 0, int kv_pitch = 0) {
   if (rows <= 0) return 0;
   if (!pack || !es.rhat) return fail("infgen_edge_attn_fused", "needs the layer pack and rhat");
   const int dbg = knob::edge_dbg, no_xcd = knob::edge_noxcd, small_max = knob::edge_small, wg2 = knob::edge_wg2;
@@ -552,6 +572,7 @@
   const bool two = !small && wg2 && G == 6;
   const int tr = (small || two) ? 16 : 32;
   EdgeFusedArgs a{rows, Q, pack, Ksrc, Vsrc, es, AGG, nullptr, nullptr, dbg, 0, kv_once};
+  a.kv_pitch = kv_pitch;
   int grid = ceil_div(rows, tr);
   if (O().row_groups && rows == group_rows()) { a.groups = O().row_groups; a.n_groups = O().n_row_groups; }
   else if (rows_per_scene > tr && rows_per_scene % tr == 0 && !(no_xcd & 1)) {
@@ -607,6 +628,17 @@
                                       float* AGG, void* stream) {
   return edge_fused_launch(rows, Q, pack, Ksrc, Vsrc, EdgeSet{off, cnt, src, rhat}, AGG, 0, 0, stream);
 }
+extern "C" int infgen_edge_attn_fused_kv(int rows, const float* Q, const float* pack, const float* Ksrc, const float* Vsrc, int kv_pitch,
+                                         const int* off, const int* cnt, const int* src, const float* rhat, float* AGG, void* stream) {
+  RET_IF(kv_pitch_ok("infgen_edge_attn_fused_kv", kv_pitch));
+  return edge_fused_launch(rows, Q, pack, Ksrc, Vsrc, EdgeSet{off, cnt, src, rhat}, AGG, 0, 0, stream, 0, kv_pitch);
+}
+extern "C" int infgen_edge_attn_kv(int rows, const float* Q, const float* U, const float* Ksrc, const float* Vsrc, int kv_pitch,
+                                   const int* off, const int* cnt, const int* src, const float* rhat,
+                                   float* AGG, float* Z, float* SIG, int wide, void* stream) {
+  RET_IF(kv_pitch_ok("infgen_edge_attn_kv", kv_pitch));
+  return edge_attn_impl(rows, Q, U, Ksrc, Vsrc, off, cnt, src, rhat, AGG, Z, SIG, wide, stream, nullptr, kv_pitch);
+}
 
 extern "C" int infgen_fourier_embed_r24(const float* raw, int n, const int* count_dev, int e_cap, const float* pack, void* out,
                                         void* stream) {
@@ -632,13 +664,15 @@
 }
 
 static int attn_post_fused(float* X, int rows, const float* pack, const float* AGG, const float* Z, const float* SIG,
-                           int has_pos, const float* next_pack, float* nQ, float* nU, float* nK, float* nV, void* stream) {
+                           int has_pos, const float* next_pack, float* nQ, float* nU, float* nK, float* nV, void* stream, int kv_stride = 0) {
   if (rows <= 0) return 0;
   { ProfScope _ps(INFGEN_KID_ATTN_POST, stream, attn_post_macs(rows, has_pos, next_pack, nQ, nU, nK, nV));
     if (attn_kind(rows)) {
-      launch_attn_h(AttnHArgs{X, rows, pack, AGG, Z, SIG, has_pos, next_pack, 0, nQ, nU, nK, nV}, stream);
+      AttnHArgs h{X, rows, pack, AGG, Z, SIG, has_pos, next_pack, 0, nQ, nU, nK, nV};
+      h.kv_stride = kv_stride;
+      launch_attn_h(h, stream);
     } else {
-      AttnPostArgs a{X, rows, pack, AGG, Z, SIG, has_pos, next_pack, nQ, nU, nK, nV};
+      AttnPostArgs a{X, rows, pack, AGG, Z, SIG, has_pos, next_pack, nQ, nU, nK, nV, kv_stride};
       hipLaunchKernelGGL(k_attn_post, dim3(ceil_div(rows, TR)), dim3(NT), 0, (hipStream_t)stream, a);
     } }
   return check_launch("infgen_attn_post");
@@ -653,6 +687,15 @@
                                     const float* SIG, int has_pos, const float* next_pack, float* nQ, float* nU,
                                     float* nK, float* nV, void* stream) {
   return attn_post_fused(X, rows, pack, AGG, Z, SIG, has_pos, next_pack, nQ, nU, nK, nV, stream);
+}
+extern "C" int infgen_attn_post_pre_kv(float* X, int rows, const float* pack, const float* AGG, const float* Z,
+                                       const float* SIG, int has_pos, const float* next_pack, float* nQ, float* nU,
+                                       float* nK, float* nV, int kv_stride, void* stream) {
+  RET_IF(kv_stride_ok("infgen_attn_post_pre_kv", kv_stride));
+  return attn_post_fused(X, rows, pack, AGG, Z, SIG, has_pos, next_pack, nQ, nU, nK, nV, stream, kv_stride);
+}
+extern "C" long long infgen_ring_row_index(int row, int slot, int rows, int ring, int row_major) {
+  return ring_row_index(row, slot, rows, ring, row_major);
 }
 
 extern "C" int infgen_match_agent_tokens(const unsigned char* valid, const float* pos, const float* heading, const float* shape,
@@ -1098,7 +1141,7 @@
 
 static SceneState scene_of(const InfgenRollout* r) {
   SceneState st;
-  st.S = r->S; st.A_cap = r->A_cap; st.T = r->T; st.M_cap = r->M_cap; st.W = r->W; st.ring = r->ring;
+  st.S = r->S; st.A_cap = r->A_cap; st.T = r->T; st.M_cap = r->M_cap; st.W = r->W; st.ring = r->ring; st.ring_row_major = r->ring_row_major;
   st.n_agents = r->n_agents; st.n_map = r->n_map; st.av_index = r->av_index;
   st.pos = r->pos; st.head = r->head; st.state = r->state; st.token = r->token; st.grid = r->grid;
   st.tmask = r->tmask; st.imask = r->imask; st.catflag = r->catflag; st.type = r->type; st.bos = r->bos;
@@ -1115,6 +1158,9 @@
   if (r->A_cap % 32) return fail(where, "A_cap must be a multiple of 32");
   if (r->num_layers <= 0 || r->num_layers > INFGEN_MAX_LAYERS) return fail(where, "bad num_layers");
   if (r->ring <= r->W) return fail(where, "ring must exceed the temporal window");
+  RET_IF(kv_pitch_ok(where, r->kv_pitch));
+  if (r->ring_row_major & ~1) return fail(where, "ring_row_major must be 0 or 1");
+  if ((long long)r->S * r->A_cap * r->ring > 0x7fffffffLL) return fail(where, "ring rows exceed the 32-bit source index of the temporal edges");
   if (r->W > 16) return fail(where, "temporal window larger than 16 columns is not supported");
   if ((r->no_grid_token | r->no_state_token) & ~1) return fail(where, "no_grid_token / no_state_token must be 0 or 1");
   if (r->token_logprob && !(r->store_logits && r->logits) && !r->logits_scratch) {
@@ -1432,8 +1478,10 @@
     a.attn_t[i] = r->attn_t[i]; a.attn_m[i] = r->attn_m[i]; a.attn_a[i] = r->attn_a[i];
     a.ringK[i] = r->ringK[i]; a.ringV[i] = r->ringV[i]; a.mapK[i] = r->mapK[i]; a.mapV[i] = r->mapV[i];
   }
-  a.slot_off = (size_t)(c % r->ring) * rows * D;
-  a.Ka[0] = r->Ka; a.Va[0] = r->Va; a.Ka[1] = r->U; a.Va[1] = r->U + (size_t)rows * D;
+  a.kv_pitch = r->kv_pitch;
+  a.slot_off = (size_t)ring_store_offset(c % r->ring, rows, r->ring, r->ring_row_major, r->kv_pitch);
+  a.ring_stride = ring_row_stride(r->ring, r->ring_row_major, r->kv_pitch);
+  a.Ka[0] = r->Ka; a.Va[0] = r->Va; a.Ka[1] = r->U; a.Va[1] = r->U + (kv_pitch_of(r->kv_pitch) >= 2 * D ? (size_t)D : (size_t)rows * D);
   a.et = eset(r->et); a.em = eset(r->em); a.ea = eset(r->ea);
   a.sync = reinterpret_cast<int*>(r->SIG);
   a.trace = nullptr;
@@ -1515,7 +1563,9 @@
     if (rc != LP_REFUSED) return rc;
   }
   const bool overlap = sm.overlap, fuse = sm.fuse; const int r24 = sm.r24;
-  const size_t slot = (size_t)(c % r->ring) * rows * D;
+  const int kvp = r->kv_pitch;
+  const size_t slot = (size_t)ring_store_offset(c % r->ring, rows, r->ring, r->ring_row_major, kvp);
+  const int kvs = ring_row_stride(r->ring, r->ring_row_major, kvp);
   const int L = r->num_layers;
   float* U = fuse ? nullptr : r->U;
   const float* Z = fuse ? nullptr : r->Z;
@@ -1529,10 +1579,11 @@
     if (skip_edges) return 0;
     if (fuse && O().attn_mode != 0)
       warm_request(pack + AH_POST + 4 * (QB / 4), 48 * QB, next_pack ? next_pack + AH_PRE : nullptr, 16 * QB);
-    return fuse ? edge_fused_launch(rows, r->Q, pack, Ks, Vs, eset(e), r->AGG, r->A_cap, kv_once, stream, fmt < 0 ? r24 : fmt)
-                : infgen_edge_attn(rows, r->Q, r->U, Ks, Vs, e.off, e.cnt, e.src, e.rhat, r->AGG, r->Z, r->SIG, stream);
+    return fuse ? edge_fused_launch(rows, r->Q, pack, Ks, Vs, eset(e), r->AGG, r->A_cap, kv_once, stream, fmt < 0 ? r24 : fmt, kvp)
+                : edge_attn_impl(rows, r->Q, r->U, Ks, Vs, e.off, e.cnt, e.src, e.rhat, r->AGG, r->Z, r->SIG, rows <= 256 ? 1 : 0, stream,
+                                 nullptr, kvp);
   };
-  RET_IF(infgen_attn_pre(r->X, rows, r->attn_t[0], 0, r->Q, U, r->ringK[0] + slot, r->ringV[0] + slot, stream));
+  RET_IF(attn_pre_impl(r->X, rows, r->attn_t[0], 0, r->Q, U, r->ringK[0] + slot, r->ringV[0] + slot, kvs, stream));
   auto warm_post = [&](const float* pack) { if (fuse && O().attn_mode != 0) warm_request(pack + AH_POST, 52 * QB, nullptr, 0); };
   for (int i = 0; i < L; ++i) {
     RET_IF(edge(r->attn_t[i], r->ringK[i], r->ringV[i], r->et, 1, r->attn_m[i]));
@@ -1543,15 +1594,15 @@
       return fail("infgen_decode_layers", "join failed");
     RET_IF(edge(r->attn_m[i], r->mapK[i], r->mapV[i], r->em, 0, r->attn_a[i]));
     warm_post(r->attn_a[i]);
-    RET_IF(infgen_attn_post_pre(r->X, rows, r->attn_m[i], r->AGG, Z, SIG, has_pos, r->attn_a[i], r->Q, U,
-                                r->Ka, r->Va, stream));
+    RET_IF(attn_post_fused(r->X, rows, r->attn_m[i], r->AGG, Z, SIG, has_pos, r->attn_a[i], r->Q, U,
+                           r->Ka, r->Va, stream, kvp));
     if (overlap && i == 0 && hipStreamWaitEvent((hipStream_t)stream, g_ev_a, 0) != hipSuccess)
       return fail("infgen_decode_layers", "join failed");
     RET_IF(edge(r->attn_a[i], r->Ka, r->Va, r->ea, 0, i + 1 < L ? r->attn_t[i + 1] : nullptr, sm.ra));
     if (i + 1 < L) {
       warm_post(r->attn_t[i + 1]);
-      RET_IF(infgen_attn_post_pre(r->X, rows, r->attn_a[i], r->AGG, Z, SIG, has_pos, r->attn_t[i + 1], r->Q, U,
-                                  r->ringK[i + 1] + slot, r->ringV[i + 1] + slot, stream));
+      RET_IF(attn_post_fused(r->X, rows, r->attn_a[i], r->AGG, Z, SIG, has_pos, r->attn_t[i + 1], r->Q, U,
+                             r->ringK[i + 1] + slot, r->ringV[i + 1] + slot, stream, kvs));
     } else {
       RET_IF(infgen_attn_post(r->X, rows, r->attn_a[i], r->AGG, Z, SIG, has_pos, stream));
     }
@@ -1881,8 +1932,8 @@
   if (riders) RET_IF(gather_rows(r->X, I->pend_row, I->pend_mask, S, rows, I->XS + (size_t)S * D, stream));
   RET_IF(infgen_attn_pre(I->XS, R, r->attn_m[0], 0, I->QS, I->US, nullptr, nullptr, stream));
   for (int i = 0; i < 3; ++i) {
-    RET_IF(infgen_edge_attn(S, I->QS, I->US, r->mapK[i], r->mapV[i], I->em_h.off, I->em_h.cnt, I->em_h.src, I->em_h.rhat, I->AGGS, I->ZS,
-                            I->SIGS, stream));
+    RET_IF(edge_attn_impl(S, I->QS, I->US, r->mapK[i], r->mapV[i], I->em_h.off, I->em_h.cnt, I->em_h.src, I->em_h.rhat, I->AGGS, I->ZS,
+                          I->SIGS, S <= 256 ? 1 : 0, stream, nullptr, r->kv_pitch));
     RET_IF(infgen_attn_post_pre(I->XS, R, r->attn_m[i], I->AGGS, I->ZS, I->SIGS, 1, r->attn_a[i], I->QS, I->US, riders ? I->KN : nullptr,
                                 riders ? I->VN : nullptr, stream));
     if (riders) {
diff --git a/infgen_amd/csrc/attn_h.hip b/infgen_amd/csrc/attn_h.hip
--- a/infgen_amd/csrc/attn_h.hip
+++ b/infgen_amd/csrc/attn_h.hip
@@ -237,15 +237,16 @@
         }
       }
       if (need_kv) {
+        const size_t kvs = (size_t)kv_pitch_of(a.kv_stride);
         f32x4 kk[8];
         zero_acc(kk);
         gemm_unit(kk, Bh, Bl);
         scale_bias(kk, inv_n * hdr[2], nullptr, rg);
-        store_row(valid ? a.nK + (size_t)row * D : nullptr, kk, rg);
+        store_row(valid ? a.nK + (size_t)row * kvs : nullptr, kk, rg);
         zero_acc(kk);
         gemm_unit(kk, Bh, Bl);
         scale_bias(kk, inv_n * hdr[3], Vt + VT_N_BV, rg);
-        store_row(valid && a.nV ? a.nV + (size_t)row * D : nullptr, kk, rg);
+        store_row(valid && a.nV ? a.nV + (size_t)row * kvs : nullptr, kk, rg);
       }
     }
   }
diff --git a/infgen_amd/csrc/attn_hs.hip b/infgen_amd/csrc/attn_hs.hip
--- a/infgen_amd/csrc/attn_hs.hip
+++ b/infgen_amd/csrc/attn_hs.hip
@@ -261,8 +261,9 @@
       kk = kk * splat4(inv_n * hdr[2]);
       vv = fma4(vv, splat4(inv_n * hdr[3]), lds4(Vt + VT_N_BV + own));
       if (valid) {
-        *reinterpret_cast<float4*>(a.nK + (size_t)row * D + own) = make_float4(kk[0], kk[1], kk[2], kk[3]);
-        if (a.nV) *reinterpret_cast<float4*>(a.nV + (size_t)row * D + own) = make_float4(vv[0], vv[1], vv[2], vv[3]);
+        const size_t kvs = (size_t)kv_pitch_of(a.kv_stride);
+        *reinterpret_cast<float4*>(a.nK + (size_t)row * kvs + own) = make_float4(kk[0], kk[1], kk[2], kk[3]);
+        if (a.nV) *reinterpret_cast<float4*>(a.nV + (size_t)row * kvs + own) = make_float4(vv[0], vv[1], vv[2], vv[3]);
       }
     }
   }
diff --git a/infgen_amd/csrc/edge_attn.cuh b/infgen_amd/csrc/edge_attn.cuh
--- a/infgen_amd/csrc/edge_attn.cuh
+++ b/infgen_amd/csrc/edge_attn.cuh
@@ -141,6 +141,7 @@
                                                 int e_step, AttnState& st, const float* u_lds = nullptr, bool kv_once = false) {
   const int lane = lane_id();
   const bool b3 = lane & 8;
+  const int kvsh = __builtin_amdgcn_readfirstlane(kv_shift_of(a.kv_pitch));
   EdgeAcc<HASR> acc;
   acc.q = *reinterpret_cast<const float2*>(a.Q + (size_t)row * D + 2 * lane);
   if constexpr (ULDS) acc.load_u(u_lds, lane);
@@ -157,8 +158,8 @@
         const int ic = min(i0 + s, mc - 1);
         const int sj = __builtin_amdgcn_readlane(srcv, ic);
         const size_t e = (size_t)(e_base + e_first + (c0 + ic) * e_step);
-        kb[s] = ea_ld(a.Ksrc + (size_t)sj * D + 2 * lane, kv_once);
-        vb[s] = ea_ld(a.Vsrc + (size_t)sj * D + 2 * lane, kv_once);
+        kb[s] = ea_ld(a.Ksrc + ((size_t)sj << kvsh) + 2 * lane, kv_once);
+        vb[s] = ea_ld(a.Vsrc + ((size_t)sj << kvsh) + 2 * lane, kv_once);
         if constexpr (HASR) rb[s] = __builtin_nontemporal_load(reinterpret_cast<const pk2*>(a.es.rhat + e * D + 2 * lane));
       }
 #pragma unroll
diff --git a/infgen_amd/csrc/edge_fused.hip b/infgen_amd/csrc/edge_fused.hip
--- a/infgen_amd/csrc/edge_fused.hip
+++ b/infgen_amd/csrc/edge_fused.hip
@@ -119,6 +119,7 @@
   {
     const bool b3 = lane & 8;
     const bool kv_once = a.kv_once != 0;
+    const int kvsh = __builtin_amdgcn_readfirstlane(kv_shift_of(a.kv_pitch));
     const unsigned lo8 = 8u * (unsigned)lane;
     auto ld8 = [&](const float* base, bool nt) {
       return ea_ld(reinterpret_cast<const float*>(reinterpret_cast<const char*>(base) + lo8), nt);
@@ -155,8 +156,8 @@
           for (int s = 0; s < G; ++s) {
             const int ic = min(i0 + s, mc - 1);
             const int sj = __builtin_amdgcn_readlane(sv, ic);
-            kb[s] = ld8(a.Ksrc + (size_t)sj * D, kv_once);
-            vb[s] = ld8(a.Vsrc + (size_t)sj * D, kv_once);
+            kb[s] = ld8(a.Ksrc + ((size_t)sj << kvsh), kv_once);
+            vb[s] = ld8(a.Vsrc + ((size_t)sj << kvsh), kv_once);
             if constexpr (R24) rb[s] = ld_r24((size_t)(e_base + c0 + ic));
             else rb[s] = ld8(a.es.rhat + (size_t)(e_base + c0 + ic) * D, true);
           }
diff --git a/infgen_amd/csrc/edge_fused3.hip b/infgen_amd/csrc/edge_fused3.hip
--- a/infgen_amd/csrc/edge_fused3.hip
+++ b/infgen_amd/csrc/edge_fused3.hip
@@ -101,6 +101,7 @@
   {
     const int eh = lane >> 3, ei = lane & 7;
     const bool kv_once = a.kv_once != 0;
+    const int kvsh = __builtin_amdgcn_readfirstlane(kv_shift_of(a.kv_pitch));
     const unsigned lo8 = 8u * (unsigned)lane;
     auto ld8 = [&](const float* base, bool nt) {
       return ea_ld(reinterpret_cast<const float*>(reinterpret_cast<const char*>(base) + lo8), nt);
@@ -150,8 +151,8 @@
           for (int s = 0; s < G; ++s) {
             const int ic = min(i0 + s, mc - 1);
             const int sj = __builtin_amdgcn_readlane(sv, ic);
-            kb[s] = ld8(a.Ksrc + (size_t)sj * D, kv_once);
-            vb[s] = ld8(a.Vsrc + (size_t)sj * D, kv_once);
+            kb[s] = ld8(a.Ksrc + ((size_t)sj << kvsh), kv_once);
+            vb[s] = ld8(a.Vsrc + ((size_t)sj << kvsh), kv_once);
           }
           asm volatile("s_waitcnt vmcnt(%0)" :: "n"(2 * G) : "memory");
           {
diff --git a/infgen_amd/csrc/edge_kernels.hip b/infgen_amd/csrc/edge_kernels.hip
--- a/infgen_amd/csrc/edge_kernels.hip
+++ b/infgen_amd/csrc/edge_kernels.hip
@@ -176,7 +176,7 @@
           if (!s_inv && d_inv) { dx = MOTION_GAP; dy = MOTION_GAP; }
           if (s_inv && d_inv) { dx = INVALID_MOTION; dy = INVALID_MOTION; dth = INVALID_HEAD; }
           if (e < a.t.cap) {
-            a.t.src[e] = (j % st.ring) * rows_total + row;
+            a.t.src[e] = (int)ring_row_index(row, j % st.ring, rows_total, st.ring, st.ring_row_major);
             *reinterpret_cast<float4*>(a.t.raw + 4 * (size_t)e) =
                 make_float4(norm2(dx, dy), angle_between(hc[t], hs[t], dx, dy), dth, (float)(j - c));
           }
diff --git a/infgen_amd/csrc/kernels.h b/infgen_amd/csrc/kernels.h
--- a/infgen_amd/csrc/kernels.h
+++ b/infgen_amd/csrc/kernels.h
@@ -74,6 +74,7 @@
   float* Q;
   float* U;
   float* K; float* V;
+  int kv_stride;
 };
 
 struct EdgeAttnArgs {
@@ -87,6 +88,7 @@
   const float* wkr;
   const int* n_agents; int A_cap, margin;
   const int* row_mask;
+  int kv_pitch;
 };
 
 struct EdgeFusedArgs {
@@ -103,6 +105,7 @@
   int n_virtual;
   unsigned* dbgbuf;
   WarmArgs warm;
+  int kv_pitch;
 };
 
 constexpr int LP_MAX_LAYERS = 8;
@@ -115,6 +118,8 @@
   const float* attn_t[LP_MAX_LAYERS]; const float* attn_m[LP_MAX_LAYERS]; const float* attn_a[LP_MAX_LAYERS];
   float* ringK[LP_MAX_LAYERS]; float* ringV[LP_MAX_LAYERS];
   size_t slot_off;
+  int kv_pitch;
+  int ring_stride;
   const float* mapK[LP_MAX_LAYERS]; const float* mapV[LP_MAX_LAYERS];
   float* Ka[2]; float* Va[2];
   EdgeSet et, em, ea;
@@ -130,6 +135,7 @@
   int has_pos;
   const float* next_pack;
   float* nQ; float* nU; float* nK; float* nV;
+  int kv_stride;
 };
 
 struct AttnHArgs {
@@ -143,6 +149,7 @@
   const int* groups; const int* n_groups;
   int dbg;
   WarmArgs warm;
+  int kv_stride;
 };
 
 struct ActiveGroupsArgs { const int* n_agents; int S, A_cap, margin; int* groups; int* n_groups; };
@@ -299,6 +306,7 @@
   const int* map_scene;
   const int* first_new;
   const float* hv_ovr;
+  int ring_row_major;
 };
 
 struct EdgeBuf {
diff --git a/infgen_amd/csrc/layer_kernels.hip b/infgen_amd/csrc/layer_kernels.hip
--- a/infgen_amd/csrc/layer_kernels.hip
+++ b/infgen_amd/csrc/layer_kernels.hip
@@ -5,7 +5,8 @@
 __global__ __launch_bounds__(NT, 2) void k_attn_pre(AttnPreArgs a);
 
 __device__ __forceinline__ void pre_from_lds(const float* Xn, float* Qs, const float* P, int row0, int nvalid,
-                                             float* Q, float* U, float* K, float* V, BHalf& cur) {
+                                             float* Q, float* U, float* K, float* V, int kv_stride, BHalf& cur) {
+  const size_t kvs = (size_t)kv_pitch_of(kv_stride);
   const int n0 = 32 * wave_id();
   const int col = n0 + acc_col();
   const int lane = lane_id();
@@ -27,7 +28,7 @@
 #pragma unroll
     for (int reg = 0; reg < 16; ++reg) {
       const int r = acc_row(reg);
-      if (r < nvalid) K[(size_t)(row0 + r) * D + col] = acc[reg];
+      if (r < nvalid) K[(size_t)(row0 + r) * kvs + col] = acc[reg];
     }
     f32x16 accv = zero16();
     gemm128(accv, Xn, LDT, P + AL_WV, 128, n0, cur, [&] { return cur; });
@@ -35,7 +36,7 @@
 #pragma unroll
     for (int reg = 0; reg < 16; ++reg) {
       const int r = acc_row(reg);
-      if (r < nvalid) V[(size_t)(row0 + r) * D + col] = accv[reg] + bv;
+      if (r < nvalid) V[(size_t)(row0 + r) * kvs + col] = accv[reg] + bv;
     }
   }
   if (U) {
@@ -177,7 +178,7 @@
   if (NP) {
     seg_store(B1 + srow * LDT, seg_layernorm(x, NP + AL_LN_DST_G, NP + AL_LN_DST_B, false));
     __syncthreads();
-    pre_from_lds(B1, B3, NP, row0, nvalid, a.nQ, a.nU, a.nK, a.nV, cur);
+    pre_from_lds(B1, B3, NP, row0, nvalid, a.nQ, a.nU, a.nK, a.nV, a.kv_stride, cur);
   }
 }
 
@@ -195,7 +196,7 @@
   seg_store(Xs + srow * LDT, seg_layernorm(seg_load(srow < nvalid ? a.X + (size_t)(row0 + srow) * D : nullptr), g, b, false));
   __syncthreads();
   if (a.Q || a.U) {
-    pre_from_lds(Xs, Qs, a.pack, row0, nvalid, a.Q, a.U, a.K, a.V, cur);
+    pre_from_lds(Xs, Qs, a.pack, row0, nvalid, a.Q, a.U, a.K, a.V, a.kv_stride, cur);
   } else {
     const int col = n0 + acc_col();
     f32x16 acc = zero16();
@@ -203,7 +204,7 @@
 #pragma unroll
     for (int reg = 0; reg < 16; ++reg) {
       const int r = acc_row(reg);
-      if (r < nvalid && a.K) a.K[(size_t)(row0 + r) * D + col] = acc[reg];
+      if (r < nvalid && a.K) a.K[(size_t)(row0 + r) * kv_pitch_of(a.kv_stride) + col] = acc[reg];
     }
     f32x16 accv = zero16();
     gemm128(accv, Xs, LDT, a.pack + AL_WV, 128, n0, cur, [&] { return cur; });
@@ -211,7 +212,7 @@
 #pragma unroll
     for (int reg = 0; reg < 16; ++reg) {
       const int r = acc_row(reg);
-      if (r < nvalid && a.V) a.V[(size_t)(row0 + r) * D + col] = accv[reg] + bv;
+      if (r < nvalid && a.V) a.V[(size_t)(row0 + r) * kv_pitch_of(a.kv_stride) + col] = accv[reg] + bv;
     }
   }
 }
diff --git a/infgen_amd/csrc/layers_p.hip b/infgen_amd/csrc/layers_p.hip
--- a/infgen_amd/csrc/layers_p.hip
+++ b/infgen_amd/csrc/layers_p.hip
@@ -209,6 +209,8 @@
   constexpr int R = ROWS;
   const int gps = a.A_cap / R;
   const int L = a.num_layers;
+  const size_t kvp = (size_t)kv_pitch_of(a.kv_pitch), ring_stride = a.ring_stride ? (size_t)a.ring_stride : kvp;
+  const int kvsh = __builtin_amdgcn_readfirstlane(kv_shift_of(a.kv_pitch));
   int grp = blockIdx.x;
   if (a.xcd_order) {
     const int per = 8 * gps, bq = grp / per, br = grp % per;
@@ -279,7 +281,7 @@
     }
   };
 
-  auto node_pre = [&](const float* NP, float* nK, float* nV) __attribute__((always_inline)) {
+  auto node_pre = [&](const float* NP, float* nK, float* nV, size_t nstride) __attribute__((always_inline)) {
     const unsigned short* pre = reinterpret_cast<const unsigned short*>(NP + AH_PRE);
     const float* hdr = Vt + VT_N_HDR;
     STAMP(16);
@@ -308,8 +310,8 @@
       kk = kk * splat4(hdr[2]);
       vv = fma4(vv, splat4(hdr[3]), lds4(Vt + VT_N_BV + own));
       if (own_row && !IG_LP_NOKV) {
-        *reinterpret_cast<float4*>(nK + (size_t)row * D + own) = make_float4(kk[0], kk[1], kk[2], kk[3]);
-        *reinterpret_cast<float4*>(nV + (size_t)row * D + own) = make_float4(vv[0], vv[1], vv[2], vv[3]);
+        *reinterpret_cast<float4*>(nK + (size_t)row * nstride + own) = make_float4(kk[0], kk[1], kk[2], kk[3]);
+        *reinterpret_cast<float4*>(nV + (size_t)row * nstride + own) = make_float4(vv[0], vv[1], vv[2], vv[3]);
       }
     }
     STAMP(19);
@@ -354,7 +356,7 @@
   };
 
   auto sublayer = [&](const EdgeSet& es, const EdgeSet& es_next, const float* Ksrc, const float* Vsrc, bool kv_once, const float* P,
-                      const float* NP, float* nK, float* nV) __attribute__((always_inline)) {
+                      const float* NP, float* nK, float* nV, size_t nstride) __attribute__((always_inline)) {
     const unsigned short* post = reinterpret_cast<const unsigned short*>(P + AH_POST);
     const unsigned short* pre_any = reinterpret_cast<const unsigned short*>((NP ? NP : P) + AH_PRE);
     float4 tv0, tv1; int to0, to1;
@@ -396,8 +398,8 @@
             for (int s = 0; s < LP_G; ++s) {
               const int ic = min(i0 + s, mc - 1);
               const int sj = __builtin_amdgcn_readlane(sv, ic);
-              kb[s] = ld8(Ksrc + (size_t)sj * D, kv_once);
-              vb[s] = ld8(Vsrc + (size_t)sj * D, kv_once);
+              kb[s] = ld8(Ksrc + ((size_t)sj << kvsh), kv_once);
+              vb[s] = ld8(Vsrc + ((size_t)sj << kvsh), kv_once);
               if constexpr (R24) rb[s] = ld_r24((size_t)(e_base + c0 + ic));
               else rb[s] = ld8(es.rhat + (size_t)(e_base + c0 + ic) * D, true);
             }
@@ -600,7 +602,7 @@
       row_stats(STp[sp], j, m2, r2); sp ^= 1;
       x += ln_own(f, m2, r2, Vt + VT_LNO_G + own, Vt + VT_LNO_B + own);
     }
-    if (NP) node_pre(NP, nK, nV);
+    if (NP) node_pre(NP, nK, nV, nstride);
     STAMP(20);
   };
 
@@ -616,7 +618,7 @@
     *reinterpret_cast<float4*>(Vt + to0) = tv0;
     *reinterpret_cast<float4*>(Vt + to1) = tv1;
     wg_barrier();
-    node_pre(a.attn_t[0], a.ringK[0] + a.slot_off, a.ringV[0] + a.slot_off);
+    node_pre(a.attn_t[0], a.ringK[0] + a.slot_off, a.ringV[0] + a.slot_off, ring_stride);
   }
   for (int k = 0; k < 3 * L; ++k) {
     const int i = k / 3, kind = k - 3 * i;
@@ -667,7 +669,7 @@
 #endif
     }
     STAMP(0);
-    sublayer(es, es_next, Ksrc, Vsrc, kind == 0, P, NP, nK, nV);
+    sublayer(es, es_next, Ksrc, Vsrc, kind == 0, P, NP, nK, nV, kind == 1 ? kvp : ring_stride);
   }
   if (own_row) *reinterpret_cast<float4*>(a.X + (size_t)row * D + own) = make_float4(x[0], x[1], x[2], x[3]);
 }
diff --git a/infgen_amd/csrc/layout.h b/infgen_amd/csrc/layout.h
--- a/infgen_amd/csrc/layout.h
+++ b/infgen_amd/csrc/layout.h
@@ -78,6 +78,22 @@
   return fourier_pack_size_f32(n) + FH_VEC_SIZE + 2 * (2 * n + 1) * FH_HALF_MAT_FLOATS;
 }
 
+__host__ __device__ inline int kv_pitch_of(int kv_pitch) { return kv_pitch > 0 ? kv_pitch : 128; }
+__host__ __device__ inline int kv_shift_of(int kv_pitch) {
+  int s = 7;
+  while ((128 << (s - 7)) < kv_pitch) ++s;
+  return s;
+}
+__host__ __device__ inline long long ring_row_index(int row, int slot, int rows, int ring, int row_major) {
+  return row_major ? (long long)row * ring + slot : (long long)slot * rows + row;
+}
+__host__ __device__ inline long long ring_store_offset(int slot, int rows, int ring, int row_major, int kv_pitch) {
+  return ring_row_index(0, slot, rows, ring, row_major) * kv_pitch_of(kv_pitch);
+}
+__host__ __device__ inline int ring_row_stride(int ring, int row_major, int kv_pitch) {
+  return (int)(ring_row_index(1, 0, 0, ring, row_major) - ring_row_index(0, 0, 0, ring, row_major)) * kv_pitch_of(kv_pitch);
+}
+
 constexpr float AH_HDR_VERSION = 2.0f;
 
 }
diff --git a/infgen_amd/engine.py b/infgen_amd/engine.py
--- a/infgen_amd/engine.py
+++ b/infgen_amd/engine.py
@@ -343,10 +343,11 @@
                    'infgen_fourier_embed')
         return out
 
-    def attn_pre(self, x, pack, use_src_ln=False, q=None, u=None, k=None, v=None, rows=None):
+    def attn_pre(self, x, pack, use_src_ln=False, q=None, u=None, k=None, v=None, rows=None, kv_stride=0):
         rows = x.shape[0] if rows is None else rows
-        _lib.check(self.lib.infgen_attn_pre(_lib.ptr(x), rows, _lib.ptr(pack), int(use_src_ln), _lib.ptr(q),
-                                            _lib.ptr(u), _lib.ptr(k), _lib.ptr(v), self.stream), 'infgen_attn_pre')
+        _lib.check(self.lib.infgen_attn_pre_kv(_lib.ptr(x), rows, _lib.ptr(pack), int(use_src_ln), _lib.ptr(q),
+                                               _lib.ptr(u), (_lib.ptr_rows if kv_stride else _lib.ptr)(k), (_lib.ptr_rows if kv_stride else _lib.ptr)(v),
+                                               int(kv_stride), self.stream), 'infgen_attn_pre')
 
     def edge_attn(self, rows, q, u, ksrc, vsrc, off, cnt, src, rhat, agg, z, sig, wide=None):
         args = (rows, _lib.ptr(q), _lib.ptr(u), _lib.ptr(ksrc), _lib.ptr(vsrc), _lib.ptr(off), _lib.ptr(cnt),
@@ -612,11 +613,19 @@
         self.X, self.Q, self.U = f(rows, D), f(rows, D), f(rows, 8 * D)
         if self._tap_layers:
             self.tap_x = f(cfg.num_agent_layers, rows, D)
-        self.Ka, self.Va, self.AGG, self.Z, self.SIG = f(rows, D), f(rows, D), f(rows, D), f(rows, 8 * D), f(rows, 8)
-        self.ringK = [f(self.ring, rows, D) for _ in range(L)]
-        self.ringV = [f(self.ring, rows, D) for _ in range(L)]
-        self.mapK = [f(self.S0 * M_cap, D) for _ in range(L)]
-        self.mapV = [f(self.S0 * M_cap, D) for _ in range(L)]
+        self.AGG, self.Z, self.SIG = f(rows, D), f(rows, 8 * D), f(rows, 8)
+        lo = self._effective_options()
+        self.kv_interleave, self.ring_row_major = int(bool(lo.kv_interleave)), int(bool(lo.ring_row_major))
+        self.kv_pitch = 2 * D if self.kv_interleave else D
+
+        def kv_store(n_rows):
+            if not self.kv_interleave:
+                return f(n_rows, D), f(n_rows, D)
+            kv = f(n_rows, 2 * D)
+            return kv[:, :D], kv[:, D:]
+        self.Ka, self.Va = kv_store(rows)
+        self.ringK, self.ringV = map(list, zip(*[kv_store(self.ring * rows) for _ in range(L)]))
+        self.mapK, self.mapV = map(list, zip(*[kv_store(self.S0 * M_cap) for _ in range(L)]))
         self.edges = {}
         totals = i32(3)
         for k, (name, cap) in enumerate((('t', rows * self.W), ('m', rows * 5), ('a', rows * (A_cap - 1)))):
@@ -1089,7 +1098,7 @@
         ops, w, cfg = self.ops, self.w, self.cfg
         x_pt = self.x_pt
         for i in range(cfg.num_agent_layers):
-            ops.attn_pre(x_pt, w.attn_m[i], use_src_ln=True, k=self.mapK[i], v=self.mapV[i])
+            ops.attn_pre(x_pt, w.attn_m[i], use_src_ln=True, k=self.mapK[i], v=self.mapV[i], kv_stride=self.kv_pitch)
 
         if self.insertion:
             self._alloc_insertion()
@@ -1289,14 +1298,15 @@
         c.map_pos, c.map_orient = P(self.map_pos), P(self.map_orient)
         c.map_scene = P(self.map_scene)
         c.tap_x = P(self.tap_x)
+        c.kv_pitch, c.ring_row_major = self.kv_pitch, self.ring_row_major
         for i in range(cfg.num_agent_layers):
             c.attn_t[i], c.attn_m[i], c.attn_a[i] = P(w.attn_t[i]), P(w.attn_m[i]), P(w.attn_a[i])
-            c.ringK[i], c.ringV[i], c.mapK[i], c.mapV[i] = P(self.ringK[i]), P(self.ringV[i]), P(self.mapK[i]), P(self.mapV[i])
+            c.ringK[i], c.ringV[i], c.mapK[i], c.mapV[i] = map(_lib.ptr_rows, (self.ringK[i], self.ringV[i], self.mapK[i], self.mapV[i]))
         c.four_t, c.four_m, c.four_a, c.four_xa = P(w.four_t), P(w.four_m), P(w.four_a), P(w.four_xa)
         c.fusion_pack, c.tok_head_pack, c.st_head_pack = P(w.fusion), P(w.tok_head), P(w.st_head)
         c.tok_tab, c.grid_tab, c.state_emb = P(self.tok_tab), P(self.grid_tab), P(w.state_a_emb)
         c.cat_agent, c.cat_seed, c.vocab, c.grid_xy = P(self.cat_agent), P(self.cat_seed), P(self.vocab), P(self.grid_xy)
-        c.X, c.Q, c.U, c.Ka, c.Va, c.AGG, c.Z, c.SIG = (P(self.X), P(self.Q), P(self.U), P(self.Ka), P(self.Va),
+        c.X, c.Q, c.U, c.Ka, c.Va, c.AGG, c.Z, c.SIG = (P(self.X), P(self.Q), P(self.U), _lib.ptr_rows(self.Ka), _lib.ptr_rows(self.Va),
                                                           P(self.AGG), P(self.Z), P(self.SIG))
         for name, field in (('t', 'et'), ('m', 'em'), ('a', 'ea')):
             e, b = self.edges[name], getattr(c, field)
```
